# maciejkula/spotlight

Hardware: AMD Instinct MI355X
Metric: training interactions/sec, BPR dim=64 (higher is better)
Workload: dtype f32

## Files before the change

spotlight_amd/csrc/slk_api.hip:

```cpp
#include <stdarg.h>

#include <stdlib.h>

#include "slk_common.h"

static char g_create_err[512] = {0};

int slk_fail(slk_ctx *ctx, int code, const char *fmt, ...) {
    char *dst = ctx ? ctx->err : g_create_err;
    va_list ap;
    va_start(ap, fmt);
    vsnprintf(dst, 512, fmt, ap);
    va_end(ap);
    return code;
}

int slk_ensure(slk_ctx *ctx, slk_buf &b, size_t bytes) {
    if (bytes <= b.cap) return SLK_OK;
    if (b.p) {
        SLK_HIP(ctx, hipFree(b.p));
        b.p = nullptr;
        b.cap = 0;
    }
    size_t want = bytes + bytes / 8 + 256;
    void *p = nullptr;
    if (hipMalloc(&p, want) != hipSuccess) {
        (void)hipGetLastError();
        return slk_fail(ctx, SLK_ENOMEM, "hipMalloc of %zu scratch bytes failed", want);
    }
    b.p = p;
    b.cap = want;
    return SLK_OK;
}

int slk_ensure_lflags_host(slk_ctx *ctx, slk_prep_bufs &pb, size_t n) {
    if (n > pb.h_lflags_cap) {
        if (pb.h_lflags) (void)hipHostFree(pb.h_lflags);
        pb.h_lflags = nullptr;
        pb.h_lflags_cap = 0;
        void *p = nullptr;
        const size_t want = n + n / 4 + 64;
        if (hipHostMalloc(&p, want * sizeof(int), hipHostMallocDefault) != hipSuccess) {
            (void)hipGetLastError();
            return slk_fail(ctx, SLK_ENOMEM, "hipHostMalloc of %zu flag words failed", want);
        }
        pb.h_lflags = (int *)p;
        pb.h_lflags_cap = want;
    }
    for (size_t i = 0; i < n; ++i) pb.h_lflags[i] = 1;
    pb.h_lflags_n = n;
    return SLK_OK;
}

void slk_prof_begin(slk_ctx *ctx, int cls, hipStream_t s) {
    if (!ctx->prof_on) return;
    slk_prof_span sp;
    sp.cls = cls;
    for (hipEvent_t *e : {&sp.a, &sp.b}) {
        if (!ctx->ev_pool.empty()) {
            *e = ctx->ev_pool.back();
            ctx->ev_pool.pop_back();
        } else {
            (void)hipEventCreate(e);
        }
    }
    (void)hipEventRecord(sp.a, s);
    ctx->spans.push_back(sp);
}

void slk_prof_end(slk_ctx *ctx, hipStream_t s) {
    if (!ctx->prof_on) return;
    (void)hipEventRecord(ctx->spans.back().b, s);
    if (ctx->spans.size() >= 8192) slk_prof_drain(ctx);
}

int slk_prof_drain(slk_ctx *ctx) {
    for (slk_prof_span &sp : ctx->spans) {
        SLK_HIP(ctx, hipEventSynchronize(sp.b));
        float ms = 0.0f;
        SLK_HIP(ctx, hipEventElapsedTime(&ms, sp.a, sp.b));
        ctx->prof_launches[sp.cls] += 1;
        ctx->prof_ms[sp.cls] += (double)ms;
        ctx->ev_pool.push_back(sp.a);
        ctx->ev_pool.push_back(sp.b);
    }
    ctx->spans.clear();
    return SLK_OK;
}

int slk_prep_stream_init(slk_ctx *ctx) {
    if (ctx->prep_stream) return SLK_OK;
    SLK_HIP(ctx, hipStreamCreateWithFlags(&ctx->prep_stream, hipStreamNonBlocking));
    SLK_HIP(ctx, hipMemsetAsync(&ctx->d_rng->sort_abort, 0, sizeof(int32_t), ctx->prep_stream));
    SLK_HIP(ctx, hipStreamSynchronize(ctx->prep_stream));
    for (hipEvent_t *e : {&ctx->ev_start, &ctx->ev_prep[0], &ctx->ev_prep[1], &ctx->ev_done[0], &ctx->ev_done[1]})
        if (!*e) SLK_HIP(ctx, hipEventCreateWithFlags(e, hipEventDisableTiming));
    return SLK_OK;
}

hipStream_t slk_copy_stream(slk_ctx *ctx) {
    if (!ctx->copy_stream && hipStreamCreateWithFlags(&ctx->copy_stream, hipStreamNonBlocking) != hipSuccess) {
        (void)hipGetLastError();
        ctx->copy_stream = nullptr;
    }
    return ctx->copy_stream;
}

SLK_EXPORT int slk_abi_version(void) { return SLK_ABI_VERSION; }

SLK_EXPORT int slk_ctx_create(slk_ctx **out, int device_id) {
    if (!out) return slk_fail(nullptr, SLK_EINVAL, "slk_ctx_create: out is NULL");
    *out = nullptr;
    int ndev = 0;
    if (hipGetDeviceCount(&ndev) != hipSuccess || ndev <= 0) {
        (void)hipGetLastError();
        return slk_fail(nullptr, SLK_EIO, "slk_ctx_create: no HIP device visible");
    }
    if (device_id < 0 || device_id >= ndev)
        return slk_fail(nullptr, SLK_EINVAL, "slk_ctx_create: device %d out of range (%d devices)",
                        device_id, ndev);
    slk_ctx *ctx = new slk_ctx();
    ctx->device = device_id;
    if (hipSetDevice(device_id) != hipSuccess) {
        delete ctx;
        return slk_fail(nullptr, SLK_EIO, "slk_ctx_create: hipSetDevice(%d) failed", device_id);
    }
    hipDeviceProp_t prop;
    if (hipGetDeviceProperties(&prop, device_id) == hipSuccess && prop.multiProcessorCount > 0) {
        ctx->num_cus = prop.multiProcessorCount;
        if (prop.sharedMemPerBlock > 0) ctx->lds_per_block = prop.sharedMemPerBlock;
        if (prop.maxSharedMemoryPerMultiProcessor > 0) ctx->lds_per_cu = prop.maxSharedMemoryPerMultiProcessor;
        if (ctx->lds_per_cu < ctx->lds_per_block) ctx->lds_per_cu = ctx->lds_per_block;
    }
    if (hipMalloc(reinterpret_cast<void **>(&ctx->d_rng), sizeof(slk_rng_dev)) != hipSuccess) {
        delete ctx;
        return slk_fail(nullptr, SLK_ENOMEM, "slk_ctx_create: hipMalloc(rng) failed");
    }
    (void)hipMemset(ctx->d_rng, 0, sizeof(slk_rng_dev));
    int32_t pos = 624;
    (void)hipMemcpy(&ctx->d_rng->pos, &pos, sizeof(pos), hipMemcpyHostToDevice);
    *out = ctx;
    return SLK_OK;
}

SLK_EXPORT void slk_ctx_destroy(slk_ctx *ctx) {
    if (!ctx) return;
    if (ctx->shadow_active)
        fprintf(stderr, "libspotlight_hip: slk_ctx_destroy with an OPEN item-bias shadow (slk_bias_shadow_begin without _end): "
                        "the caller's item biases and their Adagrad accumulator keep their pre-scope values; the training of the "
                        "scope is lost\n");
    if (ctx->pp_active)
        fprintf(stderr, "libspotlight_hip: slk_ctx_destroy with an OPEN user-row ping-pong (slk_user_pingpong_begin without _end): "
                        "the rows whose current copy is the ctx's are not written back; the caller's user table is a mix of pre- and "
                        "in-scope rows -- the training of the scope is lost\n");
    (void)hipSetDevice(ctx->device);
    (void)hipDeviceSynchronize();
    slk_prof_drain(ctx);
    for (hipEvent_t e : ctx->ev_pool) (void)hipEventDestroy(e);
    slk_buf *bufs[] = {&ctx->raw, &ctx->cnt, &ctx->neg32, &ctx->ukey[0], &ctx->ukey[1], &ctx->uval[0],
                       &ctx->uval[1], &ctx->uit, &ctx->ikey[0], &ctx->ikey[1], &ctx->ipay[0],
                       &ctx->ipay[1], &ctx->gk, &ctx->sk, &ctx->snap, &ctx->losspart,
                       &ctx->sort_tmp, &ctx->dgrad[0], &ctx->dgrad[1], &ctx->dgrad[2], &ctx->dgrad[3], &ctx->ipart,
                       &ctx->ipart_meta, &ctx->upart_meta, &ctx->pf_neg, &ctx->call_neg, &ctx->mt_tmp, &ctx->bias_shadow, &ctx->pp_alt,
                       &ctx->pp_flags};
    for (slk_buf *b : bufs)
        if (b->p) (void)hipFree(b->p);
    for (slk_buf &b : ctx->extra)
        if (b.p) (void)hipFree(b.p);
    for (slk_prep_bufs &pb : ctx->pb) {
        slk_buf *pbs[] = {&pb.neg32, &pb.ukey[0], &pb.ukey[1], &pb.uval[0], &pb.uval[1], &pb.uit, &pb.ikey[0],
                          &pb.ikey[1], &pb.ipay[0], &pb.ipay[1], &pb.bik[0], &pb.bik[1], &pb.bip[0], &pb.bip[1],
                          &pb.buk[0], &pb.buk[1], &pb.bup[0], &pb.bup[1], &pb.lflags, &pb.mflag, &pb.msorted};
        for (slk_buf *b : pbs)
            if (b->p) (void)hipFree(b->p);
        if (pb.ev_lflags) (void)hipEventDestroy(pb.ev_lflags);
        if (pb.h_lflags) (void)hipHostFree(pb.h_lflags);
    }
    for (hipEvent_t e : {ctx->ev_start, ctx->ev_prep[0], ctx->ev_prep[1], ctx->ev_done[0], ctx->ev_done[1], ctx->ev_coef[0], ctx->ev_coef[1],
                         ctx->ev_sampled})
        if (e) (void)hipEventDestroy(e);
    for (void *h : ctx->h_coef)
        if (h) (void)hipHostFree(h);
    if (ctx->prep_stream) (void)hipStreamDestroy(ctx->prep_stream);
    if (ctx->copy_stream) (void)hipStreamDestroy(ctx->copy_stream);
    if (ctx->d_rng) (void)hipFree(ctx->d_rng);
    for (uint32_t *j : ctx->d_jump)
        if (j) (void)hipFree(j);
    delete ctx;
}

SLK_EXPORT const char *slk_last_error(const slk_ctx *ctx) { return ctx ? ctx->err : g_create_err; }

namespace {
struct slk_opt_desc {
    const char *name;
    int64_t lo, hi;
    int64_t (*get)(const slk_ctx *);
    void (*set)(slk_ctx *, int64_t);
};
#define SLK_OPT(name_, member_, lo_, hi_)                                              \
    {name_, (int64_t)(lo_), (int64_t)(hi_), [](const slk_ctx *c) -> int64_t { return (int64_t)c->member_; }, \
     [](slk_ctx *c, int64_t v) { c->member_ = (decltype(c->member_))v; }}
const int64_t SLK_OPT_MAX = INT64_MAX;
const slk_opt_desc slk_options[] = {
    SLK_OPT("chunk_interactions", opt_chunk_interactions, 1, SLK_OPT_MAX),
    SLK_OPT("overlap_prep", opt_overlap_prep, 0, 2),
    SLK_OPT("overlap_min_batch", opt_overlap_min_batch, 0, SLK_OPT_MAX),
    SLK_OPT("prefetch_wait", opt_prefetch_wait, 0, 1),
    SLK_OPT("mt_long_min_blocks", opt_mt_long_min_blocks, 2, SLK_OPT_MAX),
    SLK_OPT("sort_big_min", opt_sort_big_min, 1, SLK_OPT_MAX),
    SLK_OPT("sort_debug", opt_sort_debug, 0, 3),
    SLK_OPT("item_grid_mult", opt_item_grid_mult, 1, 4096),
    SLK_OPT("user_grid_mult", opt_user_grid_mult, 1, 4096),
    SLK_OPT("seq_variant", opt_seq_variant, 0, 1),
    SLK_OPT("explicit_fused", opt_explicit_fused, 0, 1),
    SLK_OPT("epoch_kernel", opt_epoch_kernel, 0, 1),
    SLK_OPT("item_lat_max_tiles", opt_item_lat_max_tiles, 0, SLK_OPT_MAX),
    SLK_OPT("epoch_adaptive", opt_epoch_adaptive, 0, 1),
    SLK_OPT("epoch_adaptive_max_batch", opt_epoch_adaptive_max_batch, 1, (int64_t)1 << 20),
    SLK_OPT("epoch_max_batch", opt_epoch_max_batch, 1, (int64_t)1 << 20),
    SLK_OPT("epoch_max_grid", opt_epoch_max_grid, 1, 16384),
    SLK_OPT("epoch_barrier", opt_epoch_barrier, -1, 1),
    SLK_OPT("epoch_cooperative", opt_epoch_cooperative, 0, 1),
    SLK_OPT("epoch_debug", opt_epoch_debug, 0, 63),
    SLK_OPT("epoch_dense_elems", opt_epoch_dense_elems, 0, SLK_OPT_MAX),
    SLK_OPT("user_lat_max_batch", opt_user_lat_max_batch, 0, SLK_OPT_MAX),
    SLK_OPT("item_long_gate", opt_item_long_gate, 0, 1),
    SLK_OPT("adaptive_late_min_batch", opt_adaptive_late_min_batch, 0, SLK_OPT_MAX),
    SLK_OPT("shuffle_band", opt_shuffle_band, 0, 1024),
    SLK_OPT("nt", opt_nt, 0, 63),
    SLK_OPT("record_nt_min_bytes", opt_record_nt_min_bytes, 0, SLK_OPT_MAX),
    SLK_OPT("user_bias_zero_hint", opt_user_bias_zero_hint, 0, 1),
    SLK_OPT("user_grid_own_occ", opt_user_grid_own_occ, 0, 1),
    SLK_OPT("item_single_min_items", opt_item_single_min_items, 0, SLK_OPT_MAX),
};
#undef SLK_OPT
const slk_opt_desc slk_eval_options[] = {
    {"topk_items_per_wg", 0, (int64_t)1 << 40, [](const slk_ctx *c) -> int64_t { return c->opt_topk_items_per_wg; },
     [](slk_ctx *c, int64_t v) { c->opt_topk_items_per_wg = v; }},
    {"eval_items_per_wg", 0, (int64_t)1 << 40, [](const slk_ctx *c) -> int64_t { return c->opt_eval_items_per_wg; },
     [](slk_ctx *c, int64_t v) { c->opt_eval_items_per_wg = v; }},
    {"foldin_wg_min_len", 0, (int64_t)1 << 40, [](const slk_ctx *c) -> int64_t { return c->opt_foldin_wg_min_len; },
     [](slk_ctx *c, int64_t v) { c->opt_foldin_wg_min_len = v; }},
};
const slk_opt_desc *slk_find_option(const char *name) {
    for (const slk_opt_desc &d : slk_options)
        if (!strcmp(name, d.name)) return &d;
    for (const slk_opt_desc &d : slk_eval_options)
        if (!strcmp(name, d.name)) return &d;
    return nullptr;
}
}

SLK_EXPORT int slk_ctx_set_option(slk_ctx *ctx, const char *name, int64_t value) {
    if (!ctx || !name) return SLK_EINVAL;
    const slk_opt_desc *d = slk_find_option(name);
    if (!d || value < d->lo || value > d->hi)
        return slk_fail(ctx, SLK_EINVAL, "slk_ctx_set_option: unknown option or bad value: %s = %lld", name,
                        (long long)value);
    d->set(ctx, value);
    return SLK_OK;
}

SLK_EXPORT int slk_ctx_get_option(slk_ctx *ctx, const char *name, int64_t *value) {
    if (!ctx || !name || !value) return SLK_EINVAL;
    const slk_opt_desc *d = slk_find_option(name);
    if (!d) return slk_fail(ctx, SLK_EINVAL, "slk_ctx_get_option: unknown option %s", name);
    *value = d->get(ctx);
    return SLK_OK;
}

SLK_EXPORT int slk_ctx_get_stat(slk_ctx *ctx, const char *name, int64_t *value) {
    if (!ctx || !name || !value) return SLK_EINVAL;
    if (!strcmp(name, "shuffle_sweeps")) *value = ctx->fy_sweeps;
    else if (!strcmp(name, "shuffle_fallbacks")) *value = ctx->fy_fallbacks;
    else if (!strcmp(name, "epoch_refused")) *value = ctx->epoch_refused ? 1 : 0;
    else if (!strcmp(name, "user_long_launches")) *value = ctx->stat_user_long;
    else if (!strcmp(name, "item_long_launches")) *value = ctx->stat_item_long;
    else if (!strcmp(name, "overlapped_chunks")) *value = ctx->stat_overlapped;
    else if (!strcmp(name, "prefetched_chunks")) *value = ctx->stat_prefetched;
    else if (!strcmp(name, "shadowed_calls")) *value = ctx->stat_shadowed;
    else if (!strcmp(name, "pingpong_calls")) *value = ctx->stat_pingpong;
    else if (!strcmp(name, "single_minibatches")) *value = ctx->stat_single;
    else if (!strcmp(name, "lds_per_block")) *value = (int64_t)ctx->lds_per_block;
    else if (!strcmp(name, "lds_per_cu")) *value = (int64_t)ctx->lds_per_cu;
    else if (!strcmp(name, "prefetch_pending")) *value = !ctx->pf.valid ? 0 : (ctx->pf.all ? 2 : 1);
    else return slk_fail(ctx, SLK_EINVAL, "slk_ctx_get_stat: unknown statistic %s", name);
    return SLK_OK;
}

SLK_EXPORT int slk_profile_enable(slk_ctx *ctx, int32_t on) {
    if (!ctx) return SLK_EINVAL;
    if (!on) slk_prof_drain(ctx);
    ctx->prof_on = on != 0;
    return SLK_OK;
}

SLK_EXPORT int slk_profile_read(slk_ctx *ctx, int32_t cls, int64_t *launches, double *total_ms) {
    if (!ctx || cls < 0 || cls >= SLK_K_COUNT) return SLK_EINVAL;
    int rc = slk_prof_drain(ctx);
    if (rc) return rc;
    if (launches) *launches = ctx->prof_launches[cls];
    if (total_ms) *total_ms = ctx->prof_ms[cls];
    return SLK_OK;
}

SLK_EXPORT int slk_profile_reset(slk_ctx *ctx) {
    if (!ctx) return SLK_EINVAL;
    int rc = slk_prof_drain(ctx);
    for (int i = 0; i < SLK_K_COUNT; ++i) {
        ctx->prof_launches[i] = 0;
        ctx->prof_ms[i] = 0.0;
    }
    return rc;
}
```

spotlight_amd/csrc/slk_bilinear.hip:

```cpp
#include <math.h>

#include "slk_kernels.h"

#ifndef SLK_PP_PIPE
#define SLK_PP_PIPE 2
#endif
template <int VEC, int G, int UPD, int UMODE, bool BLOOM, bool LAT = false, bool ULONG = false, bool PP = false, bool SGL = false>
__global__ __launch_bounds__(256) void k_user_pass(slk_pass_args a) {
    static_assert(!LAT || (UMODE == 0 && !BLOOM), "LAT is the pair mode over plain tables");
    static_assert(!PP || (UMODE == 0 && !BLOOM), "PP is the pair mode over plain tables");
    static_assert(!SGL || (PP && !LAT && !ULONG && UPD == SLK_UPD_ADAGRAD), "SGL: the plain ping-pong form, Adagrad");
    static_assert(!ULONG || !BLOOM, "long user runs: plain tables");
    constexpr uint32_t S = SLK_USER_TILE;
    constexpr bool PRE = UMODE != 0;
    constexpr bool EXPL = UMODE == 2;
    __shared__ double red[256];
    constexpr int GPB = 256 / G;
    const int lane = threadIdx.x % G;
    const int grp = threadIdx.x / G;
    const int D = a.D;
    const int d0 = lane * VEC;
    const bool on = d0 < D;
    const uint32_t stride = gridDim.x * GPB;
    float loss_acc = 0.0f;

    const uint32_t n_turns = ULONG ? (a.end - a.begin + S - 1u) / S : a.end - a.begin;
    constexpr bool PIPE = PP && !LAT && !ULONG && SLK_PP_PIPE >= 1;
    constexpr bool PIPE_IDS = PIPE && SLK_PP_PIPE >= 2;
    uint32_t pk_key = 0u, pk_prev = 0u, pk_flag = 0u, pn_key = 0u, pn_prev = 0u;
    uint32_t pk_ip = 0u, pk_in = 0u, pn_ip = 0u, pn_in = 0u;
    uint32_t pk_mf = 0u, pn_mf = 0u;
    auto ld_mf = [&](uint32_t pos) -> uint32_t { return (uint32_t)*reinterpret_cast<const uint16_t *>(a.mflag + 2 * (size_t)pos); };
    if (PIPE) {
        const uint32_t t0 = blockIdx.x * GPB + grp;
        if (t0 < n_turns) {
            pk_key = a.ukey[a.begin + t0];
            pk_prev = t0 > 0u ? a.ukey[a.begin + t0 - 1u] : 0u;
            if (PIPE_IDS) {
                pk_ip = a.uit[2 * (size_t)(a.begin + t0)];
                pk_in = a.uit[2 * (size_t)(a.begin + t0) + 1];
            }
            if (SGL) pk_mf = ld_mf(a.begin + t0);
            pk_flag = (uint32_t)a.uflag[pk_key & a.umask];
        }
        if (t0 + stride < n_turns) {
            pn_key = a.ukey[a.begin + t0 + stride];
            pn_prev = a.ukey[a.begin + t0 + stride - 1u];
            if (PIPE_IDS) {
                pn_ip = a.uit[2 * (size_t)(a.begin + t0 + stride)];
                pn_in = a.uit[2 * (size_t)(a.begin + t0 + stride) + 1];
            }
            if (SGL) pn_mf = ld_mf(a.begin + t0 + stride);
        }
    }
    for (uint32_t turn = blockIdx.x * GPB + grp; turn < n_turns; turn += stride) {
    const uint32_t p_lo = a.begin + (ULONG ? turn * S : turn);
    const uint32_t p_hi = ULONG ? (p_lo + S < a.end ? p_lo + S : a.end) : p_lo + 1u;
    for (uint32_t p = p_lo; p < p_hi; ++p) {
        const bool nt_keys = (SLK_NT_OF(a) & 8) != 0;
        const uint32_t key = PIPE ? pk_key : slk_ld_u32(a.ukey + p, nt_keys);
        uint32_t lat_ip = 0u, lat_in = 0u;
        bool is_head;
        uint32_t cur_piped = 0u, mf_piped = 0u;
        if (PIPE) {
            is_head = !(p > a.begin && pk_prev == key);
            cur_piped = pk_flag;
            lat_ip = pk_ip;
            lat_in = pk_in;
            mf_piped = pk_mf;
            pk_mf = pn_mf;
            pk_key = pn_key;
            pk_prev = pn_prev;
            pk_ip = pn_ip;
            pk_in = pn_in;
            if (turn + stride < n_turns) pk_flag = (uint32_t)a.uflag[pn_key & a.umask];
            if (turn + 2u * stride < n_turns) {
                pn_key = a.ukey[p + 2u * stride];
                pn_prev = a.ukey[p + 2u * stride - 1u];
                if (PIPE_IDS) {
                    pn_ip = a.uit[2 * (size_t)(p + 2u * stride)];
                    pn_in = a.uit[2 * (size_t)(p + 2u * stride) + 1];
                }
                if (SGL) pn_mf = ld_mf(p + 2u * stride);
            }
        } else if (LAT) {
            const uint32_t prev = p > a.begin ? a.ukey[p - 1] : ~key;
            lat_ip = a.uit[2 * (size_t)p];
            lat_in = a.uit[2 * (size_t)p + 1];
            is_head = prev != key;
        } else {
            is_head = !(p > a.begin && a.ukey[p - 1] == key);
        }
        bool run_long = false;
        uint32_t seg_limit = a.end;
        if (ULONG) {
            const uint32_t rel = p - a.begin;
            if (is_head) {
                const uint32_t t0 = a.begin + (rel + S - 1u) / S * S;
                run_long = t0 + S <= a.end && a.ukey[t0 + S - 1u] == key;
            } else if (rel % S == 0u) {
                run_long = (rel >= S && a.ukey[p - S] == key) || (p + S <= a.end && a.ukey[p + S - 1u] == key);
                is_head = false;
            }
            if (!is_head && !(run_long && rel % S == 0u)) continue;
            if (run_long) seg_limit = a.begin + (rel / S + 1u) * S < a.end ? a.begin + (rel / S + 1u) * S : a.end;
        } else if (!is_head) {
            continue;
        }
        const uint32_t user = key & a.umask;
        const size_t uoff = (size_t)user * D + d0;
        constexpr bool pp = PP;
        const uint32_t cur = PIPE ? cur_piped : (pp ? (uint32_t)a.uflag[user] : 0u);
        float *const unew = pp ? (cur ? a.P[0] : a.P0alt) + uoff : nullptr;
        slk_vec<VEC> u;
        if (BLOOM)
            u = slk_emb_vec<VEC>(a.P[0], a.ub, user, D, d0, on);
        else
            u = on ? slk_vload_if_nt<VEC>((cur ? a.P0alt : a.P[0]) + uoff, (SLK_NT_OF(a) & 1) != 0) : slk_vzero<VEC>();
        const float bu = (UMODE == 0 && !BLOOM && a.ubz) ? 0.0f : a.P[2][user];
        constexpr bool EARLY_ADAM = !BLOOM && UPD == SLK_UPD_SPARSE_ADAM && !ULONG;
        constexpr bool EARLY_STATE = ((EXPL || LAT || SGL || (PIPE && SLK_PP_PIPE >= 3)) && !BLOOM && UPD == SLK_UPD_ADAGRAD) || EARLY_ADAM;
        slk_vec<VEC> su = slk_vzero<VEC>(), su2 = slk_vzero<VEC>();
        if (EARLY_STATE && on) su = slk_vload_if_nt<VEC>(a.S1[0] + uoff, (SLK_NT_OF(a) & 1) != 0);
        if (EARLY_ADAM && on) su2 = slk_vload_if_nt<VEC>(a.S2[0] + uoff, (SLK_NT_OF(a) & 1) != 0);
        float sbu = 0.0f, sbu2 = 0.0f;
        if (EARLY_STATE && !(SGL && a.ubz)) sbu = a.S1[2][user];
        if (EARLY_ADAM) sbu2 = a.S2[2][user];
        slk_vec<VEC> gu = slk_vzero<VEC>();
        float gbu = 0.0f;
        uint32_t q = p;
        constexpr bool NEXT_KEY = UMODE != 0;
        uint32_t next_key = 0;
        if (NEXT_KEY) next_key = (q + 1 < seg_limit) ? a.ukey[q + 1] : ~key;
        do {
            float *rec = a.snap + (size_t)(q - a.begin) * a.RS;
            uint32_t e_item = 0;
            float e_rating = 0.0f;
            if (EXPL) {
                e_item = a.uit[q];
                e_rating = a.ratings[a.uk[q]];
            }
            if (on && !pp) slk_vstore_if_nt<VEC>(rec + d0, u, (SLK_NT_OF(a) & 16) != 0);
            if (!PRE) {
                uint32_t ip, in;
                if ((LAT || PIPE_IDS) && q == p) {
                    ip = lat_ip;
                    in = lat_in;
                } else {
                    ip = slk_ld_u32(a.uit + 2 * (size_t)q, nt_keys);
                    in = slk_ld_u32(a.uit + 2 * (size_t)q + 1, nt_keys);
                }
                slk_vec<VEC> vi, vj;
                if (BLOOM) {
                    vi = slk_emb_vec<VEC>(a.P[1], a.ib, ip, D, d0, on);
                    vj = slk_emb_vec<VEC>(a.P[1], a.ib, in, D, d0, on);
                } else {
                    vi = on ? slk_vload<VEC>(a.P[1] + (size_t)ip * D + d0) : slk_vzero<VEC>();
                    vj = on ? slk_vload<VEC>(a.P[1] + (size_t)in * D + d0) : slk_vzero<VEC>();
                }
                const float bip = a.P[3][SLK_B3(a, ip)], bin = a.P[3][SLK_B3(a, in)];
                uint32_t mf = 0xffffu;
                slk_vec<VEC> svi = slk_vzero<VEC>(), svj = slk_vzero<VEC>();
                float sbi = 0.0f, sbj = 0.0f;
                if (SGL) {
                    mf = (q == p) ? mf_piped : ld_mf(q);
                    const bool nt_rows = (SLK_NT_OF(a) & 2) != 0;
                    if (!(mf & 0xffu)) {
                        if (on) svi = slk_vload_if_nt<VEC>(a.S1[1] + (size_t)ip * D + d0, nt_rows);
                        if (lane == 0) sbi = a.S1[3][SLK_B3(a, ip)];
                    }
                    if (!(mf >> 8)) {
                        if (on) svj = slk_vload_if_nt<VEC>(a.S1[1] + (size_t)in * D + d0, nt_rows);
                        if (lane == 0) sbj = a.S1[3][SLK_B3(a, in)];
                    }
                }
                const float sp = slk_group_sum<G>(slk_vdot<VEC>(u, vi)) + bu + bip;
                const float sn = slk_group_sum<G>(slk_vdot<VEC>(u, vj)) + bu + bin;
                float l, gp, gn;
                slk_pair_loss(a.loss_kind, sp, sn, a.inv_b, l, gp, gn);
#pragma unroll
                for (int i = 0; i < VEC; ++i) gu.v[i] += gp * vi.v[i] + gn * vj.v[i];
                gbu += gp + gn;
                if (lane == 0) {
                    if (pp) {
                        float srcf;
                        const uint32_t src = user | (cur << 31);
                        memcpy(&srcf, &src, 4);
                        reinterpret_cast<float4 *>(a.gsn)[q - a.begin] = make_float4(gp, srcf, gn, srcf);
                    } else {
                        float *gq = a.gsn + 2 * (size_t)(q - a.begin);
                        gq[0] = gp;
                        gq[1] = gn;
                    }
                    loss_acc += l;
                }
                if (SGL) {
                    const bool nt_rows = (SLK_NT_OF(a) & 2) != 0;
                    auto once = [&](uint32_t item, slk_vec<VEC> &v, slk_vec<VEC> &sv, float g, float b, float bs) {
                        const size_t voff = (size_t)item * D + d0;
                        if (on) {
                            slk_vec<VEC> gv;
#pragma unroll
                            for (int i = 0; i < VEC; ++i) gv.v[i] = 0.0f + g * u.v[i];
                            slk_apply_vec_pre<VEC, UPD>(a, 1, voff, v, sv, gv, nullptr, nt_rows);
                        }
                        if (lane == 0) {
                            slk_vec<1> bpv, bsv, gbv;
                            bpv.v[0] = b;
                            bsv.v[0] = bs;
                            gbv.v[0] = 0.0f + g;
                            slk_apply_vec_pre<1, UPD>(a, 3, SLK_B3(a, item), bpv, bsv, gbv);
                        }
                    };
                    if (!(mf & 0xffu) && gp != 0.0f) once(ip, vi, svi, gp, bip, sbi);
                    if (!(mf >> 8) && gn != 0.0f) once(in, vj, svj, gn, bin, sbj);
                }
            } else if (EXPL) {
                const uint32_t it = e_item;
                const float bi = a.P[3][SLK_B3(a, it)];
                slk_vec<VEC> v;
                if (BLOOM)
                    v = slk_emb_vec<VEC>(a.P[1], a.ib, it, D, d0, on);
                else
                    v = on ? slk_vload<VEC>(a.P[1] + (size_t)it * D + d0) : slk_vzero<VEC>();
                const float sc = slk_group_sum<G>(slk_vdot<VEC>(u, v)) + bu + bi;
                float l, g;
                slk_explicit_loss(a.loss_kind, sc, e_rating, a.inv_b, a.end - a.begin, l, g);
                if (lane == 0) {
                    a.gsn[q - a.begin] = g;
                    loss_acc += l;
                }
                if (g != 0.0f) {
                    slk_vaxpy<VEC>(gu, g, v);
                    gbu += g;
                }
            } else {
                const size_t kb = (size_t)a.uk[q] * a.NP, qb = (size_t)q * a.NP;
                for (int s0 = 0; s0 < a.NP; s0 += G) {
                    const int s = s0 + lane;
                    float gs = 0.0f;
                    uint32_t it_l = 0u;
                    if (s < a.NP) {
                        gs = a.gk[kb + s];
                        it_l = a.uit[qb + s];
                        a.gsn[(size_t)(q - a.begin) * a.NP + s] = gs;
                    }
                    unsigned long long live = slk_group_or<G>(gs != 0.0f ? 1ull << lane : 0ull);
                    while (live) {
                        const int j0 = __builtin_ctzll(live);
                        live &= live - 1ull;
                        const bool two = live != 0ull;
                        const int j1 = two ? __builtin_ctzll(live) : j0;
                        if (two) live &= live - 1ull;
                        const uint32_t i0 = __shfl(it_l, j0, G), i1 = __shfl(it_l, j1, G);
                        const float g0 = __shfl(gs, j0, G), g1 = __shfl(gs, j1, G);
                        slk_vec<VEC> v0, v1 = slk_vzero<VEC>();
                        if (BLOOM) {
                            v0 = slk_emb_vec<VEC>(a.P[1], a.ib, i0, D, d0, on);
                            if (two) v1 = slk_emb_vec<VEC>(a.P[1], a.ib, i1, D, d0, on);
                        } else {
                            v0 = on ? slk_vload<VEC>(a.P[1] + (size_t)i0 * D + d0) : slk_vzero<VEC>();
                            if (two && on) v1 = slk_vload<VEC>(a.P[1] + (size_t)i1 * D + d0);
                        }
                        slk_vaxpy<VEC>(gu, g0, v0);
                        gbu += g0;
                        if (two) {
                            slk_vaxpy<VEC>(gu, g1, v1);
                            gbu += g1;
                        }
                    }
                }
            }
            ++q;
            if (NEXT_KEY) {
                if (next_key != key) break;
                next_key = (q + 1 < seg_limit) ? a.ukey[q + 1] : ~key;
            } else if (!(q < seg_limit && a.ukey[q] == key)) {
                break;
            }
        } while (true);

        if (ULONG && run_long) {
            const bool ends = !(q < a.end && a.ukey[q] == key);
            const size_t slot = 2 * (size_t)((p - a.begin) / S) + (is_head ? 1u : 0u);
            float *pp = a.upart + slot * (size_t)a.UPS;
            if (on) slk_vstore<VEC>(pp + d0, gu);
            if (lane == 0) {
                pp[a.UPS - 1] = gbu;
                a.upart_meta[2 * slot] = key;
                a.upart_meta[2 * slot + 1] = (a.upart_gen << SLK_IPART_GEN_SHIFT) | (is_head ? (uint32_t)SLK_IPART_STARTS : 0u) |
                                             (ends ? (uint32_t)SLK_IPART_ENDS : 0u);
                if (is_head) atomicAdd(a.upart_count, 1u);
            }
            p = q - 1u;
            continue;
        }
        if (BLOOM && a.ub.n_hash) {
            if (on) slk_vstore<VEC>(a.urec + (size_t)(p - a.begin) * a.RSU + d0, gu);
        } else if (on) {
            if (EARLY_ADAM)
                slk_apply_vec_pre<VEC, UPD, true>(a, 0, uoff, u, su, gu, &su2, (SLK_NT_OF(a) & 1) != 0, unew);
            else if (EARLY_STATE)
                slk_apply_vec_pre<VEC, UPD>(a, 0, uoff, u, su, gu, nullptr, (SLK_NT_OF(a) & 1) != 0, unew);
            else
                slk_apply_vec<VEC, UPD>(a, 0, uoff, u, gu, (SLK_NT_OF(a) & 1) != 0, unew);
        }
        if (pp && lane == 0) a.uflag[user] = (uint8_t)(cur ^ 1u);
        if (EARLY_ADAM) {
            if (lane == 0) {
                slk_vec<1> bpv, bsv, bsv2, gbv;
                bpv.v[0] = bu;
                bsv.v[0] = sbu;
                bsv2.v[0] = sbu2;
                gbv.v[0] = gbu;
                slk_apply_vec_pre<1, UPD, true>(a, 2, user, bpv, bsv, gbv, &bsv2);
            }
        } else if (EARLY_STATE) {
            if (lane == 0 && gbu != 0.0f) {
                slk_vec<1> bpv, bsv, gbv;
                bpv.v[0] = bu;
                bsv.v[0] = sbu;
                gbv.v[0] = gbu;
                slk_apply_vec_pre<1, UPD>(a, 2, user, bpv, bsv, gbv);
            }
        } else if (lane == 0) {
            slk_apply_bias<UPD>(a, 2, user, gbu);
        }
        if (ULONG) p = q - 1u;
    }
    }
    if (!PRE || EXPL) {
        const double tot = slk_block_sum_256((double)loss_acc, red);
        if (threadIdx.x == 0) a.loss_partial[blockIdx.x] = tot;
    }
}

template <int VEC, int G, int UPD, bool PP = false>
__global__ __launch_bounds__(256) void k_user_stitch(slk_pass_args a) {
    constexpr int GPB = 256 / G;
    constexpr uint32_t S = SLK_USER_TILE;
    const int lane = threadIdx.x % G;
    const int grp = threadIdx.x / G;
    const int D = a.D;
    const int d0 = lane * VEC;
    const bool on = d0 < D;
    const uint32_t ntiles = (a.end - a.begin + S - 1u) / S;
    if (*a.upart_count == 0u) return;
    const uint32_t gen = a.upart_gen;
    for (uint32_t tile = blockIdx.x * GPB + grp; tile < ntiles; tile += gridDim.x * GPB) {
        const size_t slot = 2 * (size_t)tile + 1;
        const uint32_t fl = a.upart_meta[2 * slot + 1];
        if ((fl >> SLK_IPART_GEN_SHIFT) != gen) continue;
        const uint32_t key = a.upart_meta[2 * slot];
        const float *pp = a.upart + slot * (size_t)a.UPS;
        slk_vec<VEC> gu = on ? slk_vload<VEC>(pp + d0) : slk_vzero<VEC>();
        float gbu = pp[a.UPS - 1];
        uint32_t t2 = tile + 1;
        bool more = (fl & SLK_IPART_ENDS) == 0;
        constexpr int R = G <= 16 ? 2 : 1;
        constexpr int TPR = R * G;
        constexpr bool SPEC = G <= 16;
        while (more) {
            slk_vec<VEC> sc[SPEC ? TPR : 1];
            float sb[SPEC ? TPR : 1];
            if (SPEC) {
#pragma unroll
                for (int e = 0; e < (SPEC ? TPR : 1); ++e) {
                    sc[e] = slk_vzero<VEC>();
                    sb[e] = 0.0f;
                    if (t2 + (uint32_t)e < ntiles) {
                        const float *q = a.upart + 2 * (size_t)(t2 + (uint32_t)e) * (size_t)a.UPS;
                        if (on) sc[e] = slk_vload<VEC>(q + d0);
                        sb[e] = q[a.UPS - 1];
                    }
                }
            }
            uint2 kf[R];
#pragma unroll
            for (int j = 0; j < R; ++j) {
                const uint32_t tl = t2 + (uint32_t)(lane + j * G);
                kf[j] = make_uint2(0u, 0u);
                if (tl < ntiles) kf[j] = *reinterpret_cast<const uint2 *>(a.upart_meta + 4 * (size_t)tl);
            }
            uint32_t f[R];
#pragma unroll
            for (int j = 0; j < R; ++j) {
                f[j] = kf[j].y;
                if (t2 + (uint32_t)(lane + j * G) >= ntiles || (f[j] >> SLK_IPART_GEN_SHIFT) != gen || (f[j] & SLK_IPART_STARTS) ||
                    kf[j].x != key)
                    f[j] = 0u;
                else
                    f[j] |= 1u;
            }
            int cnt = 0;
            bool ended = false;
#pragma unroll
            for (int j = 0; j < R; ++j) {
                if (!ended && cnt == j * G) {
                    const unsigned long long valid = slk_group_or<G>((f[j] & 1u) ? 1ull << lane : 0ull);
                    const unsigned long long ends = slk_group_or<G>((f[j] & SLK_IPART_ENDS) ? 1ull << lane : 0ull);
                    const unsigned long long full = G == 64 ? ~0ull : (1ull << G) - 1ull;
                    int c = (valid & full) == full ? G : __builtin_ctzll(~valid);
                    const unsigned long long e_in = ends & (c == 64 ? ~0ull : (1ull << c) - 1ull);
                    if (e_in) {
                        c = __builtin_ctzll(e_in) + 1;
                        ended = true;
                    }
                    cnt += c;
                }
            }
            if (SPEC) {
#pragma unroll
                for (int e = 0; e < (SPEC ? TPR : 1); ++e) {
                    if (e < cnt) {
#pragma unroll
                        for (int i = 0; i < VEC; ++i) gu.v[i] += sc[e].v[i];
                        gbu += sb[e];
                    }
                }
            }
            for (int l0 = 0; !SPEC && l0 < cnt; l0 += SLK_STITCH_BATCH) {
                slk_vec<VEC> cc[SLK_STITCH_BATCH];
                float cb[SLK_STITCH_BATCH];
#pragma unroll
                for (int e = 0; e < SLK_STITCH_BATCH; ++e) {
                    cc[e] = slk_vzero<VEC>();
                    cb[e] = 0.0f;
                    if (l0 + e < cnt) {
                        const float *q = a.upart + 2 * (size_t)(t2 + (uint32_t)(l0 + e)) * (size_t)a.UPS;
                        if (on) cc[e] = slk_vload<VEC>(q + d0);
                        cb[e] = q[a.UPS - 1];
                    }
                }
#pragma unroll
                for (int e = 0; e < SLK_STITCH_BATCH; ++e) {
                    if (l0 + e < cnt) {
#pragma unroll
                        for (int i = 0; i < VEC; ++i) gu.v[i] += cc[e].v[i];
                        gbu += cb[e];
                    }
                }
            }
            more = !ended && cnt == TPR;
            t2 += (uint32_t)TPR;
        }
        const uint32_t user = key & a.umask;
        const size_t uoff = (size_t)user * D + d0;
        constexpr bool pingpong = PP;
        uint32_t cur = 0u;
        if (pingpong) cur = __shfl(lane == 0 ? (uint32_t)a.uflag[user] : 0u, 0, G);
        if (on) {
            slk_vec<VEC> u = slk_vload_if_nt<VEC>((cur ? a.P0alt : a.P[0]) + uoff, (SLK_NT_OF(a) & 1) != 0);
            slk_apply_vec<VEC, UPD>(a, 0, uoff, u, gu, (SLK_NT_OF(a) & 1) != 0, pingpong ? (cur ? a.P[0] : a.P0alt) + uoff : nullptr);
        }
        if (pingpong && lane == 0) a.uflag[user] = (uint8_t)(cur ^ 1u);
        if (lane == 0) slk_apply_bias<UPD>(a, 2, user, gbu);
    }
}

__global__ __launch_bounds__(256) void k_user_long_flags(const uint32_t *ukey, uint32_t n, uint32_t per_mb, int *flags) {
    constexpr uint32_t S = SLK_USER_TILE;
    const uint32_t tiles_per_mb = (per_mb + S - 1) / S;
    const uint32_t n_mb = (n + per_mb - 1) / per_mb;
    for (uint32_t i = blockIdx.x * 256 + threadIdx.x; i < n_mb * tiles_per_mb; i += gridDim.x * 256) {
        const uint32_t mb = i / tiles_per_mb, q = i - mb * tiles_per_mb;
        const uint32_t w0 = mb * per_mb, w1 = (n - w0 < per_mb) ? n : w0 + per_mb;
        const uint32_t t0 = w0 + q * S;
        if (t0 >= w1 || w1 - t0 < S) continue;
        if (ukey[t0] == ukey[t0 + S - 1]) flags[mb] = 1;
    }
}

template <int VEC, int G>
__global__ __launch_bounds__(256) void k_score_pass(slk_pass_args a) {
    constexpr int GPB = 256 / G;
    const int lane = threadIdx.x % G;
    const int grp = threadIdx.x / G;
    const int D = a.D;
    const int d0 = lane * VEC;
    const bool on = d0 < D;
    const uint32_t stride = gridDim.x * GPB;
    for (uint32_t q = a.begin + blockIdx.x * GPB + grp; q < a.end; q += stride) {
        const uint32_t user = a.ukey[q] & a.umask;
        const slk_vec<VEC> u = slk_emb_vec<VEC>(a.P[0], a.ub, user, D, d0, on);
        const float bu = a.P[2][user];
        const size_t kb = (size_t)a.uk[q] * a.NP, qb = (size_t)q * a.NP;
        constexpr int SB = 3;
        for (int s0 = 0; s0 < a.NP; s0 += SB) {
            slk_vec<VEC> v[SB];
            float bi[SB];
#pragma unroll
            for (int j = 0; j < SB; ++j) {
                v[j] = slk_vzero<VEC>();
                bi[j] = 0.0f;
                if (s0 + j < a.NP) {
                    const uint32_t it = a.uit[qb + s0 + j];
                    v[j] = slk_emb_vec<VEC>(a.P[1], a.ib, it, D, d0, on);
                    bi[j] = a.P[3][SLK_B3(a, it)];
                }
            }
#pragma unroll
            for (int j = 0; j < SB; ++j) {
                const float sc = slk_group_sum<G>(slk_vdot<VEC>(u, v[j])) + bu + bi[j];
                if (lane == 0 && s0 + j < a.NP) a.sk[kb + s0 + j] = sc;
            }
        }
    }
}


__global__ __launch_bounds__(256) void k_explicit_loss(const float *sk, const float *ratings, float *gk, uint32_t k0,
                                                       uint32_t bm, int loss_kind, float inv_b, double *loss_partial) {
    __shared__ double red[256];
    double lsum = 0.0;
    for (uint32_t c = blockIdx.x * 256 + threadIdx.x; c < bm; c += gridDim.x * 256) {
        const float sc = sk[k0 + c], r = ratings[k0 + c];
        float l, g;
        slk_explicit_loss(loss_kind, sc, r, inv_b, bm, l, g);
        gk[k0 + c] = g;
        lsum += (double)l;
    }
    const double tot = slk_block_sum_256(lsum, red);
    if (threadIdx.x == 0) loss_partial[blockIdx.x] = tot;
}


struct slk_sweep_all_args {
    float *p[4], *s1[4], *s2[4], *g[4];
    size_t numel[4];
    unsigned first[5];
    int adam;
    float wd, w1, beta2, omb2, step_size, bc2_sqrt, eps, clr;
};

__global__ __launch_bounds__(256) void k_dense_sweep_all(slk_sweep_all_args a) {
    int t = 0;
    while (t < 3 && blockIdx.x >= a.first[t + 1]) ++t;
    const size_t local = blockIdx.x - a.first[t], nblk = a.first[t + 1] - a.first[t];
    float *p = a.p[t], *s1 = a.s1[t], *s2 = a.s2[t], *g = a.g[t];
    const size_t numel = a.numel[t];
    if (a.adam) {
        for (size_t e = local * 256 + threadIdx.x; e < numel; e += nblk * 256) {
            const float gv = g[e] + a.wd * p[e];
            g[e] = 0.0f;
            const float m = s1[e] + a.w1 * (gv - s1[e]);
            const float v = s2[e] * a.beta2 + a.omb2 * (gv * gv);
            s1[e] = m;
            s2[e] = v;
            p[e] += -a.step_size * (m / (sqrtf(v) / a.bc2_sqrt + a.eps));
        }
    } else {
        for (size_t e = local * 256 + threadIdx.x; e < numel; e += nblk * 256) {
            const float gv = g[e] + a.wd * p[e];
            g[e] = 0.0f;
            const float s = s1[e] + gv * gv;
            s1[e] = s;
            p[e] += -a.clr * (gv / (sqrtf(s) + a.eps));
        }
    }
}

__global__ __launch_bounds__(256) void k_i64_to_u32(const int64_t *in, uint32_t *out, size_t n) {
    for (size_t i = (size_t)blockIdx.x * 256 + threadIdx.x; i < n; i += (size_t)gridDim.x * 256)
        out[i] = (uint32_t)in[i];
}

__global__ __launch_bounds__(256) void k_u32_to_i64(const uint32_t *in, int64_t *out, size_t n) {
    for (size_t i = (size_t)blockIdx.x * 256 + threadIdx.x; i < n; i += (size_t)gridDim.x * 256)
        out[i] = (int64_t)in[i];
}

__global__ __launch_bounds__(256) void k_pack_items(const uint32_t *uk, const int64_t *items,
                                                    const uint32_t *neg32, uint32_t nc, int nn, uint32_t *uit) {
    const int NP = nn + 1;
    for (uint32_t q = blockIdx.x * 256 + threadIdx.x; q < nc; q += gridDim.x * 256) {
        const uint32_t k = uk[q];
        uit[(size_t)q * NP] = (uint32_t)items[k];
        for (int r = 0; r < nn; ++r) uit[(size_t)q * NP + 1 + r] = neg32[(size_t)k * nn + r];
    }
}

__global__ __launch_bounds__(256) void k_invert_perm(const uint32_t *uk, uint32_t nc, uint32_t *qk) {
    for (uint32_t q = blockIdx.x * 256 + threadIdx.x; q < nc; q += gridDim.x * 256) qk[uk[q]] = q;
}

__global__ __launch_bounds__(256) void k_build_live_keys(const uint32_t *live, const uint32_t *uit, uint32_t n_live,
                                                         slk_bloom_dev ib, bool hashed, uint32_t *key, uint32_t *val) {
    const uint32_t H = hashed ? (uint32_t)ib.n_hash : 1u;
    for (uint32_t e = blockIdx.x * 256 + threadIdx.x; e < n_live * H; e += gridDim.x * 256) {
        const uint32_t l = e / H, h = e - l * H;
        const uint32_t r = live[l];
        uint32_t k = 0xffffffffu;
        if (r != 0xffffffffu) k = hashed ? slk_bloom_row(ib, uit[r], (int)h) : uit[r];
        key[e] = k;
        val[e] = r;
    }
}

__global__ __launch_bounds__(256) void k_build_item_bloom_keys(const uint32_t *uit, uint32_t nocc, int NP,
                                                               uint32_t bsz, unsigned cbits, slk_bloom_dev ib,
                                                               uint32_t *key, uint32_t *val) {
    const uint32_t H = (uint32_t)ib.n_hash;
    for (uint32_t e = blockIdx.x * 256 + threadIdx.x; e < nocc * H; e += gridDim.x * 256) {
        const uint32_t r = e / H, h = e - r * H;
        const uint32_t q = r / (uint32_t)NP;
        key[e] = ((q / bsz) << cbits) | slk_bloom_row(ib, uit[r], (int)h);
        val[e] = r;
    }
}

__global__ __launch_bounds__(256) void k_build_user_bloom_keys(const uint32_t *ukey, uint32_t umask, uint32_t nc,
                                                               uint32_t bsz, unsigned cbits, slk_bloom_dev ub,
                                                               uint32_t *key, uint32_t *val) {
    const uint32_t H = (uint32_t)ub.n_hash;
    for (uint32_t e = blockIdx.x * 256 + threadIdx.x; e < nc * H; e += gridDim.x * 256) {
        const uint32_t p = e / H, h = e - p * H;
        const uint32_t mb = p / bsz;
        const bool head = (p % bsz == 0) || ukey[p - 1] != ukey[p];
        key[e] = (mb << cbits) | (head ? slk_bloom_row(ub, ukey[p] & umask, (int)h) : ub.rows);
        val[e] = p;
    }
}

template <int VEC, int G>
__global__ __launch_bounds__(256) void k_predict(const float *U, const float *V, const float *bu,
                                                 const float *bi, int D, slk_bloom_dev ub, slk_bloom_dev ib,
                                                 const int64_t *users, int64_t n_users, const int64_t *items,
                                                 int64_t n, float *out) {
    constexpr int GPB = 256 / G;
    const int lane = threadIdx.x % G;
    const int grp = threadIdx.x / G;
    const int d0 = lane * VEC;
    const bool on = d0 < D;
    for (int64_t k = (int64_t)blockIdx.x * GPB + grp; k < n; k += (int64_t)gridDim.x * GPB) {
        const int64_t u = users[n_users == 1 ? 0 : k];
        const int64_t i = items ? items[k] : k;
        const slk_vec<VEC> a = slk_emb_vec<VEC>(U, ub, (uint32_t)u, D, d0, on);
        const slk_vec<VEC> b = slk_emb_vec<VEC>(V, ib, (uint32_t)i, D, d0, on);
        const float s = (slk_chain_dot<VEC, G>(a, b) + bu[u]) + bi[i];
        if (lane == 0) out[k] = s;
    }
}

typedef slk_pass_fn pass_fn;

template <int VEC, int G, bool BLOOM>
static pass_fn user_pass_fn2(int upd, int umode) {
    if (umode == 2) {
        if (upd == SLK_UPD_ADAGRAD) return k_user_pass<VEC, G, SLK_UPD_ADAGRAD, 2, BLOOM>;
        if (upd == SLK_UPD_SPARSE_ADAM) return k_user_pass<VEC, G, SLK_UPD_SPARSE_ADAM, 2, BLOOM>;
        if (upd == SLK_UPD_SGD) return k_user_pass<VEC, G, SLK_UPD_SGD, 2, BLOOM>;
        return k_user_pass<VEC, G, SLK_UPD_GRAD_ONLY, 2, BLOOM>;
    }
    if (umode == 1) {
        if (upd == SLK_UPD_ADAGRAD) return k_user_pass<VEC, G, SLK_UPD_ADAGRAD, 1, BLOOM>;
        if (upd == SLK_UPD_SPARSE_ADAM) return k_user_pass<VEC, G, SLK_UPD_SPARSE_ADAM, 1, BLOOM>;
        if (upd == SLK_UPD_SGD) return k_user_pass<VEC, G, SLK_UPD_SGD, 1, BLOOM>;
        return k_user_pass<VEC, G, SLK_UPD_GRAD_ONLY, 1, BLOOM>;
    }
    if (upd == SLK_UPD_ADAGRAD) return k_user_pass<VEC, G, SLK_UPD_ADAGRAD, 0, BLOOM>;
    if (upd == SLK_UPD_SPARSE_ADAM) return k_user_pass<VEC, G, SLK_UPD_SPARSE_ADAM, 0, BLOOM>;
    if (upd == SLK_UPD_SGD) return k_user_pass<VEC, G, SLK_UPD_SGD, 0, BLOOM>;
    return k_user_pass<VEC, G, SLK_UPD_GRAD_ONLY, 0, BLOOM>;
}

template <int VEC, int G, bool ULONG = false>
static pass_fn user_pass_lat_fn(int upd) {
    if (upd == SLK_UPD_ADAGRAD) return k_user_pass<VEC, G, SLK_UPD_ADAGRAD, 0, false, true, ULONG>;
    if (upd == SLK_UPD_SPARSE_ADAM) return k_user_pass<VEC, G, SLK_UPD_SPARSE_ADAM, 0, false, true, ULONG>;
    if (upd == SLK_UPD_SGD) return k_user_pass<VEC, G, SLK_UPD_SGD, 0, false, true, ULONG>;
    return k_user_pass<VEC, G, SLK_UPD_GRAD_ONLY, 0, false, true, ULONG>;
}

template <int VEC, int G, bool LAT, bool ULONG>
static pass_fn user_pass_pp_fn(int upd) {
    if (upd == SLK_UPD_ADAGRAD) return k_user_pass<VEC, G, SLK_UPD_ADAGRAD, 0, false, LAT, ULONG, true>;
    if (upd == SLK_UPD_SPARSE_ADAM) return k_user_pass<VEC, G, SLK_UPD_SPARSE_ADAM, 0, false, LAT, ULONG, true>;
    return k_user_pass<VEC, G, SLK_UPD_SGD, 0, false, LAT, ULONG, true>;
}
template <int VEC, int G>
static pass_fn user_pass_sgl_fn() {
    return k_user_pass<VEC, G, SLK_UPD_ADAGRAD, 0, false, false, false, true, true>;
}
template <int VEC, int G>
static slk_item_fns item_pass_sgl_fn() {
    return {k_item_pass<VEC, G, SLK_UPD_ADAGRAD, SLK_ITEM_SNAPPPS>, k_item_stitch<VEC, G, SLK_UPD_ADAGRAD, SLK_PART_BOTH>,
            k_item_pass<VEC, G, SLK_UPD_ADAGRAD, SLK_ITEM_SNAPPPS, SLK_PART_BOTH, false>,
            k_item_pass<VEC, G, SLK_UPD_ADAGRAD, SLK_ITEM_SNAPPPS, SLK_PART_BOTH, false, 4>};
}
template <int VEC, int G>
static pass_fn user_stitch_pp_fn(int upd) {
    if (upd == SLK_UPD_ADAGRAD) return k_user_stitch<VEC, G, SLK_UPD_ADAGRAD, true>;
    if (upd == SLK_UPD_SPARSE_ADAM) return k_user_stitch<VEC, G, SLK_UPD_SPARSE_ADAM, true>;
    return k_user_stitch<VEC, G, SLK_UPD_SGD, true>;
}
template <int VEC, int G>
static slk_item_fns item_pass_pp_fn(int upd) {
    if (upd == SLK_UPD_ADAGRAD)
        return {k_item_pass<VEC, G, SLK_UPD_ADAGRAD, SLK_ITEM_SNAPPP>, k_item_stitch<VEC, G, SLK_UPD_ADAGRAD, SLK_PART_BOTH>,
                k_item_pass<VEC, G, SLK_UPD_ADAGRAD, SLK_ITEM_SNAPPP, SLK_PART_BOTH, false>,
                k_item_pass<VEC, G, SLK_UPD_ADAGRAD, SLK_ITEM_SNAPPP, SLK_PART_BOTH, false, 4>};
    if (upd == SLK_UPD_SPARSE_ADAM)
        return {k_item_pass<VEC, G, SLK_UPD_SPARSE_ADAM, SLK_ITEM_SNAPPP>, k_item_stitch<VEC, G, SLK_UPD_SPARSE_ADAM, SLK_PART_BOTH>,
                k_item_pass<VEC, G, SLK_UPD_SPARSE_ADAM, SLK_ITEM_SNAPPP, SLK_PART_BOTH, false>,
                k_item_pass<VEC, G, SLK_UPD_SPARSE_ADAM, SLK_ITEM_SNAPPP, SLK_PART_BOTH, false, 4>};
    return {k_item_pass<VEC, G, SLK_UPD_SGD, SLK_ITEM_SNAPPP>, k_item_stitch<VEC, G, SLK_UPD_SGD, SLK_PART_BOTH>,
            k_item_pass<VEC, G, SLK_UPD_SGD, SLK_ITEM_SNAPPP, SLK_PART_BOTH, false>,
            k_item_pass<VEC, G, SLK_UPD_SGD, SLK_ITEM_SNAPPP, SLK_PART_BOTH, false, 4>};
}

template <int VEC, int G, int UMODE>
static pass_fn user_pass_long_fn1(int upd) {
    if (upd == SLK_UPD_ADAGRAD) return k_user_pass<VEC, G, SLK_UPD_ADAGRAD, UMODE, false, false, true>;
    if (upd == SLK_UPD_SPARSE_ADAM) return k_user_pass<VEC, G, SLK_UPD_SPARSE_ADAM, UMODE, false, false, true>;
    if (upd == SLK_UPD_SGD) return k_user_pass<VEC, G, SLK_UPD_SGD, UMODE, false, false, true>;
    return k_user_pass<VEC, G, SLK_UPD_GRAD_ONLY, UMODE, false, false, true>;
}
template <int VEC, int G>
static pass_fn user_pass_long_fn(int upd, int umode) {
    if (umode == 2) return user_pass_long_fn1<VEC, G, 2>(upd);
    if (umode == 1) return user_pass_long_fn1<VEC, G, 1>(upd);
    return user_pass_long_fn1<VEC, G, 0>(upd);
}
template <int VEC, int G>
static pass_fn user_stitch_fn(int upd) {
    if (upd == SLK_UPD_ADAGRAD) return k_user_stitch<VEC, G, SLK_UPD_ADAGRAD>;
    if (upd == SLK_UPD_SPARSE_ADAM) return k_user_stitch<VEC, G, SLK_UPD_SPARSE_ADAM>;
    if (upd == SLK_UPD_SGD) return k_user_stitch<VEC, G, SLK_UPD_SGD>;
    return k_user_stitch<VEC, G, SLK_UPD_GRAD_ONLY>;
}

template <int VEC, int G>
static pass_fn user_pass_fn(int upd, int umode, bool bloom) {
    return bloom ? user_pass_fn2<VEC, G, true>(upd, umode) : user_pass_fn2<VEC, G, false>(upd, umode);
}


int slk_check_tables(slk_ctx *ctx, const slk_tables *t, unsigned table_mask, int *vec, int *g, bool shadow_ok, bool pingpong_ok) {
    if (!t) return slk_fail(ctx, SLK_EINVAL, "tables is NULL");
    for (int i = 0; i < 4; ++i)
        if (((table_mask >> i) & 1u) && !t->d_param[i])
            return slk_fail(ctx, SLK_EINVAL, "tables->d_param[%d] is NULL", i);
    if (!shadow_ok && (table_mask & 8u) && ctx->shadow_active && t->d_param[3] == ctx->shadow_src_p)
        return slk_fail(ctx, SLK_EINVAL, "the item biases of these tables are shadowed (slk_bias_shadow_begin): the array is stale until "
                                         "slk_bias_shadow_end, and only slk_bilinear_train indexes the shadow");
    if (!pingpong_ok && (table_mask & 1u) && ctx->pp_active && t->d_param[0] == ctx->pp_src_u)
        return slk_fail(ctx, SLK_EINVAL, "the user rows of these tables are ping-ponged (slk_user_pingpong_begin): the array holds only "
                                         "some of the current rows until slk_user_pingpong_end, and only slk_bilinear_train reads both copies");
    if (((table_mask & 5u) && (t->num_users < 1 || t->num_users >= ((int64_t)1 << 31))) || t->num_items < 1 ||
        t->num_items >= ((int64_t)1 << 31))
        return slk_fail(ctx, SLK_EINVAL, "table rows must be in [1, 2^31): users %lld items %lld",
                        (long long)t->num_users, (long long)t->num_items);
    if (!slk_pick_layout(t->dim, vec, g))
        return slk_fail(ctx, SLK_EINVAL,
                        "embedding dim %d unsupported (need dim %% 4 == 0 and <= 256, or dim <= 64)", t->dim);
    const slk_bloom *bl[2] = {(table_mask & 1u) ? t->user_bloom : nullptr, (table_mask & 2u) ? t->item_bloom : nullptr};
    for (int side = 0; side < 2; ++side) {
        const slk_bloom *b = bl[side];
        if (!b) continue;
        if (b->n_hash < 1 || b->n_hash > 8 || b->rows < 1 || b->rows >= ((int64_t)1 << 30) || b->skip_row >= b->rows ||
            b->skip_row < -1 || b->padding_idx < -1)
            return slk_fail(ctx, SLK_EINVAL, "bad BloomEmbedding descriptor: rows %lld n_hash %d skip_row %lld",
                            (long long)b->rows, b->n_hash, (long long)b->skip_row);
    }
    return SLK_OK;
}

int slk_check_optim(slk_ctx *ctx, const slk_optim *optim, unsigned table_mask) {
    if (!optim) return slk_fail(ctx, SLK_EINVAL, "optim is NULL");
    if (optim->kind < SLK_OPT_ADAGRAD || optim->kind > SLK_OPT_SGD)
        return slk_fail(ctx, SLK_EINVAL, "unknown optimizer kind %d", optim->kind);
    if (optim->kind == SLK_OPT_SGD) {
        if (optim->weight_decay != 0.0) return slk_fail(ctx, SLK_EINVAL, "SGD: weight_decay must be 0 (a full-table sweep per step is not built)");
        return SLK_OK;
    }
    const bool need_s2 = optim->kind == SLK_OPT_SPARSE_ADAM || optim->kind == SLK_OPT_ADAM_DENSE;
    for (int i = 0; i < 4; ++i) {
        if (!((table_mask >> i) & 1u)) continue;
        if (!optim->d_state1[i]) return slk_fail(ctx, SLK_EINVAL, "optim->d_state1[%d] is NULL", i);
        if (need_s2 && !optim->d_state2[i]) return slk_fail(ctx, SLK_EINVAL, "optim->d_state2[%d] is NULL", i);
    }
    if (optim->kind == SLK_OPT_ADAGRAD && optim->weight_decay != 0.0)
        return slk_fail(ctx, SLK_EINVAL, "row-sparse Adagrad requires weight_decay == 0 (use ADAGRAD_DENSE)");
    return SLK_OK;
}

int slk_ensure_dgrad(slk_ctx *ctx, const size_t elems[4], unsigned table_mask, hipStream_t s) {
    for (int t = 0; t < 4; ++t) {
        if (!((table_mask >> t) & 1u)) continue;
        if (ctx->dgrad_elems[t] != elems[t] || !ctx->dgrad[t].p) {
            int rc = slk_ensure(ctx, ctx->dgrad[t], elems[t] * 4);
            if (rc) return rc;
            SLK_HIP(ctx, hipMemsetAsync(ctx->dgrad[t].p, 0, elems[t] * 4, s));
            ctx->dgrad_elems[t] = elems[t];
        }
    }
    return SLK_OK;
}

int slk_dense_sweeps(slk_ctx *ctx, float *const params[4], const slk_optim *optim, unsigned table_mask,
                     hipStream_t s) {
    const double step = (double)(optim->step + 1);
    slk_prof_begin(ctx, SLK_K_DENSE_SWEEP, s);
    slk_sweep_all_args w;
    memset(&w, 0, sizeof(w));
    w.wd = (float)optim->weight_decay;
    w.eps = (float)optim->eps;
    w.adam = optim->kind == SLK_OPT_ADAM_DENSE;
    if (w.adam) {
        const double bc1 = 1.0 - pow(optim->beta1, step), bc2 = 1.0 - pow(optim->beta2, step);
        w.w1 = (float)(1.0 - optim->beta1);
        w.beta2 = (float)optim->beta2;
        w.omb2 = (float)(1.0 - optim->beta2);
        w.step_size = (float)(optim->lr / bc1);
        w.bc2_sqrt = (float)sqrt(bc2);
    } else {
        w.clr = (float)(optim->lr / (1.0 + (step - 1.0) * optim->lr_decay));
    }
    unsigned blocks = 0;
    for (int t = 0; t < 4; ++t) {
        w.first[t] = blocks;
        if (!((table_mask >> t) & 1u)) continue;
        w.p[t] = params[t];
        w.s1[t] = optim->d_state1[t];
        w.s2[t] = optim->d_state2[t];
        w.g[t] = (float *)ctx->dgrad[t].p;
        w.numel[t] = ctx->dgrad_elems[t];
        blocks += slk_grid_for(ctx, w.numel[t], 256);
    }
    w.first[4] = blocks;
    if (blocks) {
        hipLaunchKernelGGL(k_dense_sweep_all, dim3(blocks), dim3(256), 0, s, w);
        SLK_LAUNCH_CHECK(ctx, "k_dense_sweep_all");
    }
    slk_prof_end(ctx, s);
    return SLK_OK;
}

int slk_launch_i64_to_u32(slk_ctx *ctx, const int64_t *in, uint32_t *out, size_t n, hipStream_t s) {
    hipLaunchKernelGGL(k_i64_to_u32, dim3(slk_grid_for(ctx, n, 256)), dim3(256), 0, s, in, out, n);
    SLK_LAUNCH_CHECK(ctx, "k_i64_to_u32");
    return SLK_OK;
}

SLK_EXPORT int slk_bilinear_predict(slk_ctx *ctx, const slk_tables *tables, const int64_t *d_users,
                                    int64_t n_users, const int64_t *d_items, int64_t n, float *d_out,
                                    void *stream) {
    if (!ctx) return SLK_EINVAL;
    int vec, g, rc;
    if ((rc = slk_check_tables(ctx, tables, 15u, &vec, &g))) return rc;
    if (n < 0 || !d_users || (n > 0 && !d_out)) return slk_fail(ctx, SLK_EINVAL, "slk_bilinear_predict: bad arguments");
    if (n_users != 1 && n_users != n)
        return slk_fail(ctx, SLK_EINVAL, "slk_bilinear_predict: n_users must be 1 or n (%lld vs %lld)",
                        (long long)n_users, (long long)n);
    if (n == 0) return SLK_OK;
    SLK_HIP(ctx, hipSetDevice(ctx->device));
    hipStream_t s = (hipStream_t)stream;
    ctx->last_stream = s;
    slk_prof_begin(ctx, SLK_K_SCORE, s);
    if (n_users == 1 && !d_items) {
        if (n != tables->num_items)
            return slk_fail(ctx, SLK_EINVAL, "slk_bilinear_predict: d_items == NULL scores all %lld items, n is %lld",
                            (long long)tables->num_items, (long long)n);
        const float *rep, *rbias;
        const int64_t *gmap;
        if ((rc = slk_eval_user_rep(ctx, tables, vec, g, d_users, &rep, &rbias, &gmap, s))) return rc;
        rc = slk_eval_predict_all(ctx, tables, rep, rbias, gmap, d_out, s);
        slk_prof_end(ctx, s);
        return rc;
    }
#define SLK_PREDICT(V_, G_)                                                                          \
    hipLaunchKernelGGL((k_predict<V_, G_>), dim3(slk_grid_for(ctx, (size_t)n, 256 / G_)), dim3(256), 0, s, \
                       (const float *)tables->d_param[0], (const float *)tables->d_param[1],          \
                       (const float *)tables->d_param[2], (const float *)tables->d_param[3],          \
                       (int)tables->dim, ubd, ibd, d_users, n_users, d_items, n, d_out)
    slk_bloom_dev ubd, ibd;
    slk_bloom_to_dev(tables->user_bloom, &ubd);
    slk_bloom_to_dev(tables->item_bloom, &ibd);
    SLK_FOR_LAYOUT(vec, g, SLK_PREDICT);
#undef SLK_PREDICT
    SLK_LAUNCH_CHECK(ctx, "k_predict");
    slk_prof_end(ctx, s);
    return SLK_OK;
}

struct train_call {
    enum { TRAIN, RESERVE, PREFETCH } mode;
    const slk_tables *tables;
    slk_optim *optim;
    const int64_t *users, *items;
    const float *ratings;
    const int64_t *neg_in;
    int64_t *neg_out;
    float *mb_loss;
    int64_t n, batch_size;
    int32_t loss, n_neg;
    hipStream_t s;
};

struct train_plan {
    int vec, g, D;
    int RS, RSU, UPS;
    size_t utiles;
    unsigned ubits, ibits, ucbits, icbits;
    slk_bloom_dev ubd, ibd;
    int Hu, Hi;
    bool bloom, adaptive, expl, fused, pre, dense, late;
    int nn, NP, umode, nsets;
    int64_t bsz, mb_per_chunk, chunk_cap, occ_mult;
    size_t nc_max, n_chunks;
    bool side, pingpong, sgl_on, shadowed, one_draw, epoch_route;
    size_t dense_elems[4];
};

struct train_run {
    const uint32_t *neg_all;
    int64_t mb_global;
    bool epoch_route;
};

struct train_kernels {
    pass_fn upass, spass, upass_lat, upass_long, upass_lat_long, ustitch, upass_sgl;
    slk_item_fns ipass, ipass_rows, ipass_bias, rpass_rows, ipass_sgl;
    unsigned gpb;
    int occ_user, occ_sgl;
};

static inline uint32_t *u32p(const slk_buf &b) { return (uint32_t *)b.p; }
static inline float *f32p(const slk_buf &b) { return (float *)b.p; }
static inline int64_t chunk_begin(const train_plan &p, size_t ck) { return (int64_t)ck * p.chunk_cap; }
static inline uint32_t chunk_len(const train_plan &p, const train_call &c, size_t ck) {
    const int64_t c1 = chunk_begin(p, ck + 1);
    return (uint32_t)((c1 < c.n ? c1 : c.n) - chunk_begin(p, ck));
}

static int run_training(slk_ctx *ctx, const train_call &c);

SLK_EXPORT int slk_bilinear_train(slk_ctx *ctx, const slk_tables *tables, slk_optim *optim,
                                  const int64_t *d_users, const int64_t *d_items, int64_t n,
                                  int64_t batch_size, int32_t loss, int32_t n_neg, const int64_t *d_neg_in,
                                  int64_t *d_neg_out, float *d_mb_loss, void *stream) {
    return run_training(ctx, {train_call::TRAIN, tables, optim, d_users, d_items, nullptr, d_neg_in, d_neg_out, d_mb_loss, n,
                              batch_size, loss, n_neg, (hipStream_t)stream});
}

SLK_EXPORT int slk_bilinear_reserve(slk_ctx *ctx, const slk_tables *tables, const slk_optim *optim, int64_t n,
                                    int64_t batch_size, int32_t loss, int32_t n_neg, void *stream) {
    slk_optim o;
    if (!optim) return slk_fail(ctx, SLK_EINVAL, "optim is NULL");
    o = *optim;
    return run_training(ctx, {train_call::RESERVE, tables, &o, nullptr, nullptr, nullptr, nullptr, nullptr, nullptr, n, batch_size,
                              loss, n_neg, (hipStream_t)stream});
}

SLK_EXPORT int slk_bilinear_prefetch(slk_ctx *ctx, const slk_tables *tables, const slk_optim *optim, const int64_t *d_users,
                                     const int64_t *d_items, int64_t n, int64_t batch_size, int32_t loss, int32_t n_neg,
                                     const uint32_t *h_key, int32_t pos, void *stream) {
    if (!ctx) return SLK_EINVAL;
    if (!optim) return slk_fail(ctx, SLK_EINVAL, "optim is NULL");
    if (h_key) {
        if (pos < 0 || pos > 624) return slk_fail(ctx, SLK_EINVAL, "slk_bilinear_prefetch: pos %d outside [0, 624]", pos);
        SLK_HIP(ctx, hipSetDevice(ctx->device));
        if (ctx->sampled_valid && ctx->ev_sampled) SLK_HIP(ctx, hipEventSynchronize(ctx->ev_sampled));
        int rc = slk_rng_write_state(ctx, h_key, pos);
        if (rc) return rc;
    }
    slk_optim o = *optim;
    return run_training(ctx, {train_call::PREFETCH, tables, &o, d_users, d_items, nullptr, nullptr, nullptr, nullptr, n, batch_size,
                              loss, n_neg, (hipStream_t)stream});
}

SLK_EXPORT int slk_bilinear_train_explicit(slk_ctx *ctx, const slk_tables *tables, slk_optim *optim,
                                           const int64_t *d_users, const int64_t *d_items, const float *d_ratings,
                                           int64_t n, int64_t batch_size, int32_t loss, float *d_mb_loss,
                                           void *stream) {
    if (ctx && (loss < SLK_LOSS_REGRESSION || loss > SLK_LOSS_LOGISTIC))
        return slk_fail(ctx, SLK_EINVAL, "slk_bilinear_train_explicit: loss kind %d is not regression/poisson/logistic", loss);
    if (ctx && n > 0 && !d_ratings) return slk_fail(ctx, SLK_EINVAL, "slk_bilinear_train_explicit: d_ratings is NULL");
    return run_training(ctx, {train_call::TRAIN, tables, optim, d_users, d_items, d_ratings, nullptr, nullptr, d_mb_loss, n,
                              batch_size, loss, 0, (hipStream_t)stream});
}

static int plan_training(slk_ctx *ctx, const train_call &c, train_plan *plan) {
    train_plan &p = *plan;
    const slk_tables *tables = c.tables;
    const slk_optim *optim = c.optim;
    const bool reserve = c.mode == train_call::RESERVE, prefetch = c.mode == train_call::PREFETCH;
    const int64_t n = c.n;
    int rc;
    p.n_chunks = 0;
    if ((rc = slk_check_tables(ctx, tables, 15u, &p.vec, &p.g, true, true))) return rc;
    if ((rc = slk_check_optim(ctx, optim, 15u))) return rc;
    if (n < 0 || c.batch_size < 1) return slk_fail(ctx, SLK_EINVAL, "slk_bilinear_train: n %lld batch_size %lld",
                                                   (long long)n, (long long)c.batch_size);
    if (c.loss < SLK_LOSS_POINTWISE || c.loss > SLK_LOSS_LOGISTIC)
        return slk_fail(ctx, SLK_EINVAL, "unknown loss kind %d", c.loss);
    p.adaptive = c.loss == SLK_LOSS_ADAPTIVE_HINGE;
    p.expl = c.loss >= SLK_LOSS_REGRESSION;
    if (p.expl != (c.ratings != nullptr) && !reserve)
        return slk_fail(ctx, SLK_EINVAL, "ratings go with (and only with) the regression/poisson/logistic losses");
    p.fused = p.expl && ctx->opt_explicit_fused;
    p.pre = p.adaptive || p.expl;
    p.umode = p.fused ? 2 : (p.pre ? 1 : 0);
    p.nn = p.adaptive ? c.n_neg : (p.expl ? 0 : 1);
    if (!p.expl && (p.nn < 1 || p.nn > 1024)) return slk_fail(ctx, SLK_EINVAL, "num_negative_samples %d outside [1, 1024]", p.nn);
    p.NP = p.nn + 1;
    p.dense = optim->kind == SLK_OPT_ADAM_DENSE || optim->kind == SLK_OPT_ADAGRAD_DENSE;
    if (n == 0) return SLK_OK;
    if (!reserve && (!c.users || !c.items || (!c.mb_loss && !prefetch)))
        return slk_fail(ctx, SLK_EINVAL, "slk_bilinear_train: NULL id/loss pointer");
    if (c.batch_size * (int64_t)p.NP >= ((int64_t)1 << 31))
        return slk_fail(ctx, SLK_EINVAL, "batch_size * (1 + negatives) must be < 2^31");
    SLK_HIP(ctx, hipSetDevice(ctx->device));
    ctx->last_stream = c.s;

    p.D = tables->dim;
    p.ubits = slk_bits_for((uint64_t)tables->num_users - 1);
    p.ibits = slk_bits_for((uint64_t)tables->num_items - 1);
    unsigned idbits = p.ubits > p.ibits ? p.ubits : p.ibits;
    slk_bloom_to_dev(tables->user_bloom, &p.ubd);
    slk_bloom_to_dev(tables->item_bloom, &p.ibd);
    p.bloom = p.ubd.n_hash || p.ibd.n_hash;
    const int Hu = p.Hu = p.ubd.n_hash, Hi = p.Hi = p.ibd.n_hash;
    p.ucbits = Hu ? slk_bits_for((uint64_t)p.ubd.rows) : 0;
    p.icbits = Hi ? slk_bits_for((uint64_t)p.ibd.rows - 1) : 0;
    if (p.ucbits > idbits) idbits = p.ucbits;
    if (p.icbits > idbits) idbits = p.icbits;
    p.occ_mult = (int64_t)p.NP * (Hi ? Hi : 1) > (int64_t)(Hu ? Hu : 1) ? (int64_t)p.NP * (Hi ? Hi : 1) : (int64_t)(Hu ? Hu : 1);
    const int64_t bsz = p.bsz = c.batch_size < n ? c.batch_size : n;
    int64_t mb_per_chunk = (int64_t)1 << (32 - idbits);
    const int64_t cap_inter = ctx->opt_chunk_interactions;
    if (mb_per_chunk * bsz > cap_inter) mb_per_chunk = cap_inter / bsz;
    while (mb_per_chunk > 1 && mb_per_chunk * bsz * p.occ_mult >= ((int64_t)1 << 31)) mb_per_chunk >>= 1;
    if (mb_per_chunk < 1) mb_per_chunk = 1;
    if (bsz * p.occ_mult >= ((int64_t)1 << 31))
        return slk_fail(ctx, SLK_EINVAL, "batch_size * lookups per interaction must be < 2^31");
    const bool maybe_epoch = ctx->opt_epoch_kernel && !ctx->epoch_refused && bsz <= ctx->opt_epoch_max_batch;
    if (maybe_epoch && mb_per_chunk > ((int64_t)1 << 13)) mb_per_chunk = (int64_t)1 << 13;
    p.mb_per_chunk = mb_per_chunk;
    p.chunk_cap = mb_per_chunk * bsz;
    p.nc_max = (size_t)(p.chunk_cap < n ? p.chunk_cap : n);
    p.n_chunks = (size_t)((n + p.chunk_cap - 1) / p.chunk_cap);

    p.late = p.adaptive && optim->kind != SLK_OPT_SPARSE_ADAM && (Hi > 0 || bsz >= ctx->opt_adaptive_late_min_batch);
    p.side = ctx->opt_overlap_prep && p.n_chunks > 1 && bsz >= ctx->opt_overlap_min_batch;
    p.nsets = p.n_chunks > 1 ? 2 : 1;
    p.one_draw = !c.neg_in && p.nn > 0 && p.n_chunks > 1 && (uint64_t)n * (uint64_t)p.nn < ((uint64_t)1 << 30);
    p.RS = (p.D + 3) / 4 * 4;
    p.UPS = p.RS + 4;
    p.utiles = ((size_t)bsz + SLK_USER_TILE - 1) / SLK_USER_TILE;
    p.RSU = p.D + 4;
    p.pingpong = ctx->pp_active && ctx->pp_src_u == tables->d_param[0];
    if (ctx->pp_active && !p.pingpong && !reserve)
        return slk_fail(ctx, SLK_EINVAL, "slk_bilinear_train: a user-row ping-pong (slk_user_pingpong_begin) is open on this ctx for OTHER "
                                         "tables; close it (slk_user_pingpong_end / _abort) before training another model");
    if (p.pingpong && (p.pre || p.bloom || p.dense || tables->num_users != ctx->pp_rows || p.D != ctx->pp_dim))
        return slk_fail(ctx, SLK_EINVAL, "slk_bilinear_train: the user rows are ping-ponged (slk_user_pingpong_begin): only the pair losses "
                                         "(pointwise, bpr, hinge) over plain tables of the scope's shape with a row-sparse optimizer train inside the scope");
    p.sgl_on = p.pingpong && optim->kind == SLK_OPT_ADAGRAD && ctx->opt_item_single_min_items > 0 &&
               tables->num_items >= ctx->opt_item_single_min_items;
    p.shadowed = ctx->shadow_active && ctx->shadow_src_p == tables->d_param[3] && !p.dense &&
                 optim->kind == SLK_OPT_ADAGRAD && ctx->shadow_src_s == optim->d_state1[3];
    if (ctx->shadow_active && !p.shadowed && ctx->shadow_src_p == tables->d_param[3])
        return slk_fail(ctx, SLK_EINVAL, "slk_bilinear_train: the item biases are shadowed (slk_bias_shadow_begin) for another optimizer state");
    if (ctx->shadow_active && !p.shadowed && !reserve)
        return slk_fail(ctx, SLK_EINVAL, "slk_bilinear_train: an item-bias shadow (slk_bias_shadow_begin) is open on this ctx for OTHER "
                                         "tables; close it (slk_bias_shadow_end / _abort) before training another model");
    p.epoch_route = !p.shadowed && !p.pingpong && (!p.pre || p.adaptive || p.fused) &&
                    slk_epoch_eligible(ctx, tables, optim, bsz, c.loss, p.bloom);
    p.dense_elems[0] = (size_t)(Hu ? p.ubd.rows : tables->num_users) * p.D;
    p.dense_elems[1] = (size_t)(Hi ? p.ibd.rows : tables->num_items) * p.D;
    p.dense_elems[2] = (size_t)tables->num_users;
    p.dense_elems[3] = (size_t)tables->num_items;
    return SLK_OK;
}

static int ensure_dense_buffers(slk_ctx *ctx, const train_plan &p, hipStream_t s) { return slk_ensure_dgrad(ctx, p.dense_elems, 15u, s); }

static int ensure_scratch(slk_ctx *ctx, const train_plan &p, hipStream_t s) {
    const size_t nc_max = p.nc_max, NP = (size_t)p.NP, Hi = (size_t)p.Hi, Hu = (size_t)p.Hu, bsz = (size_t)p.bsz;
    const bool late = p.late;
    int rc;
    for (int st = 0; st < p.nsets; ++st) {
        slk_prep_bufs &pb = ctx->pb[st];
        if ((rc = slk_ensure(ctx, pb.neg32, nc_max * p.nn * 4))) return rc;
        for (int b = 0; b < 2; ++b) {
            if ((rc = slk_ensure(ctx, pb.ukey[b], nc_max * 4))) return rc;
            if ((rc = slk_ensure(ctx, pb.uval[b], nc_max * 8))) return rc;
            if (!late && (rc = slk_ensure(ctx, pb.ikey[b], nc_max * NP * 4))) return rc;
            if (!(late && b == 1) && (rc = slk_ensure(ctx, pb.ipay[b], late ? nc_max * 4 : nc_max * NP * 4))) return rc;
            if (!late && Hi && (rc = slk_ensure(ctx, pb.bik[b], nc_max * NP * Hi * 4))) return rc;
            if (!late && Hi && (rc = slk_ensure(ctx, pb.bip[b], nc_max * NP * Hi * 4))) return rc;
            if (Hu && (rc = slk_ensure(ctx, pb.buk[b], nc_max * Hu * 4))) return rc;
            if (Hu && (rc = slk_ensure(ctx, pb.bup[b], nc_max * Hu * 4))) return rc;
        }
        if (p.pre && (rc = slk_ensure(ctx, pb.uit, nc_max * NP * 4))) return rc;
        if (p.sgl_on && (rc = slk_ensure(ctx, pb.mflag, nc_max * NP + 16))) return rc;
        if (p.sgl_on && (rc = slk_ensure(ctx, pb.msorted, nc_max * NP + 16))) return rc;
        if ((rc = slk_ensure(ctx, pb.lflags, 2 * (size_t)p.mb_per_chunk * 4))) return rc;
    }
    if ((rc = slk_ensure(ctx, ctx->snap, bsz * p.RS * 4))) return rc;
    if ((rc = slk_ensure(ctx, ctx->extra[BL_GSN], bsz * NP * (p.pingpong ? 8 : 4)))) return rc;
    const unsigned max_grid = (unsigned)ctx->num_cus * (unsigned)(ctx->opt_user_grid_mult > 8 ? ctx->opt_user_grid_mult : 8);
    if ((rc = slk_ensure(ctx, ctx->losspart, (size_t)max_grid * 8))) return rc;
    if (p.pre) {
        if ((rc = slk_ensure(ctx, ctx->gk, nc_max * NP * 4))) return rc;
        if ((rc = slk_ensure(ctx, ctx->sk, nc_max * NP * 4))) return rc;
    }
    if (late) {
        const size_t nl = 2 * bsz, nlh = nl * (Hi ? Hi : 1);
        if ((rc = slk_ensure(ctx, ctx->extra[BL_LIVE], nl * 4))) return rc;
        for (int b = 0; b < 4; ++b)
            if ((rc = slk_ensure(ctx, ctx->extra[BL_LK0 + b], nlh * 4))) return rc;
    }
    if (!p.bloom) {
        if ((rc = slk_ensure(ctx, ctx->extra[BL_UPART], 2 * p.utiles * (size_t)p.UPS * 4))) return rc;
        const size_t meta_bytes = 2 * p.utiles * 8 + 64;
        if (meta_bytes > ctx->upart_meta.cap) {
            if ((rc = slk_ensure(ctx, ctx->upart_meta, meta_bytes))) return rc;
            SLK_HIP(ctx, hipMemsetAsync(ctx->upart_meta.p, 0, ctx->upart_meta.cap, s));
        }
    }
    if (Hu && (rc = slk_ensure(ctx, ctx->extra[BL_UREC], bsz * p.RSU * 4))) return rc;
    if (p.dense && !p.epoch_route && (rc = ensure_dense_buffers(ctx, p, s))) return rc;
    return SLK_OK;
}

static int warm_prep_stream(slk_ctx *ctx, const train_plan &p, const train_call &c) {
    hipStream_t s = c.s, ps = ctx->prep_stream;
    slk_prep_bufs &pb = ctx->pb[1];
    int rc;
    if ((rc = slk_ensure(ctx, ctx->extra[BL_LIVE], sizeof(slk_rng_dev) + 64))) return rc;
    SLK_HIP(ctx, hipEventRecord(ctx->ev_start, s));
    SLK_HIP(ctx, hipStreamWaitEvent(ps, ctx->ev_start, 0));
    SLK_HIP(ctx, hipMemcpyAsync(ctx->extra[BL_LIVE].p, ctx->d_rng, sizeof(slk_rng_dev), hipMemcpyDeviceToDevice, ps));
    if ((rc = slk_sample_u32(ctx, c.tables->num_items, 4096, u32p(pb.neg32), nullptr, ps))) return rc;
    SLK_HIP(ctx, hipMemcpyAsync(ctx->d_rng, ctx->extra[BL_LIVE].p, sizeof(slk_rng_dev), hipMemcpyDeviceToDevice, ps));
    SLK_HIP(ctx, hipMemsetAsync(pb.ukey[0].p, 0, 4096 * 4, ps));
    if ((rc = slk_sort_pairs_u32_u64(ctx, u32p(pb.ukey[0]), u32p(pb.ukey[1]), (const uint64_t *)pb.uval[0].p, (uint64_t *)pb.uval[1].p,
                                     4096, 20, ps)))
        return rc;
    if (!p.late) {
        SLK_HIP(ctx, hipMemsetAsync(pb.ikey[0].p, 0, 4096 * 4, ps));
        if ((rc = slk_sort_pairs_u32_u32(ctx, u32p(pb.ikey[0]), u32p(pb.ikey[1]), u32p(pb.ipay[0]), u32p(pb.ipay[1]), 4096, 20, ps)))
            return rc;
    }
    SLK_HIP(ctx, hipEventRecord(ctx->ev_prep[1], ps));
    SLK_HIP(ctx, hipStreamWaitEvent(s, ctx->ev_prep[1], 0));
    SLK_HIP(ctx, hipEventRecord(ctx->ev_done[1], s));
    SLK_HIP(ctx, hipStreamWaitEvent(ps, ctx->ev_done[1], 0));
    SLK_HIP(ctx, hipStreamSynchronize(ps));
    SLK_HIP(ctx, hipStreamSynchronize(s));
    ctx->last_stream = s;
    ctx->sampled_valid = false;
    ctx->prep_warmed = true;
    return SLK_OK;
}

static int reserve_extras(slk_ctx *ctx, const train_plan &p, const train_call &c) {
    int rc;
    if (p.side && (rc = slk_prep_stream_init(ctx))) return rc;
    for (int st = 0; st < p.nsets; ++st) {
        slk_prep_bufs &pb = ctx->pb[st];
        if ((rc = slk_ensure_lflags_host(ctx, pb, 2 * (size_t)p.mb_per_chunk))) return rc;
        pb.h_lflags_n = 0;
        if (!pb.ev_lflags) SLK_HIP(ctx, hipEventCreateWithFlags(&pb.ev_lflags, hipEventDisableTiming));
    }
    if (p.side && !ctx->prep_warmed && p.nn > 0 && p.nc_max >= 4096 && (rc = warm_prep_stream(ctx, p, c))) return rc;
    const uint32_t n_mb = (uint32_t)((p.nc_max + p.bsz - 1) / p.bsz);
    if (p.epoch_route && (rc = slk_epoch_reserve(ctx, c.tables, c.optim, n_mb, p.bsz, (int)c.loss, p.NP))) return rc;
    if (p.one_draw && (rc = slk_ensure(ctx, ctx->call_neg, (size_t)c.n * p.nn * 4))) return rc;
    if ((rc = slk_sample_reserve(ctx, c.tables->num_items, p.one_draw ? c.n * (int64_t)p.nn : (int64_t)p.nc_max * p.nn))) return rc;
    return slk_sort_reserve(ctx, p.nc_max * (size_t)p.occ_mult);
}

static void pick_kernels(slk_ctx *ctx, const train_plan &p, const slk_optim *optim, train_kernels *kernels) {
    train_kernels &k = *kernels;
    const int upd = slk_upd_for(optim->kind), umode = p.umode;
    const bool bloom = p.bloom;
    k = train_kernels{};
#define SLK_PICK(V_, G_)                                                                    \
    do {                                                                                    \
        k.upass = user_pass_fn<V_, G_>(upd, umode, bloom);                                  \
        if (umode == 0 && !bloom) k.upass_lat = user_pass_lat_fn<V_, G_>(upd);              \
        if (umode == 0 && !bloom) k.upass_lat_long = user_pass_lat_fn<V_, G_, true>(upd);   \
        if (!bloom) k.upass_long = user_pass_long_fn<V_, G_>(upd, umode);                   \
        if (!bloom) k.ustitch = user_stitch_fn<V_, G_>(upd);                                \
        k.ipass = slk_item_pass_fn<V_, G_, SLK_ITEM_SNAP>(upd);                             \
        k.spass = k_score_pass<V_, G_>;                                                     \
        if (p.pingpong) {                                                                   \
            k.upass = user_pass_pp_fn<V_, G_, false, false>(upd);                           \
            k.upass_lat = user_pass_pp_fn<V_, G_, true, false>(upd);                        \
            k.upass_long = user_pass_pp_fn<V_, G_, false, true>(upd);                       \
            k.upass_lat_long = user_pass_pp_fn<V_, G_, true, true>(upd);                    \
            k.ustitch = user_stitch_pp_fn<V_, G_>(upd);                                     \
            k.ipass = item_pass_pp_fn<V_, G_>(upd);                                         \
            if (p.sgl_on) {                                                                 \
                k.upass_sgl = user_pass_sgl_fn<V_, G_>();                                   \
                k.ipass_sgl = item_pass_sgl_fn<V_, G_>();                                   \
            }                                                                               \
        }                                                                                   \
        if (bloom) {                                                                        \
            k.ipass_rows = slk_item_pass_fn<V_, G_, SLK_ITEM_SNAP, SLK_PART_ROWS>(upd);     \
            k.ipass_bias = slk_item_pass_fn<V_, G_, SLK_ITEM_SNAP, SLK_PART_BIAS>(upd);     \
            k.rpass_rows = slk_item_pass_fn<V_, G_, SLK_ITEM_ROW, SLK_PART_ROWS>(upd);      \
        }                                                                                   \
    } while (0)
    SLK_FOR_LAYOUT(p.vec, p.g, SLK_PICK);
#undef SLK_PICK
    k.gpb = 256u / (unsigned)p.g;
    k.occ_user = slk_occupancy_of(ctx, k.upass);
    for (pass_fn f : {k.upass_lat, k.upass_long, k.upass_lat_long}) {
        const int o = slk_occupancy_of(ctx, f);
        if (o < k.occ_user) k.occ_user = o;
    }
    k.occ_sgl = p.sgl_on ? slk_occupancy_of(ctx, k.upass_sgl) : k.occ_user;
}

static int prep_sample(slk_ctx *ctx, const train_plan &p, const train_call &c, const train_run &run, size_t ck, slk_prep_bufs &pb, hipStream_t s) {
    const int64_t c0 = chunk_begin(p, ck);
    const size_t nneg = (size_t)chunk_len(p, c, ck) * p.nn;
    if (run.neg_all) return SLK_OK;

    if (p.nn == 0) return SLK_OK;
    if (c.neg_in) {
        slk_prof_begin(ctx, SLK_K_SAMPLE, s);
        hipLaunchKernelGGL(k_i64_to_u32, dim3(slk_grid_for(ctx, nneg, 256)), dim3(256), 0, s, c.neg_in + c0 * p.nn, u32p(pb.neg32), nneg);
        SLK_LAUNCH_CHECK(ctx, "k_i64_to_u32");
        if (c.neg_out)
            SLK_HIP(ctx, hipMemcpyAsync(c.neg_out + c0 * p.nn, c.neg_in + c0 * p.nn, nneg * 8, hipMemcpyDeviceToDevice, s));
        slk_prof_end(ctx, s);
        return SLK_OK;
    }
    return slk_sample_u32(ctx, c.tables->num_items, (int64_t)nneg, u32p(pb.neg32), c.neg_out ? c.neg_out + c0 * p.nn : nullptr, s);
}

static int prep_single_flags(slk_ctx *ctx, const train_plan &p, const train_call &c, slk_prep_bufs &pb, size_t ck, hipStream_t s) {
    const uint32_t nocc = chunk_len(p, c, ck) * (uint32_t)p.NP;
    SLK_HIP(ctx, hipMemsetAsync(pb.mflag.p, 0, (size_t)nocc, s));
    hipLaunchKernelGGL(k_item_multi_flags, dim3(slk_grid_for(ctx, nocc, 256)), dim3(256), 0, s, (const uint32_t *)pb.ikey[1].p,
                       (const uint32_t *)pb.ipay[1].p, nocc, (uint32_t)p.bsz * (uint32_t)p.NP, (uint8_t *)pb.msorted.p, (uint8_t *)pb.mflag.p);
    SLK_LAUNCH_CHECK(ctx, "k_item_multi_flags");
    return SLK_OK;
}

static int prep_sort(slk_ctx *ctx, const train_plan &p, const train_call &c, const train_run &run, size_t ck, slk_prep_bufs &pb, hipStream_t s) {
    int rc;
    const int64_t c0 = chunk_begin(p, ck);
    const uint32_t nc = chunk_len(p, c, ck), nocc = nc * (uint32_t)p.NP, bsz = (uint32_t)p.bsz;
    const int64_t *cu = c.users + c0, *ci = c.items + c0;
    const uint32_t *neg32 = run.neg_all ? run.neg_all + (size_t)c0 * p.nn : u32p(pb.neg32);
    const int Hi = p.Hi, Hu = p.Hu;

    slk_prof_begin(ctx, SLK_K_PREP, s);
    const unsigned mbbits = slk_bits_for((uint64_t)((nc - 1) / bsz));
    uint32_t *const ukey = u32p(pb.ukey[1]);
    const uint32_t *uit, *uk = nullptr;
    uint32_t *const ukeys[2] = {u32p(pb.ukey[0]), ukey};
    if (!p.pre) {
        uint64_t *const uvals[2] = {(uint64_t *)pb.uval[0].p, (uint64_t *)pb.uval[1].p};
        if ((rc = slk_sort_user_fat(ctx, cu, ci, neg32, nc, (size_t)bsz, p.ubits, mbbits, ukeys, uvals, s))) return rc;
        uit = u32p(pb.uval[1]);
    } else {
        uint32_t *const uvals[2] = {u32p(pb.uval[0]), u32p(pb.uval[1])};
        if ((rc = slk_sort_user_idx(ctx, cu, nc, (size_t)bsz, p.ubits, mbbits, ukeys, uvals, s))) return rc;
        uk = u32p(pb.uval[1]);
        hipLaunchKernelGGL(k_pack_items, dim3(slk_grid_for(ctx, nc, 256)), dim3(256), 0, s, uk, ci, neg32, nc, p.nn, u32p(pb.uit));
        SLK_LAUNCH_CHECK(ctx, "k_pack_items");
        uit = u32p(pb.uit);
    }
    if (p.late) {
        hipLaunchKernelGGL(k_invert_perm, dim3(slk_grid_for(ctx, nc, 256)), dim3(256), 0, s, uk, nc, u32p(pb.ipay[0]));
        SLK_LAUNCH_CHECK(ctx, "k_invert_perm");
    } else {
        uint32_t *const ikeys[2] = {u32p(pb.ikey[0]), u32p(pb.ikey[1])};
        uint32_t *const ivals[2] = {u32p(pb.ipay[0]), u32p(pb.ipay[1])};
        if ((rc = slk_sort_item_occ(ctx, uit, nocc, (size_t)bsz, p.NP, p.ibits, mbbits, ikeys, ivals, s))) return rc;
        if (p.sgl_on && (rc = prep_single_flags(ctx, p, c, pb, ck, s))) return rc;
    }
    if (!run.epoch_route) {
        const uint32_t n_mb_c = (nc + bsz - 1) / bsz;
        const unsigned gpb = 256u / (unsigned)p.g;
        if ((rc = slk_ensure(ctx, pb.lflags, 2 * (size_t)n_mb_c * 4))) return rc;
        SLK_HIP(ctx, hipMemsetAsync(pb.lflags.p, 0, 2 * (size_t)n_mb_c * 4, s));
        if (!p.late) {
            hipLaunchKernelGGL(k_item_long_flags, dim3(slk_grid_for(ctx, nocc / (4 * gpb) + n_mb_c, 256)), dim3(256), 0, s,
                               (const uint32_t *)pb.ikey[1].p, nocc, bsz * (uint32_t)p.NP, 4u * gpb,
                               (uint32_t)((1ull << p.ibits) - 1), 0xffffffffu, 0xffffffffu, (int *)pb.lflags.p);
            SLK_LAUNCH_CHECK(ctx, "k_item_long_flags");
        }
        if (!p.bloom) {
            hipLaunchKernelGGL(k_user_long_flags, dim3(slk_grid_for(ctx, nc / SLK_USER_TILE + n_mb_c, 256)), dim3(256), 0, s,
                               (const uint32_t *)ukey, nc, bsz, (int *)pb.lflags.p + n_mb_c);
            SLK_LAUNCH_CHECK(ctx, "k_user_long_flags");
        }
        if ((rc = slk_ensure_lflags_host(ctx, pb, 2 * (size_t)n_mb_c))) return rc;
        SLK_HIP(ctx, hipMemcpyAsync(pb.h_lflags, pb.lflags.p, 2 * (size_t)n_mb_c * 4, hipMemcpyDeviceToHost, s));
        if (!pb.ev_lflags) SLK_HIP(ctx, hipEventCreateWithFlags(&pb.ev_lflags, hipEventDisableTiming));
        SLK_HIP(ctx, hipEventRecord(pb.ev_lflags, s));
    } else {
        pb.h_lflags_n = 0;
    }
    if (Hi && !p.late) {
        hipLaunchKernelGGL(k_build_item_bloom_keys, dim3(slk_grid_for(ctx, (size_t)nocc * Hi, 256)), dim3(256), 0, s,
                           uit, nocc, p.NP, bsz, p.icbits, p.ibd, u32p(pb.bik[0]), u32p(pb.bip[0]));
        SLK_LAUNCH_CHECK(ctx, "k_build_item_bloom_keys");
        if ((rc = slk_sort_pairs_u32_u32(ctx, u32p(pb.bik[0]), u32p(pb.bik[1]), u32p(pb.bip[0]), u32p(pb.bip[1]), (size_t)nocc * Hi,
                                         p.icbits + mbbits, s, true)))
            return rc;
    }
    if (Hu) {
        hipLaunchKernelGGL(k_build_user_bloom_keys, dim3(slk_grid_for(ctx, (size_t)nc * Hu, 256)), dim3(256), 0, s,
                           (const uint32_t *)ukey, (uint32_t)((1ull << p.ubits) - 1), nc, bsz, p.ucbits, p.ubd,
                           u32p(pb.buk[0]), u32p(pb.bup[0]));
        SLK_LAUNCH_CHECK(ctx, "k_build_user_bloom_keys");
        if ((rc = slk_sort_pairs_u32_u32(ctx, u32p(pb.buk[0]), u32p(pb.buk[1]), u32p(pb.bup[0]), u32p(pb.bup[1]), (size_t)nc * Hu,
                                         p.ucbits + mbbits, s, true)))
            return rc;
    }
    slk_prof_end(ctx, s);
    return SLK_OK;
}

struct minibatch {
    uint32_t b0, b1, bm;
    slk_pass_args a;
    int ugm;
    unsigned ugrid;
    bool item_may_long, user_may_long;
    bool sgl;
};

static void chunk_pass_args(slk_ctx *ctx, const train_plan &p, const train_call &c, size_t ck, const slk_prep_bufs &pb, slk_pass_args *args) {
    slk_pass_args &a = *args;
    const slk_tables *tables = c.tables;
    const slk_optim *optim = c.optim;
    memset(&a, 0, sizeof(a));
    for (int t = 0; t < 4; ++t) {
        a.P[t] = tables->d_param[t];
        a.S1[t] = p.dense ? f32p(ctx->dgrad[t]) : optim->d_state1[t];
        a.S2[t] = optim->d_state2[t];
    }
    if (p.shadowed) {
        a.P[3] = f32p(ctx->bias_shadow);
        a.S1[3] = f32p(ctx->bias_shadow) + 1;
        a.bsh3 = 1u;
    }
    if (p.pingpong) {
        a.P0alt = f32p(ctx->pp_alt);
        a.uflag = (uint8_t *)ctx->pp_flags.p;
    }
    a.D = p.D;
    a.NP = p.NP;
    a.ukey = u32p(pb.ukey[1]);
    a.umask = (uint32_t)((1ull << p.ubits) - 1);
    a.uit = p.pre ? u32p(pb.uit) : u32p(pb.uval[1]);
    a.uk = p.pre ? u32p(pb.uval[1]) : nullptr;
    a.gk = f32p(ctx->gk);
    a.sk = f32p(ctx->sk);
    a.snap = f32p(ctx->snap);
    a.RS = p.RS;
    a.gsn = f32p(ctx->extra[BL_GSN]);
    a.ikey = u32p(pb.ikey[1]);
    a.imask = (uint32_t)((1ull << p.ibits) - 1);
    a.ipay = u32p(pb.ipay[1]);
    a.loss_partial = (double *)ctx->losspart.p;
    a.loss_kind = c.loss;
    a.pad_item = a.pad_item2 = 0xffffffffu;
    a.ub = p.ubd;
    a.ib = p.ibd;
    a.urec = f32p(ctx->extra[BL_UREC]);
    a.RSU = p.RSU;
    a.ubz = (tables->flags & SLK_TABLES_USER_BIAS_ZERO) && (c.loss == SLK_LOSS_BPR || c.loss == SLK_LOSS_HINGE) && !p.bloom &&
            (optim->kind == SLK_OPT_ADAGRAD || optim->kind == SLK_OPT_SGD) && ctx->opt_user_bias_zero_hint;
    a.nt = ctx->opt_nt;
    if (p.fused) a.ratings = c.ratings + chunk_begin(p, ck);
}

static int sort_live_list(slk_ctx *ctx, const train_plan &p, const minibatch &mb, bool hashed, hipStream_t s) {
    const uint32_t n = 2 * mb.bm * (hashed ? (uint32_t)p.Hi : 1u);
    hipLaunchKernelGGL(k_build_live_keys, dim3(slk_grid_for(ctx, n, 256)), dim3(256), 0, s, (const uint32_t *)ctx->extra[BL_LIVE].p,
                       mb.a.uit, 2 * mb.bm, p.ibd, hashed, u32p(ctx->extra[BL_LK0]), u32p(ctx->extra[BL_LV0]));
    SLK_LAUNCH_CHECK(ctx, hashed ? "k_build_live_keys<hashed>" : "k_build_live_keys");
    return slk_sort_pairs_u32_u32_in(ctx, ctx->extra[BL_LATE_SORT], u32p(ctx->extra[BL_LK0]), u32p(ctx->extra[BL_LK1]),
                                     u32p(ctx->extra[BL_LV0]), u32p(ctx->extra[BL_LV1]), n, (hashed ? p.icbits : p.ibits) + 1, s,
                                     true);
}

static int score_stage(slk_ctx *ctx, const train_plan &p, const train_call &c, const train_kernels &k, size_t ck, const slk_prep_bufs &pb, minibatch &mb, hipStream_t s) {
    slk_pass_args &a = mb.a;
    int rc;
    a.n_loss_partial = (int)mb.ugrid;
    if (!p.pre || p.fused) return SLK_OK;
    slk_prof_begin(ctx, SLK_K_SCORE, s);
    hipLaunchKernelGGL(k.spass, dim3(mb.ugrid), dim3(256), 0, s, a);
    SLK_LAUNCH_CHECK(ctx, "k_score_pass");
    const unsigned sgrid = slk_grid_for(ctx, mb.bm, 256);
    if (p.expl) {
        hipLaunchKernelGGL(k_explicit_loss, dim3(sgrid), dim3(256), 0, s, (const float *)ctx->sk.p, c.ratings + chunk_begin(p, ck),
                           f32p(ctx->gk), mb.b0, mb.bm, (int)c.loss, a.inv_b, (double *)ctx->losspart.p);
        SLK_LAUNCH_CHECK(ctx, "k_explicit_loss");
    } else {
        hipLaunchKernelGGL(k_adaptive_select<0>, dim3(sgrid), dim3(256), 0, s, (const float *)ctx->sk.p, f32p(ctx->gk), mb.b0, mb.bm,
                           p.nn, a.inv_b, (double *)ctx->losspart.p, p.late ? (const uint32_t *)pb.ipay[0].p : (const uint32_t *)nullptr,
                           p.late ? u32p(ctx->extra[BL_LIVE]) : (uint32_t *)nullptr);
        SLK_LAUNCH_CHECK(ctx, "k_adaptive_select");
    }
    a.n_loss_partial = (int)sgrid;
    slk_prof_end(ctx, s);
    if (p.late) {
        slk_prof_begin(ctx, SLK_K_PREP, s);
        if ((rc = sort_live_list(ctx, p, mb, false, s))) return rc;
        slk_prof_end(ctx, s);
        a.ikey = u32p(ctx->extra[BL_LK1]);
        a.ipay = u32p(ctx->extra[BL_LV1]);
        a.imask = 0xffffffffu;
        a.ibegin = 0;
        a.iend = 2 * mb.bm;
    }
    return SLK_OK;
}

static int user_stage(slk_ctx *ctx, const train_plan &p, const train_kernels &k, const slk_prep_bufs &pb, minibatch &mb, hipStream_t s) {
    slk_pass_args &a = mb.a;
    slk_prof_begin(ctx, SLK_K_USER_PASS, s);
    const bool lat = k.upass_lat && (int64_t)mb.bm <= ctx->opt_user_lat_max_batch;
    const bool sgl = mb.sgl = p.sgl_on && k.upass_sgl && !mb.user_may_long && !lat;
    if (sgl) {
        a.mflag = (const uint8_t *)pb.mflag.p;
        a.msorted = (const uint8_t *)pb.msorted.p;
        ++ctx->stat_single;
    }
    const pass_fn uform = sgl ? k.upass_sgl : (mb.user_may_long ? (lat ? k.upass_lat_long : k.upass_long) : (lat ? k.upass_lat : k.upass));
    unsigned ugrid_form = mb.ugrid;
    if (ctx->opt_user_grid_own_occ || sgl) {
        const int occ_form = sgl ? k.occ_sgl : slk_occupancy_of(ctx, uform);
        ugrid_form = slk_grid_for(ctx, mb.bm, k.gpb, mb.ugm < occ_form ? mb.ugm : occ_form);
        if (!p.pre || p.fused) a.n_loss_partial = (int)ugrid_form;
    }
    if (mb.user_may_long) {
        if (ctx->upart_gen >= 0x0ffffffeu) {
            SLK_HIP(ctx, hipMemsetAsync(ctx->upart_meta.p, 0, ctx->upart_meta.cap, s));
            ctx->upart_gen = 0u;
        }
        ++ctx->upart_gen;
        a.upart = f32p(ctx->extra[BL_UPART]);
        a.upart_meta = u32p(ctx->upart_meta);
        a.upart_count = a.upart_meta + 4 * p.utiles;
        a.upart_gen = ctx->upart_gen;
        a.UPS = p.UPS;
        SLK_HIP(ctx, hipMemsetAsync(a.upart_count, 0, 4, s));
        hipLaunchKernelGGL(uform, dim3(ugrid_form), dim3(256), 0, s, a);
        SLK_LAUNCH_CHECK(ctx, "k_user_pass<ULONG>");
        ++ctx->stat_user_long;
        hipLaunchKernelGGL(k.ustitch, dim3(slk_grid_for(ctx, ((size_t)mb.bm + SLK_USER_TILE - 1) / SLK_USER_TILE, k.gpb)), dim3(256), 0, s, a);
        SLK_LAUNCH_CHECK(ctx, "k_user_stitch");
    } else {
        hipLaunchKernelGGL(uform, dim3(ugrid_form), dim3(256), 0, s, a);
        SLK_LAUNCH_CHECK(ctx, "k_user_pass");
    }
    slk_prof_end(ctx, s);
    return SLK_OK;
}

static int item_stage(slk_ctx *ctx, const train_plan &p, const train_call &c, const train_kernels &k, const slk_prep_bufs &pb, minibatch &mb, hipStream_t s) {
    slk_pass_args &a = mb.a;
    const int Hi = p.Hi, Hu = p.Hu, g = p.g;
    int rc;
    slk_prof_begin(ctx, SLK_K_ITEM_PASS, s);
    if (!Hi) {
        if ((rc = slk_launch_item_pass(ctx, mb.sgl ? k.ipass_sgl : k.ipass, a, g, s, "k_item_pass", mb.item_may_long))) return rc;
    } else {
        if ((rc = slk_launch_item_pass(ctx, k.ipass_bias, a, g, s, "k_item_pass<BIAS>", mb.item_may_long))) return rc;
        slk_pass_args r = a;
        r.mb_loss_out = nullptr;
        r.ikey = u32p(pb.bik[1]);
        r.ipay = u32p(pb.bip[1]);
        r.ibegin = a.ibegin * (uint32_t)Hi;
        r.iend = a.iend * (uint32_t)Hi;
        r.imask = (uint32_t)((1ull << p.icbits) - 1);
        if (p.late) {
            if ((rc = sort_live_list(ctx, p, mb, true, s))) return rc;
            r.ikey = u32p(ctx->extra[BL_LK1]);
            r.ipay = u32p(ctx->extra[BL_LV1]);
            r.ibegin = 0;
            r.iend = 2 * mb.bm * (uint32_t)Hi;
            r.imask = 0xffffffffu;
        }
        r.pad_item = c.tables->item_bloom->skip_row < 0 ? 0xffffffffu : (uint32_t)c.tables->item_bloom->skip_row;
        if ((rc = slk_launch_item_pass(ctx, k.ipass_rows, r, g, s, "k_item_pass<ROWS>"))) return rc;
    }
    if (Hu) {
        slk_pass_args r = a;
        r.mb_loss_out = nullptr;
        r.P[1] = a.P[0];
        r.S1[1] = a.S1[0];
        r.S2[1] = a.S2[0];
        r.snap = a.urec;
        r.RS = p.RSU;
        r.ikey = u32p(pb.buk[1]);
        r.ipay = u32p(pb.bup[1]);
        r.ibegin = mb.b0 * (uint32_t)Hu;
        r.iend = mb.b1 * (uint32_t)Hu;
        r.imask = (uint32_t)((1ull << p.ucbits) - 1);
        r.pad_item = c.tables->user_bloom->skip_row < 0 ? 0xffffffffu : (uint32_t)c.tables->user_bloom->skip_row;
        r.pad_item2 = p.ubd.rows;
        if ((rc = slk_launch_item_pass(ctx, k.rpass_rows, r, g, s, "k_item_pass<ROW,ROWS>"))) return rc;
    }
    slk_prof_end(ctx, s);
    return SLK_OK;
}

static int run_passes(slk_ctx *ctx, const train_plan &p, const train_call &c, const train_kernels &k, train_run &run, size_t ck, slk_prep_bufs &pb, hipStream_t s) {
    int rc;
    const uint32_t nc = chunk_len(p, c, ck), bsz = (uint32_t)p.bsz;
    const uint32_t n_mb_c = (nc + bsz - 1) / bsz;
    slk_pass_args chunk_args;
    chunk_pass_args(ctx, p, c, ck, pb, &chunk_args);
    const int ugm = p.side && ctx->opt_user_grid_mult > 6 ? 6 : ctx->opt_user_grid_mult;
    minibatch mb;
    mb.ugm = ugm;
    for (uint32_t b0 = 0; b0 < nc; b0 += bsz, ++run.mb_global) {
        const uint32_t b1 = (nc - b0 < bsz) ? nc : b0 + bsz, bm = b1 - b0;
        mb.b0 = b0, mb.b1 = b1, mb.bm = bm;
        slk_pass_args &a = mb.a = chunk_args;
        a.begin = b0;
        a.end = b1;
        a.ibegin = b0 * (uint32_t)p.NP;
        a.iend = b1 * (uint32_t)p.NP;
        a.inv_b = 1.0f / (float)bm;
        a.mb_loss_out = c.mb_loss + run.mb_global;
        slk_set_opt_coeffs(a, c.optim);
        if (ctx->opt_record_nt_min_bytes > 0 && (int64_t)bm * p.RS * 4 >= ctx->opt_record_nt_min_bytes) a.nt |= 16;
        mb.ugrid = slk_grid_for(ctx, bm, k.gpb, ugm < k.occ_user ? ugm : k.occ_user);
        if ((rc = score_stage(ctx, p, c, k, ck, pb, mb, s))) return rc;

        if (b0 == 0 && pb.ev_lflags && pb.h_lflags_n) SLK_HIP(ctx, hipEventSynchronize(pb.ev_lflags));
        const uint32_t mb_c = b0 / bsz;
        const bool have_flags = pb.h_lflags_n >= 2 * (size_t)n_mb_c;
        mb.item_may_long = p.late || !ctx->opt_item_long_gate || !have_flags || pb.h_lflags[mb_c] != 0;
        mb.user_may_long = !p.bloom && (!ctx->opt_item_long_gate || !have_flags || pb.h_lflags[n_mb_c + mb_c] != 0);

        if ((rc = user_stage(ctx, p, k, pb, mb, s))) return rc;
        if ((rc = item_stage(ctx, p, c, k, pb, mb, s))) return rc;
        if (p.dense && (rc = slk_dense_sweeps(ctx, c.tables->d_param, c.optim, 15u, s))) return rc;
        c.optim->step += 1;
    }
    return SLK_OK;
}

static int run_chunk(slk_ctx *ctx, const train_plan &p, const train_call &c, const train_kernels &k, train_run &run, size_t ck, slk_prep_bufs &pb, hipStream_t s) {
    if (!run.epoch_route) return run_passes(ctx, p, c, k, run, ck, pb, s);
    const int64_t c0 = chunk_begin(p, ck);
    const uint32_t nc = chunk_len(p, c, ck);
    int rc = slk_epoch_run_chunk(ctx, c.tables, c.optim, pb, nc, p.bsz, p.ubits, p.ibits, (int)c.loss, p.NP, p.RS, f32p(ctx->snap),
                                 f32p(ctx->extra[BL_GSN]), c.mb_loss + run.mb_global, p.expl ? c.ratings + c0 : nullptr, s);
    if (rc == SLK_EAGAIN_EPOCH) {
        run.epoch_route = false;
        if (p.dense && (rc = ensure_dense_buffers(ctx, p, s))) return rc;
        return run_passes(ctx, p, c, k, run, ck, pb, s);
    }
    run.mb_global += (nc + p.bsz - 1) / p.bsz;
    return rc;
}

static int prefetch_first_chunk(slk_ctx *ctx, const train_plan &p, const train_call &c, train_run &run) {
    int rc;
    hipStream_t s = c.s;
    ctx->pf.valid = false;
    if (!p.side || run.epoch_route || c.neg_in) return SLK_OK;
    if ((rc = slk_prep_stream_init(ctx))) return rc;
    hipStream_t ps = ctx->prep_stream;
    const int set = ctx->last_pipe_set >= 0 ? (ctx->last_pipe_set ^ 1) : 0;
    if (ctx->opt_overlap_prep != 1 || ctx->opt_prefetch_wait || ctx->last_pipe_set < 0) {
        SLK_HIP(ctx, hipEventRecord(ctx->ev_start, s));
        SLK_HIP(ctx, hipStreamWaitEvent(ps, ctx->ev_start, 0));
    } else if (ctx->sampled_valid && ctx->ev_sampled) {
        SLK_HIP(ctx, hipStreamWaitEvent(ps, ctx->ev_sampled, 0));
    }
    SLK_HIP(ctx, hipStreamWaitEvent(ps, ctx->ev_done[set], 0));
    if (p.one_draw) {
        if ((rc = slk_ensure(ctx, ctx->pf_neg, (size_t)c.n * p.nn * 4))) return rc;
        if ((rc = slk_sample_u32(ctx, c.tables->num_items, c.n * (int64_t)p.nn, u32p(ctx->pf_neg), nullptr, ps))) return rc;
        run.neg_all = u32p(ctx->pf_neg);
    } else if ((rc = prep_sample(ctx, p, c, run, 0, ctx->pb[set], ps))) {
        return rc;
    }
    if (ctx->opt_overlap_prep == 1 && (rc = prep_sort(ctx, p, c, run, 0, ctx->pb[set], ps))) return rc;
    SLK_HIP(ctx, hipEventRecord(ctx->ev_prep[set], ps));
    ctx->pf = {true, set, c.users, c.items, c.n, p.bsz, (int64_t)p.nc_max, (int)c.loss, p.nn, p.one_draw, p.sgl_on};
    return SLK_OK;
}

static int run_inline(slk_ctx *ctx, const train_plan &p, const train_call &c, const train_kernels &k, train_run &run) {
    int rc;
    if ((rc = prep_sample(ctx, p, c, run, 0, ctx->pb[0], c.s))) return rc;
    if ((rc = prep_sort(ctx, p, c, run, 0, ctx->pb[0], c.s))) return rc;
    if ((rc = run_chunk(ctx, p, c, k, run, 0, ctx->pb[0], c.s))) return rc;
    ctx->last_stream = c.s;
    ctx->last_pipe_set = -1;
    return SLK_OK;
}

static int run_pipelined(slk_ctx *ctx, const train_plan &p, const train_call &c, const train_kernels &k, train_run &run, bool have0) {
    int rc;
    hipStream_t s = c.s;
    const bool side = p.side;
    const bool sort_ahead = !side || ctx->opt_overlap_prep == 1;
    if (side && (rc = slk_prep_stream_init(ctx))) return rc;
    hipStream_t ps = side ? ctx->prep_stream : s;
    if (side) {
        SLK_HIP(ctx, hipEventRecord(ctx->ev_start, s));
        SLK_HIP(ctx, hipStreamWaitEvent(ps, ctx->ev_start, 0));
    }
    int set = have0 ? ctx->pf.set : 0;
    if (have0) ++ctx->stat_prefetched;
    if (have0 && ctx->pf.all) run.neg_all = u32p(ctx->pf_neg);
    const bool flags0 = have0 && sort_ahead && p.sgl_on && !ctx->pf.sgl_on;
    if (!have0) {
        if (p.one_draw) {
            if ((rc = slk_ensure(ctx, ctx->call_neg, (size_t)c.n * p.nn * 4))) return rc;
            if ((rc = slk_sample_u32(ctx, c.tables->num_items, c.n * (int64_t)p.nn, u32p(ctx->call_neg), c.neg_out, ps))) return rc;
            run.neg_all = u32p(ctx->call_neg);
        } else if ((rc = prep_sample(ctx, p, c, run, 0, ctx->pb[set], ps))) {
            return rc;
        }
        if (sort_ahead && (rc = prep_sort(ctx, p, c, run, 0, ctx->pb[set], ps))) return rc;
        if (side) SLK_HIP(ctx, hipEventRecord(ctx->ev_prep[set], ps));
    }
    for (size_t ck = 0; ck < p.n_chunks; ++ck, set ^= 1) {
        if (side) SLK_HIP(ctx, hipStreamWaitEvent(s, ctx->ev_prep[set], 0));
        if (ck == 0 && flags0) {
            slk_prof_begin(ctx, SLK_K_PREP, s);
            if ((rc = prep_single_flags(ctx, p, c, ctx->pb[set], 0, s))) return rc;
            slk_prof_end(ctx, s);
        }
        if (ck == 0 && have0 && run.neg_all && c.neg_out) {
            const size_t nneg = (size_t)c.n * p.nn;
            hipLaunchKernelGGL(k_u32_to_i64, dim3(slk_grid_for(ctx, nneg, 256)), dim3(256), 0, s, run.neg_all, c.neg_out, nneg);
            SLK_LAUNCH_CHECK(ctx, "k_u32_to_i64");
        }
        if (!sort_ahead && (rc = prep_sort(ctx, p, c, run, ck, ctx->pb[set], s))) return rc;
        if (ck + 1 < p.n_chunks) {
            if (side && (ck > 0 || have0)) SLK_HIP(ctx, hipStreamWaitEvent(ps, ctx->ev_done[set ^ 1], 0));
            if (!sort_ahead) {
                SLK_HIP(ctx, hipEventRecord(ctx->ev_start, s));
                SLK_HIP(ctx, hipStreamWaitEvent(ps, ctx->ev_start, 0));
            }
            if ((rc = prep_sample(ctx, p, c, run, ck + 1, ctx->pb[set ^ 1], ps))) return rc;
            if (sort_ahead && (rc = prep_sort(ctx, p, c, run, ck + 1, ctx->pb[set ^ 1], ps))) return rc;
            if (side) {
                SLK_HIP(ctx, hipEventRecord(ctx->ev_prep[set ^ 1], ps));
                ++ctx->stat_overlapped;
            }
        }
        if ((rc = run_chunk(ctx, p, c, k, run, ck, ctx->pb[set], s))) return rc;
        if (side) SLK_HIP(ctx, hipEventRecord(ctx->ev_done[set], s));
    }
    ctx->last_pipe_set = side ? (set ^ 1) : -1;
    ctx->last_stream = s;
    return SLK_OK;
}

static int run_training(slk_ctx *ctx, const train_call &c) {
    if (!ctx) return SLK_EINVAL;
    train_plan p;
    int rc;
    if ((rc = plan_training(ctx, c, &p))) return rc;
    if (p.n_chunks == 0) return SLK_OK;
    const bool training = c.mode == train_call::TRAIN;
    if (p.shadowed && training) ++ctx->stat_shadowed;
    if (p.pingpong && training) ++ctx->stat_pingpong;
    if ((rc = ensure_scratch(ctx, p, c.s))) return rc;
    if (c.mode == train_call::RESERVE) return reserve_extras(ctx, p, c);
    train_kernels k;
    pick_kernels(ctx, p, c.optim, &k);
    train_run run = {nullptr, 0, p.epoch_route};
    if (!training) return prefetch_first_chunk(ctx, p, c, run);

    if (ctx->pf.valid && (c.neg_in || p.expl)) ctx->pf.valid = false;
    const bool have0 = ctx->pf.valid;
    ctx->pf.valid = false;
    if (have0 && (!p.side || p.epoch_route || ctx->pf.users != (const void *)c.users || ctx->pf.items != (const void *)c.items ||
                  ctx->pf.n != c.n || ctx->pf.bsz != p.bsz || ctx->pf.loss != (int)c.loss || ctx->pf.nn != p.nn ||
                  ctx->pf.nc0 != (int64_t)p.nc_max || c.neg_in))
        return slk_fail(ctx, SLK_EINVAL, "slk_bilinear_train: a chunk was prepared ahead (slk_bilinear_prefetch) for another call; its "
                                         "draws are consumed -- set the RNG state again");
    return p.nsets == 1 ? run_inline(ctx, p, c, k, run) : run_pipelined(ctx, p, c, k, run, have0);
}

__global__ __launch_bounds__(256) void k_bias_shadow_pack(const float *p, const float *s1, float2 *sh, size_t n) {
    for (size_t i = (size_t)blockIdx.x * 256 + threadIdx.x; i < n; i += (size_t)gridDim.x * 256) sh[i] = make_float2(p[i], s1[i]);
}

__global__ __launch_bounds__(256) void k_bias_shadow_unpack(const float2 *sh, float *p, float *s1, size_t n) {
    for (size_t i = (size_t)blockIdx.x * 256 + threadIdx.x; i < n; i += (size_t)gridDim.x * 256) {
        const float2 v = sh[i];
        p[i] = v.x;
        s1[i] = v.y;
    }
}

SLK_EXPORT int slk_bias_shadow_begin(slk_ctx *ctx, const slk_tables *tables, const slk_optim *optim, void *stream) {
    if (!ctx || !tables || !optim) return SLK_EINVAL;
    SLK_HIP(ctx, hipSetDevice(ctx->device));
    if (ctx->shadow_active) return slk_fail(ctx, SLK_EINVAL, "slk_bias_shadow_begin: a shadow is already active on this ctx");
    if (optim->kind != SLK_OPT_ADAGRAD || !tables->d_param[3] || !optim->d_state1[3] || tables->item_bloom || tables->num_items < 1)
        return slk_fail(ctx, SLK_EINVAL, "slk_bias_shadow_begin: row-sparse Adagrad over a plain item table only");
    hipStream_t s = (hipStream_t)stream;
    int rc;
    if ((rc = slk_ensure(ctx, ctx->bias_shadow, (size_t)tables->num_items * 8))) return rc;
    hipLaunchKernelGGL(k_bias_shadow_pack, dim3(slk_grid_for(ctx, (size_t)tables->num_items, 256)), dim3(256), 0, s,
                       (const float *)tables->d_param[3], (const float *)optim->d_state1[3], (float2 *)ctx->bias_shadow.p,
                       (size_t)tables->num_items);
    SLK_LAUNCH_CHECK(ctx, "k_bias_shadow_pack");
    ctx->shadow_src_p = tables->d_param[3];
    ctx->shadow_src_s = optim->d_state1[3];
    ctx->shadow_rows = tables->num_items;
    ctx->shadow_active = true;
    ctx->last_stream = s;
    return SLK_OK;
}

SLK_EXPORT int slk_bias_shadow_end(slk_ctx *ctx, void *stream) {
    if (!ctx) return SLK_EINVAL;
    if (!ctx->shadow_active) return SLK_OK;
    float *const dst_p = ctx->shadow_src_p, *const dst_s = ctx->shadow_src_s;
    const int64_t rows = ctx->shadow_rows;
    ctx->shadow_active = false;
    ctx->shadow_src_p = ctx->shadow_src_s = nullptr;
    SLK_HIP(ctx, hipSetDevice(ctx->device));
    hipStream_t s = (hipStream_t)stream;
    hipLaunchKernelGGL(k_bias_shadow_unpack, dim3(slk_grid_for(ctx, (size_t)rows, 256)), dim3(256), 0, s,
                       (const float2 *)ctx->bias_shadow.p, dst_p, dst_s, (size_t)rows);
    SLK_LAUNCH_CHECK(ctx, "k_bias_shadow_unpack");
    ctx->last_stream = s;
    return SLK_OK;
}

SLK_EXPORT int slk_bias_shadow_abort(slk_ctx *ctx) {
    if (!ctx) return SLK_EINVAL;
    ctx->shadow_active = false;
    ctx->shadow_src_p = ctx->shadow_src_s = nullptr;
    return SLK_OK;
}

__global__ __launch_bounds__(256) void k_pingpong_merge(float *P0, const float *alt, const uint8_t *flag, size_t rows, int D) {
    if (D % 4 == 0) {
        const size_t per = (size_t)D / 4, n = rows * per;
        for (size_t e = (size_t)blockIdx.x * 256 + threadIdx.x; e < n; e += (size_t)gridDim.x * 256)
            if (flag[e / per]) reinterpret_cast<float4 *>(P0)[e] = reinterpret_cast<const float4 *>(alt)[e];
    } else {
        const size_t n = rows * (size_t)D;
        for (size_t e = (size_t)blockIdx.x * 256 + threadIdx.x; e < n; e += (size_t)gridDim.x * 256)
            if (flag[e / (size_t)D]) P0[e] = alt[e];
    }
}

SLK_EXPORT int slk_user_pingpong_begin(slk_ctx *ctx, const slk_tables *tables, const slk_optim *optim, void *stream) {
    if (!ctx) return SLK_EINVAL;
    if (!tables || !optim) return slk_fail(ctx, SLK_EINVAL, "slk_user_pingpong_begin: NULL tables / optim");
    if (ctx->pp_active) return slk_fail(ctx, SLK_EINVAL, "slk_user_pingpong_begin: a ping-pong is already active on this ctx");
    if (tables->user_bloom || tables->item_bloom || !tables->d_param[0] ||
        (optim->kind != SLK_OPT_ADAGRAD && optim->kind != SLK_OPT_SPARSE_ADAM && optim->kind != SLK_OPT_SGD))
        return slk_fail(ctx, SLK_EINVAL, "slk_user_pingpong_begin: plain tables and a row-sparse optimizer (Adagrad, SparseAdam, SGD) only");
    int vec, g, rc;
    if ((rc = slk_check_tables(ctx, tables, 15u, &vec, &g, true))) return rc;
    SLK_HIP(ctx, hipSetDevice(ctx->device));
    hipStream_t s = (hipStream_t)stream;
    const size_t rows = (size_t)tables->num_users;
    if ((rc = slk_ensure(ctx, ctx->pp_alt, rows * (size_t)tables->dim * 4))) return rc;
    if ((rc = slk_ensure(ctx, ctx->pp_flags, (rows + 15) / 16 * 16))) return rc;
    SLK_HIP(ctx, hipMemsetAsync(ctx->pp_flags.p, 0, (rows + 15) / 16 * 16, s));
    ctx->pp_src_u = tables->d_param[0];
    ctx->pp_rows = tables->num_users;
    ctx->pp_dim = tables->dim;
    ctx->pp_active = true;
    ctx->last_stream = s;
    return SLK_OK;
}

SLK_EXPORT int slk_user_pingpong_end(slk_ctx *ctx, void *stream) {
    if (!ctx) return SLK_EINVAL;
    if (!ctx->pp_active) return SLK_OK;
    float *const dst = ctx->pp_src_u;
    const int64_t rows = ctx->pp_rows;
    const int D = ctx->pp_dim;
    ctx->pp_active = false;
    ctx->pp_src_u = nullptr;
    SLK_HIP(ctx, hipSetDevice(ctx->device));
    hipStream_t s = (hipStream_t)stream;
    hipLaunchKernelGGL(k_pingpong_merge, dim3(slk_grid_for(ctx, (size_t)rows * (size_t)((D + 3) / 4), 256)), dim3(256), 0, s, dst,
                       (const float *)ctx->pp_alt.p, (const uint8_t *)ctx->pp_flags.p, (size_t)rows, D);
    SLK_LAUNCH_CHECK(ctx, "k_pingpong_merge");
    ctx->last_stream = s;
    return SLK_OK;
}

SLK_EXPORT int slk_user_pingpong_abort(slk_ctx *ctx) {
    if (!ctx) return SLK_EINVAL;
    ctx->pp_active = false;
    ctx->pp_src_u = nullptr;
    return SLK_OK;
}
```

spotlight_amd/csrc/slk_common.h:

```cpp
#pragma once
#include <hip/hip_runtime.h>
#include <stdint.h>
#include <stdio.h>
#include <string.h>

#include <vector>

#include "../../include/spotlight_hip.h"

#define SLK_EAGAIN_EPOCH 1
#define SLK_EXPORT extern "C" __attribute__((visibility("default")))

#if defined(__HIPCC__)
#define SLK_WAVES_PER_EU(n) __attribute__((amdgpu_waves_per_eu(n, n)))
#define SLK_WAVES_PER_EU_RANGE(lo, hi) __attribute__((amdgpu_waves_per_eu(lo, hi)))
#else
#define SLK_WAVES_PER_EU(n)
#define SLK_WAVES_PER_EU_RANGE(lo, hi)
#endif

#if defined(__HIPCC__)
#define SLK_DRAIN_VMEM() asm volatile("s_waitcnt vmcnt(0)" ::: "memory")
#else
#define SLK_DRAIN_VMEM() ((void)0)
#endif

#if defined(__HIPCC__)
#define SLK_WAVE_SYNC()                                          \
    do {                                                         \
        __builtin_amdgcn_fence(__ATOMIC_RELEASE, "wavefront");   \
        __builtin_amdgcn_wave_barrier();                         \
        __builtin_amdgcn_fence(__ATOMIC_ACQUIRE, "wavefront");   \
    } while (0)
#else
#define SLK_WAVE_SYNC() __syncthreads()
#endif

#if defined(__HIPCC__)
#define SLK_SUBWAVE_SYNC() SLK_WAVE_SYNC()
#else
#define SLK_SUBWAVE_SYNC() ((void)__shfl(0, 0))
#endif

#if defined(__HIPCC__)
#define SLK_RESIDENT_GRID_LAUNCH() ((void)0)
#else
#define SLK_RESIDENT_GRID_LAUNCH() ::emu::next_launch_resident()
#endif

struct slk_buf {
    void *p = nullptr;
    size_t cap = 0;
};

struct slk_rng_dev {
    uint32_t key[624];
    int32_t pos;
    int32_t insufficient;
    unsigned long long t_last;
    unsigned long long accepted;
    int32_t epoch_abort;
    int32_t sort_abort;
};

#define SLK_EXTRA_BUFS 56

enum slk_extra_slot {
    SH_OKEY0 = 0, SH_OKEY1, SH_OVAL0, SH_OVAL1, SH_VSLOT, SH_HIST, SH_SEGSTART, SH_UNITBASE, SH_MBOFF, SH_RID, SH_SEGTAB, SH_GSLOT,
    SH_UIT = 48, SH_GPOS,
    BL_UREC = 16, BL_LIVE, BL_LK0, BL_LK1, BL_LV0, BL_LV1, BL_GSN, BL_UPART, BL_LATE_SORT = 38,
    TS_T0 = 26, TS_T1, TS_T2, TS_T3, TS_T4, TS_SMALL, TS_SORT, TS_USERS, TS_ITEMS, TS_HEADS, TS_ROWOFF,
    FY_B0 = TS_T0, FY_B1, FY_B2, FY_B3, FY_B4, FY_SMALL, FY_SORT,
    SQ_MCOUNT = 12, SQ_REP, SQ_BIK0, SQ_BIK1,
    SQ_BIP0 = BL_UREC, SQ_BIP1,
    SQ_GSN = BL_UPART,
    SQ_MCOUNT_B = TS_T4,
    EM_SORT = TS_SORT,
    EM_KEY0 = 40, EM_KEY1, EM_PAY0, EM_PAY1, EM_HEADS, EM_PART0, EM_PART1,
    EP_COEF = EM_KEY0, EP_BAR, EP_PARTIAL, EP_TOUCH,
    EV_REP = 24, EV_RBIAS, EV_ST = 37, EV_CNT = 39, EV_TOPK = 50, EV_TOPK_FLAG,
    SLK_EXTRA_END
};
static_assert(SLK_EXTRA_END <= SLK_EXTRA_BUFS, "slk_ctx::extra holds every slot of slk_extra_slot");

struct slk_prep_bufs {
    slk_buf neg32, ukey[2], uval[2], uit, ikey[2], ipay[2];
    slk_buf bik[2], bip[2], buk[2], bup[2];
    slk_buf mflag, msorted;
    slk_buf lflags;
    int *h_lflags = nullptr;
    size_t h_lflags_cap = 0;
    size_t h_lflags_n = 0;
    hipEvent_t ev_lflags = nullptr;
};

struct slk_prof_span {
    int cls;
    hipEvent_t a, b;
};

struct slk_ctx {
    int device = 0;
    int num_cus = 256;
    size_t lds_per_block = (size_t)160 * 1024;
    size_t lds_per_cu = (size_t)160 * 1024;
    char err[512] = {0};
    hipStream_t last_stream = nullptr;
    slk_rng_dev *d_rng = nullptr;
    uint32_t *d_jump[2] = {nullptr, nullptr};
    bool mt_attr_set = false;
    slk_buf bias_shadow;
    float *shadow_src_p = nullptr, *shadow_src_s = nullptr;
    int64_t shadow_rows = 0;
    bool shadow_active = false;
    slk_buf pp_alt, pp_flags;
    float *pp_src_u = nullptr;
    int64_t pp_rows = 0;
    int pp_dim = 0;
    bool pp_active = false;
    slk_buf mt_tmp;

    slk_buf raw, cnt, neg32, ukey[2], uval[2], uit, ikey[2], ipay[2], gk, sk, snap, losspart,
        sort_tmp, dgrad[4], ipart, ipart_meta, upart_meta;
    size_t dgrad_elems[4] = {0, 0, 0, 0};
    int64_t opt_chunk_interactions = (int64_t)1 << 23;
    int opt_overlap_prep = 0;
    int64_t opt_mt_long_min_blocks = 16385;
    int opt_prefetch_wait = 0;
    int64_t opt_overlap_min_batch = (int64_t)1 << 16;
    int64_t opt_sort_big_min = (int64_t)1 << 20;
    int opt_sort_debug = 0;
    int opt_item_grid_mult = 128;
    int opt_user_grid_mult = 8;
    int opt_seq_variant = 1;
    int64_t opt_adaptive_late_min_batch = (int64_t)1 << 18;
    int64_t opt_user_lat_max_batch = (int64_t)1 << 17;
    int64_t opt_item_lat_max_tiles = 2048;
    int opt_item_long_gate = 1;
    int opt_explicit_fused = 1;
    int opt_epoch_kernel = 1;
    int64_t opt_epoch_max_batch = 1024;
    bool epoch_refused = false;
    int opt_epoch_adaptive = 1;
    int64_t opt_epoch_adaptive_max_batch = 1024;
    int epoch_bars_per_mb = 2;
    int opt_epoch_barrier = -1;
    int opt_epoch_cooperative = 0;
    int opt_epoch_debug = 0;
    int opt_epoch_max_grid = 256;
    int64_t opt_epoch_dense_elems = (int64_t)1 << 18;
    void *h_coef[2] = {nullptr, nullptr};
    size_t h_coef_cap[2] = {0, 0};
    hipEvent_t ev_coef[2] = {nullptr, nullptr};
    int coef_flip = 0;
    int opt_nt = 3;
    int64_t opt_item_single_min_items = (int64_t)1 << 24;
    int opt_user_grid_own_occ = 0;
    int64_t opt_topk_items_per_wg = 0;
    int64_t opt_eval_items_per_wg = 0;
    int64_t opt_foldin_wg_min_len = 0;
    int opt_user_bias_zero_hint = 1;
    int64_t opt_record_nt_min_bytes = (int64_t)192 << 20;
    slk_prep_bufs pb[2];
    hipStream_t prep_stream = nullptr;
    bool prep_warmed = false;
    hipEvent_t ev_sampled = nullptr;
    bool sampled_valid = false;
    hipStream_t copy_stream = nullptr;
    hipEvent_t ev_start = nullptr, ev_prep[2] = {nullptr, nullptr}, ev_done[2] = {nullptr, nullptr};
    slk_buf extra[SLK_EXTRA_BUFS];
    int64_t shard_n = -1;
    int64_t sh_n = 0;
    int sh_M = 0, sh_S = 0, sh_world = 0;
    int sh_NP = 2;
    bool sh_adaptive = false;
    unsigned sh_ubits = 0;
    std::vector<int64_t> sh_ustart, sh_rstart;
    std::vector<int64_t> sh_sslots, sh_rslots;
    std::vector<uint64_t> sh_host, sh_host2;

    int64_t ts_rows = -1, ts_nseg = 0;
    int ts_L = 0, ts_step = 0;

    int64_t em_occ = -1, em_rows = 0, em_segments = -1;
    int em_dim = 0;

    struct {
        bool valid = false;
        int set = 0;
        const void *users = nullptr, *items = nullptr;
        int64_t n = 0, bsz = 0, nc0 = 0;
        int loss = 0, nn = 0;
        bool all = false;
        bool sgl_on = false;
    } pf;
    slk_buf pf_neg;
    slk_buf call_neg;
    int64_t stat_overlapped = 0;
    int64_t stat_prefetched = 0;
    int64_t stat_shadowed = 0;
    int64_t stat_pingpong = 0;
    int64_t stat_single = 0;
    int last_pipe_set = -1;
    uint32_t ipart_gen = 0;
    uint32_t upart_gen = 0;
    int64_t stat_user_long = 0, stat_item_long = 0;
    int fy_sweeps = 0;
    int fy_fallbacks = 0;
    int opt_shuffle_band = 1;

    bool prof_on = false;
    std::vector<slk_prof_span> spans;
    std::vector<hipEvent_t> ev_pool;
    std::vector<std::pair<const void *, int>> occ_cache;
    int64_t prof_launches[SLK_K_COUNT] = {0};
    double prof_ms[SLK_K_COUNT] = {0};
};

int slk_fail(slk_ctx *ctx, int code, const char *fmt, ...);
int slk_ensure(slk_ctx *ctx, slk_buf &b, size_t bytes);
int slk_ensure_lflags_host(slk_ctx *ctx, slk_prep_bufs &pb, size_t n);
void slk_prof_begin(slk_ctx *ctx, int cls, hipStream_t s);
void slk_prof_end(slk_ctx *ctx, hipStream_t s);
int slk_prof_drain(slk_ctx *ctx);
int slk_prep_stream_init(slk_ctx *ctx);
hipStream_t slk_copy_stream(slk_ctx *ctx);

#define SLK_HIP(ctx, call)                                                                   \
    do {                                                                                     \
        hipError_t e_ = (call);                                                              \
        if (e_ != hipSuccess)                                                                \
            return slk_fail((ctx), SLK_EIO, "%s failed: %s (%s:%d)", #call, hipGetErrorString(e_), \
                            __FILE__, __LINE__);                                             \
    } while (0)

#define SLK_LAUNCH_CHECK(ctx, what)                                                          \
    do {                                                                                     \
        hipError_t e_ = hipGetLastError();                                                   \
        if (e_ != hipSuccess)                                                                \
            return slk_fail((ctx), SLK_EIO, "launch of %s failed: %s", (what), hipGetErrorString(e_)); \
    } while (0)

struct slk_call {
    slk_ctx *const ctx;
    const hipStream_t s;
    bool open = false;
    slk_call(slk_ctx *c, void *stream) : ctx(c), s((hipStream_t)stream) {}
    slk_call(const slk_call &) = delete;
    int begin(int cls) {
        SLK_HIP(ctx, hipSetDevice(ctx->device));
        ctx->last_stream = s;
        slk_prof_begin(ctx, cls, s);
        open = true;
        return SLK_OK;
    }
    ~slk_call() {
        if (open) slk_prof_end(ctx, s);
    }
};

#define SLK_MT_JUMP_BLOCKS 64
#define SLK_MT_JUMP_LEVELS 2
static inline int slk_mt_jump_blocks(int level) { return level ? 4 * SLK_MT_JUMP_BLOCKS : SLK_MT_JUMP_BLOCKS; }
#define SLK_MT_JUMP_WG 256
static_assert(SLK_MT_JUMP_WG * SLK_MT_JUMP_BLOCKS + 1 == 16385, "slk_ctx::opt_mt_long_min_blocks");
#define SLK_MT_JUMP_TERMS 10752
#define SLK_MT_JUMP_PAD (33 * 624 - 1)
const uint32_t *slk_mt_jump_table(slk_ctx *ctx, int level);

int slk_sample_u32(slk_ctx *ctx, int64_t num_items, int64_t count, uint32_t *d_out32, int64_t *d_out64,
                   hipStream_t s);

int slk_sort_pairs_u32_u32(slk_ctx *ctx, const uint32_t *kin, uint32_t *kout, const uint32_t *vin,
                           uint32_t *vout, size_t n, unsigned end_bit, hipStream_t s, bool clobber = false);
int slk_sort_pairs_u32_u32_in(slk_ctx *ctx, slk_buf &scratch, const uint32_t *kin, uint32_t *kout, const uint32_t *vin,
                              uint32_t *vout, size_t n, unsigned end_bit, hipStream_t s, bool clobber = false);
int slk_sort_pairs_u64_u32_in(slk_ctx *ctx, slk_buf &scratch, const uint64_t *kin, uint64_t *kout, const uint32_t *vin,
                              uint32_t *vout, size_t n, unsigned end_bit, hipStream_t s, bool clobber = false);
int slk_sort_pairs_u32_u64(slk_ctx *ctx, const uint32_t *kin, uint32_t *kout, const uint64_t *vin,
                           uint64_t *vout, size_t n, unsigned end_bit, hipStream_t s, bool clobber = false);
int slk_sort_fy_steps(slk_ctx *ctx, slk_buf &scratch, const uint32_t *J, uint32_t n, uint32_t *const key[2], uint32_t *const val[2],
                      hipStream_t s);
int slk_sort_pairs_any(slk_ctx *ctx, int kind, const void *kin, void *kout, const void *vin, void *vout, size_t n, size_t seg_len,
                       unsigned bits, hipStream_t s, bool clobber);
int slk_sort_user_fat(slk_ctx *ctx, const int64_t *users, const int64_t *items, const uint32_t *neg32, size_t nc, size_t bsz,
                      unsigned ubits, unsigned mbbits, uint32_t *const key[2], uint64_t *const val[2], hipStream_t s);
int slk_sort_user_idx(slk_ctx *ctx, const int64_t *users, size_t nc, size_t bsz, unsigned ubits, unsigned mbbits,
                      uint32_t *const key[2], uint32_t *const val[2], hipStream_t s);
int slk_sort_item_occ(slk_ctx *ctx, const uint32_t *uit, size_t nocc, size_t bsz, int NP, unsigned ibits, unsigned mbbits,
                      uint32_t *const key[2], uint32_t *const val[2], hipStream_t s);

int slk_eval_predict_all(slk_ctx *ctx, const slk_tables *tables, const float *rep, const float *rbias, const int64_t *gmap,
                         float *d_out, hipStream_t s);
int slk_eval_user_rep(slk_ctx *ctx, const slk_tables *tables, int vec, int g, const int64_t *d_user, const float **rep,
                      const float **rbias, const int64_t **gmap, hipStream_t s);

int slk_check_tables(slk_ctx *ctx, const slk_tables *t, unsigned table_mask, int *vec, int *g, bool shadow_ok = false,
                     bool pingpong_ok = false);
int slk_launch_i64_to_u32(slk_ctx *ctx, const int64_t *in, uint32_t *out, size_t n, hipStream_t s);

int slk_sort_reserve(slk_ctx *ctx, size_t n);
int slk_compact_heads(slk_ctx *ctx, const uint32_t *d_sorted, uint32_t n, uint32_t *d_heads, uint32_t *d_segid,
                      uint32_t *nseg_out, hipStream_t s);
bool slk_epoch_eligible(const slk_ctx *ctx, const slk_tables *tables, const slk_optim *optim, int64_t bsz, int loss, bool bloom);
int slk_epoch_reserve(slk_ctx *ctx, const slk_tables *tables, const slk_optim *optim, uint32_t n_mb, int64_t bsz, int loss, int NP);
int slk_epoch_run_chunk(slk_ctx *ctx, const slk_tables *tables, slk_optim *optim, const slk_prep_bufs &pb, uint32_t nc,
                        int64_t bsz, unsigned ubits, unsigned ibits, int loss, int NP, int RS, float *snap, float *gsn,
                        float *d_mb_loss, const float *d_ratings, hipStream_t s);
int slk_mt_generate_blocks(slk_ctx *ctx, unsigned long long nblocks, hipStream_t s);
int slk_sample_reserve(slk_ctx *ctx, int64_t num_items, int64_t count);
int slk_mt_jump_reserve(slk_ctx *ctx, int level);
int slk_mt_level_for(const slk_ctx *ctx, unsigned long long nblocks);
int slk_rng_write_state(slk_ctx *ctx, const uint32_t *h_key, int32_t pos);

static inline unsigned slk_bits_for(uint64_t max_value) {
    unsigned b = 1;
    while (b < 64 && (max_value >> b)) ++b;
    return b;
}


template <int G>
__device__ __forceinline__ float slk_group_sum(float x) {
#pragma unroll
    for (int m = G / 2; m >= 1; m >>= 1) x += __shfl_xor(x, m, G);
    return x;
}

template <int G>
__device__ __forceinline__ unsigned long long slk_group_or(unsigned long long x) {
#pragma unroll
    for (int m = G / 2; m >= 1; m >>= 1) x |= __shfl_xor(x, m, G);
    return x;
}

template <int VEC>
struct slk_vec {
    float v[VEC];
};

template <int VEC>
__device__ __forceinline__ slk_vec<VEC> slk_vzero() {
    slk_vec<VEC> r;
#pragma unroll
    for (int i = 0; i < VEC; ++i) r.v[i] = 0.0f;
    return r;
}

template <int VEC>
__device__ __forceinline__ slk_vec<VEC> slk_vload(const float *p);
template <>
__device__ __forceinline__ slk_vec<4> slk_vload<4>(const float *p) {
    const float4 t = *reinterpret_cast<const float4 *>(p);
    slk_vec<4> r;
    r.v[0] = t.x; r.v[1] = t.y; r.v[2] = t.z; r.v[3] = t.w;
    return r;
}
template <>
__device__ __forceinline__ slk_vec<1> slk_vload<1>(const float *p) {
    slk_vec<1> r;
    r.v[0] = *p;
    return r;
}

template <int VEC>
__device__ __forceinline__ void slk_vstore(float *p, const slk_vec<VEC> &x);
template <>
__device__ __forceinline__ void slk_vstore<4>(float *p, const slk_vec<4> &x) {
    *reinterpret_cast<float4 *>(p) = make_float4(x.v[0], x.v[1], x.v[2], x.v[3]);
}
template <>
__device__ __forceinline__ void slk_vstore<1>(float *p, const slk_vec<1> &x) {
    *p = x.v[0];
}

#ifdef SLK_NT_FIXED
#define SLK_NT_OF(a) (SLK_NT_FIXED)
#else
#define SLK_NT_OF(a) ((a).nt)
#endif

template <int VEC>
__device__ __forceinline__ slk_vec<VEC> slk_vload_nt(const float *p) {
#if defined(__HIPCC__)
    slk_vec<VEC> r;
    if (VEC == 4) {
        typedef float slk_f4 __attribute__((ext_vector_type(4)));
        const slk_f4 t = __builtin_nontemporal_load(reinterpret_cast<const slk_f4 *>(p));
        r.v[0] = t.x; r.v[1 % VEC] = t.y; r.v[2 % VEC] = t.z; r.v[3 % VEC] = t.w;
    } else {
#pragma unroll
        for (int i = 0; i < VEC; ++i) r.v[i] = __builtin_nontemporal_load(p + i);
    }
    return r;
#else
    return slk_vload<VEC>(p);
#endif
}
template <int VEC>
__device__ __forceinline__ void slk_vstore_nt(float *p, const slk_vec<VEC> &x) {
#if defined(__HIPCC__)
    if (VEC == 4) {
        typedef float slk_f4 __attribute__((ext_vector_type(4)));
        slk_f4 t;
        t.x = x.v[0]; t.y = x.v[1 % VEC]; t.z = x.v[2 % VEC]; t.w = x.v[3 % VEC];
        __builtin_nontemporal_store(t, reinterpret_cast<slk_f4 *>(p));
    } else {
#pragma unroll
        for (int i = 0; i < VEC; ++i) __builtin_nontemporal_store(x.v[i], p + i);
    }
#else
    slk_vstore<VEC>(p, x);
#endif
}
__device__ __forceinline__ uint32_t slk_ld_u32(const uint32_t *p, bool nt) {
#if defined(__HIPCC__)
    return nt ? __builtin_nontemporal_load(p) : *p;
#else
    return *p;
#endif
}
template <int VEC>
__device__ __forceinline__ slk_vec<VEC> slk_vload_if_nt(const float *p, bool nt) {
    return nt ? slk_vload_nt<VEC>(p) : slk_vload<VEC>(p);
}
template <int VEC>
__device__ __forceinline__ void slk_vstore_if_nt(float *p, const slk_vec<VEC> &x, bool nt) {
    if (nt) slk_vstore_nt<VEC>(p, x);
    else slk_vstore<VEC>(p, x);
}

__device__ __forceinline__ float slk_ld_coh(const float *p) {
    const uint32_t b = __hip_atomic_load(reinterpret_cast<const uint32_t *>(p), __ATOMIC_RELAXED, __HIP_MEMORY_SCOPE_AGENT);
    float f;
    memcpy(&f, &b, 4);
    return f;
}
__device__ __forceinline__ void slk_st_coh(float *p, float x) {
    uint32_t b;
    memcpy(&b, &x, 4);
    __hip_atomic_store(reinterpret_cast<uint32_t *>(p), b, __ATOMIC_RELAXED, __HIP_MEMORY_SCOPE_AGENT);
}
template <int VEC>
__device__ __forceinline__ slk_vec<VEC> slk_vload_coh(const float *p) {
    slk_vec<VEC> r;
    if (VEC == 4) {
        const unsigned long long *q = reinterpret_cast<const unsigned long long *>(p);
        const unsigned long long lo = __hip_atomic_load(q, __ATOMIC_RELAXED, __HIP_MEMORY_SCOPE_AGENT);
        const unsigned long long hi = __hip_atomic_load(q + 1, __ATOMIC_RELAXED, __HIP_MEMORY_SCOPE_AGENT);
        const uint32_t w[4] = {(uint32_t)lo, (uint32_t)(lo >> 32), (uint32_t)hi, (uint32_t)(hi >> 32)};
#pragma unroll
        for (int i = 0; i < VEC; ++i) memcpy(&r.v[i], &w[i % 4], 4);
    } else {
#pragma unroll
        for (int i = 0; i < VEC; ++i) r.v[i] = slk_ld_coh(p + i);
    }
    return r;
}
template <int VEC>
__device__ __forceinline__ void slk_vstore_coh(float *p, const slk_vec<VEC> &x) {
    if (VEC == 4) {
        uint32_t w[4];
#pragma unroll
        for (int i = 0; i < 4; ++i) memcpy(&w[i], &x.v[i % VEC], 4);
        unsigned long long *q = reinterpret_cast<unsigned long long *>(p);
        __hip_atomic_store(q, (unsigned long long)w[0] | ((unsigned long long)w[1] << 32), __ATOMIC_RELAXED,
                           __HIP_MEMORY_SCOPE_AGENT);
        __hip_atomic_store(q + 1, (unsigned long long)w[2] | ((unsigned long long)w[3] << 32), __ATOMIC_RELAXED,
                           __HIP_MEMORY_SCOPE_AGENT);
    } else {
#pragma unroll
        for (int i = 0; i < VEC; ++i) slk_st_coh(p + i, x.v[i]);
    }
}

template <int VEC>
__device__ __forceinline__ float slk_vdot(const slk_vec<VEC> &a, const slk_vec<VEC> &b) {
    float s = 0.0f;
#pragma unroll
    for (int i = 0; i < VEC; ++i) s += a.v[i] * b.v[i];
    return s;
}

template <int VEC>
__device__ __forceinline__ void slk_vaxpy(slk_vec<VEC> &acc, float g, const slk_vec<VEC> &x) {
#pragma unroll
    for (int i = 0; i < VEC; ++i) acc.v[i] += g * x.v[i];
}

__device__ __forceinline__ double slk_block_sum_256(double x, double *red ) {
    const int t = threadIdx.x;
    red[t] = x;
    __syncthreads();
    for (int off = 128; off >= 1; off >>= 1) {
        if (t < off) red[t] += red[t + off];
        __syncthreads();
    }
    return red[0];
}
```

spotlight_amd/csrc/slk_sort.hip:

```cpp
#include "slk_common.h"

namespace {

constexpr int RS_RB = 8;
constexpr int RS_RADIX = 1 << RS_RB;
constexpr uint32_t RS_VAL_MASK = (1u << 30) - 1u;
constexpr uint32_t RS_AGG = 1u, RS_INC = 2u;
constexpr int RS_MAX_PASS = 8;
constexpr int RS_HIST_KEYS = 8192;
constexpr int RS_LBW = 16;
constexpr uint32_t RS_MAX_SPINS = 1u << 22;

enum { RS_LOAD_PLAIN = 0, RS_LOAD_USER_FAT, RS_LOAD_USER_IDX, RS_LOAD_ITEM_OCC, RS_LOAD_FY_STEPS };

struct rs_args {
    const void *kin, *vin;
    void *kout, *vout;
    const int64_t *users, *items;
    const uint32_t *neg32, *uit;
    uint32_t n, seg_len, tps, ntiles, hbps;
    uint32_t kseg;
    unsigned idbits;
    uint32_t fy_n;
    int npass, pass;
    int shift[RS_MAX_PASS], width[RS_MAX_PASS];
    uint32_t *hist, *base;
    uint32_t *ticket;
    uint32_t *status;
    int32_t *abort_flag;
    int xcd;
    uint32_t nseg;
    int debug;
};

template <class KeyT>
__device__ __forceinline__ uint32_t rs_digit(KeyT k, int shift, uint32_t mask) {
    return (uint32_t)(k >> shift) & mask;
}

template <class KeyT, class ValT, int LOADER>
__device__ __forceinline__ void rs_load(const rs_args &a, uint32_t gi, uint32_t seg, KeyT &k, ValT &v) {
    if (LOADER == RS_LOAD_FY_STEPS) {
        const uint32_t i = a.fy_n - 1u - gi, j = a.uit[gi];
        k = (KeyT)(j == i ? a.fy_n : j);
        v = (ValT)i;
        return;
    }
    if (LOADER != RS_LOAD_PLAIN && a.kseg) seg = gi / a.kseg;
    if (LOADER == RS_LOAD_PLAIN) {
        k = ((const KeyT *)a.kin)[gi];
        v = ((const ValT *)a.vin)[gi];
    } else if (LOADER == RS_LOAD_USER_FAT) {
        k = (KeyT)((seg << a.idbits) | (uint32_t)a.users[gi]);
        v = (ValT)(((uint64_t)a.neg32[gi] << 32) | (uint64_t)(uint32_t)a.items[gi]);
    } else if (LOADER == RS_LOAD_USER_IDX) {
        k = (KeyT)((seg << a.idbits) | (uint32_t)a.users[gi]);
        v = (ValT)gi;
    } else {
        k = (KeyT)((seg << a.idbits) | a.uit[gi]);
        v = (ValT)gi;
    }
}

template <class KeyT, int LOADER>
__device__ __forceinline__ KeyT rs_load_key(const rs_args &a, uint32_t gi, uint32_t seg) {
    if (LOADER == RS_LOAD_PLAIN) return ((const KeyT *)a.kin)[gi];
    if (LOADER == RS_LOAD_FY_STEPS) {
        const uint32_t j = a.uit[gi];
        return (KeyT)(j == a.fy_n - 1u - gi ? a.fy_n : j);
    }
    if (a.kseg) seg = gi / a.kseg;
    if (LOADER == RS_LOAD_ITEM_OCC) return (KeyT)((seg << a.idbits) | a.uit[gi]);
    return (KeyT)((seg << a.idbits) | (uint32_t)a.users[gi]);
}

template <class KeyT, int LOADER>
__global__ __launch_bounds__(256) void k_rs_hist(rs_args a) {
    __shared__ uint32_t sh[RS_MAX_PASS * RS_RADIX];
    const uint32_t seg = blockIdx.x / a.hbps, hb = blockIdx.x - seg * a.hbps;
    const uint32_t s0 = seg * a.seg_len;
    const uint32_t s1 = (a.n - s0 < a.seg_len) ? a.n : s0 + a.seg_len;
    const uint32_t b0 = s0 + hb * (uint32_t)RS_HIST_KEYS;
    const uint32_t b1 = (b0 >= s1 || s1 - b0 < (uint32_t)RS_HIST_KEYS) ? s1 : b0 + (uint32_t)RS_HIST_KEYS;
    for (int i = threadIdx.x; i < a.npass * RS_RADIX; i += 256) sh[i] = 0u;
    __syncthreads();
    for (uint32_t g0 = b0 + threadIdx.x; g0 < b1; g0 += 8u * 256u) {
        KeyT k[8];
#pragma unroll
        for (int u = 0; u < 8; ++u) {
            const uint32_t gi = g0 + (uint32_t)u * 256u;
            k[u] = gi < b1 ? rs_load_key<KeyT, LOADER>(a, gi, seg) : (KeyT)0;
        }
#pragma unroll
        for (int u = 0; u < 8; ++u) {
            if (g0 + (uint32_t)u * 256u >= b1) continue;
            for (int p = 0; p < a.npass; ++p)
                atomicAdd(&sh[p * RS_RADIX + rs_digit<KeyT>(k[u], a.shift[p], (1u << a.width[p]) - 1u)], 1u);
        }
    }
    __syncthreads();
    uint32_t *gh = a.hist + (size_t)seg * a.npass * RS_RADIX;
    for (int i = threadIdx.x; i < a.npass * RS_RADIX; i += 256) {
        const uint32_t c = sh[i];
        if (c) atomicAdd(&gh[i], c);
    }
}

template <int THREADS>
__device__ __forceinline__ uint32_t rs_block_excl_scan(uint32_t v, uint32_t *s_wsum) {
    const int lane = threadIdx.x & 63, w = threadIdx.x >> 6;
    uint32_t inc = v;
#pragma unroll
    for (int o = 1; o < 64; o <<= 1) {
        const uint32_t t = __shfl_up(inc, o);
        if (lane >= o) inc += t;
    }
    if (lane == 63) s_wsum[w] = inc;
    __syncthreads();
    uint32_t off = 0;
    for (int i = 0; i < THREADS / 64; ++i)
        if (i < w) off += s_wsum[i];
    __syncthreads();
    return off + inc - v;
}

__global__ __launch_bounds__(256) void k_rs_scan(rs_args a) {
    __shared__ uint32_t s_wsum[4];
    const uint32_t seg = blockIdx.x / (uint32_t)a.npass;
    const size_t o = (size_t)blockIdx.x * RS_RADIX + threadIdx.x;
    const uint32_t c = a.hist[o];
    a.base[o] = seg * a.seg_len + rs_block_excl_scan<256>(c, s_wsum);
}

__device__ __forceinline__ uint32_t rs_xcc_id() {
#if defined(__HIPCC__)
    return (uint32_t)__builtin_amdgcn_s_getreg((3 << 11) | 20) & 7u;
#else
    return blockIdx.x & 7u;
#endif
}

__device__ __forceinline__ unsigned long long rs_match(uint32_t d, int nbits, bool valid) {
    unsigned long long m = __ballot(valid);
    for (int b = 0; b < nbits; ++b) {
        const bool bit = (d >> b) & 1u;
        const unsigned long long bal = __ballot(bit);
        m &= bit ? bal : ~bal;
    }
    return valid ? m : 0ull;
}

__device__ __forceinline__ bool rs_walk(const rs_args &a, const uint32_t *row0, uint32_t radix, uint32_t tis, uint32_t &before) {
    int32_t t = (int32_t)tis - 1;
    uint32_t spins = 0;
    bool done = false;
    while (!done) {
        uint32_t v[RS_LBW];
#pragma unroll
        for (int i = 0; i < RS_LBW; ++i) {
            const int32_t ti = t - i;
            v[i] = ti >= 0 ? __hip_atomic_load(row0 + (size_t)ti * radix, __ATOMIC_RELAXED, __HIP_MEMORY_SCOPE_AGENT) : 0u;
        }
        int consumed = 0;
#pragma unroll
        for (int i = 0; i < RS_LBW; ++i) {
            const uint32_t f = v[i] >> 30;
            if (done || f == 0u || consumed != i) continue;
            before += v[i] & RS_VAL_MASK;
            ++consumed;
            if (f == RS_INC) done = true;
        }
        t -= consumed;
        if (!done && consumed == 0) {
            if (++spins > RS_MAX_SPINS) {
                *a.abort_flag = 1;
                return false;
            }
            __builtin_amdgcn_s_sleep(1);
        }
    }
    return true;
}

template <class KeyT, class ValT, int THREADS, int KPT, int LOADER, bool SINGLE>
__global__ __launch_bounds__(THREADS) SLK_WAVES_PER_EU_RANGE(4, 6) void k_rs_scatter(rs_args a) {
    constexpr int WAVES = THREADS / 64, KW = WAVES, TILE = KW * 64 * KPT;
    constexpr int OPT = (TILE + THREADS - 1) / THREADS;
    constexpr int XB = sizeof(KeyT) > sizeof(ValT) ? sizeof(KeyT) : sizeof(ValT);
    __shared__ uint32_t s_cnt[KW * RS_RADIX];
    __shared__ uint32_t s_lbase[RS_RADIX];
    __shared__ uint32_t s_goff[RS_RADIX];
    __shared__ uint32_t s_wsum[WAVES];
    __shared__ uint32_t s_tile;
    __shared__ __attribute__((aligned(16))) unsigned char s_x[(size_t)TILE * XB];

    const int lane = threadIdx.x & 63, wave = threadIdx.x >> 6;
    constexpr bool is_key = true;
    const int shift = a.shift[a.pass], nbits = a.width[a.pass];
    const uint32_t radix = 1u << nbits, dmask = radix - 1u;
    if (!SINGLE && threadIdx.x == 0) {
        if (a.xcd) {
            const uint32_t x0 = rs_xcc_id();
            uint32_t t = 0xffffffffu;
            for (uint32_t i = 0; i < 8u && t == 0xffffffffu; ++i) {
                const uint32_t x = (x0 + i) & 7u;
                const uint32_t nsx = a.nseg > x ? (a.nseg - x + 7u) / 8u : 0u;
                if (!nsx) continue;
                const uint32_t k = atomicAdd(a.ticket + 8 + a.pass * 8 + x, 1u);
                if (k < nsx * a.tps) t = (x + 8u * (k / a.tps)) * a.tps + k % a.tps;
            }
            s_tile = t;
        } else {
            s_tile = atomicAdd(a.ticket + a.pass, 1u);
        }
    }
    for (int i = threadIdx.x; i < KW * RS_RADIX; i += THREADS) s_cnt[i] = 0u;
    if (threadIdx.x < RS_RADIX) s_lbase[threadIdx.x] = 0u;
    __syncthreads();
    const uint32_t tile = SINGLE ? 0u : s_tile;
    if (tile == 0xffffffffu) return;
    const uint32_t seg = tile / a.tps, tis = tile - seg * a.tps;
    const uint32_t s0 = seg * a.seg_len;
    const uint32_t s1 = (a.n - s0 < a.seg_len) ? a.n : s0 + a.seg_len;
    const uint32_t t0 = s0 + tis * (uint32_t)TILE;
    const uint32_t cnt = t0 >= s1 ? 0u : ((s1 - t0 < (uint32_t)TILE) ? s1 - t0 : (uint32_t)TILE);

    KeyT key[KPT];
    ValT val[KPT];
    uint32_t pos2[KPT / 2];
    const uint32_t e0 = (uint32_t)wave * 64u * KPT + (uint32_t)lane;
    if (is_key) {
        if (LOADER == RS_LOAD_PLAIN) {
#pragma unroll
            for (int j = 0; j < KPT; ++j) {
                const uint32_t e = e0 + (uint32_t)j * 64u;
                key[j] = e < cnt ? ((const KeyT *)a.kin)[t0 + e] : (KeyT)0;
            }
#pragma unroll
            for (int j = 0; j < KPT; ++j) {
                const uint32_t e = e0 + (uint32_t)j * 64u;
                val[j] = e < cnt ? ((const ValT *)a.vin)[t0 + e] : (ValT)0;
            }
        } else {
#pragma unroll
            for (int j = 0; j < KPT; ++j) {
                const uint32_t e = e0 + (uint32_t)j * 64u;
                key[j] = 0;
                val[j] = 0;
                if (e < cnt) rs_load<KeyT, ValT, LOADER>(a, t0 + e, seg, key[j], val[j]);
            }
        }
        if (!SINGLE) {
#pragma unroll
            for (int j = 0; j < KPT; ++j)
                if (e0 + (uint32_t)j * 64u < cnt) atomicAdd(&s_lbase[rs_digit<KeyT>(key[j], shift, dmask)], 1u);
        }
    } else {
#pragma unroll
        for (int j = 0; j < KPT; ++j) {
            key[j] = 0;
            val[j] = 0;
        }
    }
    if (!SINGLE) __syncthreads();

    uint32_t tcount = 0, before = 0;
    uint32_t *wcnt = s_cnt + (is_key ? wave : 0) * RS_RADIX;
    auto rank_keys = [&]() {
#pragma unroll
        for (int j = 0; j < KPT; ++j) {
            if ((j & 1) == 0) pos2[j / 2] = 0u;
            if ((uint32_t)wave * 64u * KPT + (uint32_t)j * 64u >= cnt) continue;
            const bool valid = e0 + (uint32_t)j * 64u < cnt;
            const uint32_t dj = rs_digit<KeyT>(key[j], shift, dmask);
            uint32_t r;
            if (a.debug & 2) {
                r = valid ? atomicAdd(&wcnt[dj], 1u) : 0u;
            } else {
                const unsigned long long m = rs_match(dj, nbits, valid);
                const int leader = m ? __ffsll((long long)m) - 1 : lane;
                uint32_t first = 0;
                if (m && lane == leader) first = atomicAdd(&wcnt[dj], (uint32_t)__popcll(m));
                first = __shfl(first, leader);
                r = first + (uint32_t)__popcll(m & ((1ull << lane) - 1ull));
            }
            pos2[j / 2] = (j & 1) ? (pos2[j / 2] | (r << 16)) : r;
        }
    };
    {
        const uint32_t d = threadIdx.x;
        if (!SINGLE && d < radix) {
            tcount = s_lbase[d];
            __hip_atomic_store(a.status + (size_t)tile * radix + d, ((tis == 0 ? RS_INC : RS_AGG) << 30) | tcount, __ATOMIC_RELAXED,
                               __HIP_MEMORY_SCOPE_AGENT);
            if (tis != 0 && !(a.debug & 1)) {
                rs_walk(a, a.status + (size_t)(tile - tis) * radix + d, radix, tis, before);
                __hip_atomic_store(a.status + (size_t)tile * radix + d, (RS_INC << 30) | ((before + tcount) & RS_VAL_MASK), __ATOMIC_RELAXED,
                                   __HIP_MEMORY_SCOPE_AGENT);
            }
        }
        rank_keys();
        __syncthreads();
        if (d < radix) {
            uint32_t run = 0;
            for (int w = 0; w < KW; ++w) {
                const uint32_t c = s_cnt[w * RS_RADIX + d];
                s_cnt[w * RS_RADIX + d] = run;
                run += c;
            }
            if (SINGLE) tcount = run;
        }
        const uint32_t lb = rs_block_excl_scan<THREADS>(tcount, s_wsum);
        if (d < radix) {
            uint32_t gbase = lb;
            if (!SINGLE) gbase = a.base[((size_t)seg * a.npass + a.pass) * RS_RADIX + d];
            s_lbase[d] = lb;
            s_goff[d] = gbase + before - lb;
        }
    }
    __syncthreads();
    KeyT *xk = reinterpret_cast<KeyT *>(s_x);
    if (is_key) {
#pragma unroll
        for (int j = 0; j < KPT; ++j) {
            if (e0 + (uint32_t)j * 64u < cnt) {
                const uint32_t dj = rs_digit<KeyT>(key[j], shift, dmask);
                const uint32_t pj = ((pos2[j / 2] >> ((j & 1) * 16)) & 0xffffu) + s_lbase[dj] + wcnt[dj];
                pos2[j / 2] = (j & 1) ? ((pos2[j / 2] & 0xffffu) | (pj << 16)) : ((pos2[j / 2] & 0xffff0000u) | pj);
                xk[pj] = key[j];
            }
        }
    }
    __syncthreads();
    uint32_t gidx[OPT];
#pragma unroll
    for (int j = 0; j < OPT; ++j) {
        const uint32_t i = (uint32_t)j * THREADS + threadIdx.x;
        gidx[j] = 0;
        if (i < cnt) {
            const KeyT k = xk[i];
            gidx[j] = s_goff[rs_digit<KeyT>(k, shift, dmask)] + i;
            ((KeyT *)a.kout)[gidx[j]] = k;
        }
    }
    __syncthreads();
    ValT *xv = reinterpret_cast<ValT *>(s_x);
    if (is_key) {
#pragma unroll
        for (int j = 0; j < KPT; ++j)
            if (e0 + (uint32_t)j * 64u < cnt) xv[(pos2[j / 2] >> ((j & 1) * 16)) & 0xffffu] = val[j];
    }
    __syncthreads();
#pragma unroll
    for (int j = 0; j < OPT; ++j) {
        const uint32_t i = (uint32_t)j * THREADS + threadIdx.x;
        if (i < cnt) ((ValT *)a.vout)[gidx[j]] = xv[i];
    }
}

struct rs_plan {
    uint32_t n = 0, seg_len = 0, nseg = 0, tps = 0, ntiles = 0, hbps = 0;
    int npass = 0, shift[RS_MAX_PASS], width[RS_MAX_PASS];
    size_t off_ticket = 0, off_status[RS_MAX_PASS], zero_bytes = 0, off_base = 0, off_data = 0, ctl_bytes = 0;
};

static void rs_split_bits(unsigned bits, int *npass, int *shift, int *width) {
    int P = (int)((bits + RS_RB - 1) / RS_RB);
    if (P < 1) P = 1;
    const int lo = (int)bits / P, rem = (int)bits % P;
    int s = 0;
    for (int p = 0; p < P; ++p) {
        width[p] = lo + (p < rem ? 1 : 0);
        if (width[p] < 1) width[p] = 1;
        shift[p] = s;
        s += width[p];
    }
    *npass = P;
}

static void rs_make_plan(rs_plan &pl, size_t n, size_t seg_len, unsigned bits, unsigned tile) {
    pl.n = (uint32_t)n;
    pl.seg_len = (uint32_t)(seg_len && seg_len < n ? seg_len : n);
    pl.nseg = (uint32_t)((n + pl.seg_len - 1) / pl.seg_len);
    pl.tps = (pl.seg_len + tile - 1) / tile;
    pl.ntiles = pl.nseg * pl.tps;
    pl.hbps = (pl.seg_len + RS_HIST_KEYS - 1) / RS_HIST_KEYS;
    rs_split_bits(bits, &pl.npass, pl.shift, pl.width);
    size_t o = (size_t)pl.nseg * pl.npass * RS_RADIX * 4;
    pl.off_ticket = o;
    o += 512;
    for (int p = 0; p < pl.npass; ++p) {
        pl.off_status[p] = o;
        o += (size_t)pl.ntiles * ((size_t)1 << pl.width[p]) * 4;
    }
    pl.zero_bytes = o;
    o = (o + 255) & ~(size_t)255;
    pl.off_base = o;
    o += (size_t)pl.nseg * pl.npass * RS_RADIX * 4;
    pl.off_data = (o + 255) & ~(size_t)255;
    pl.ctl_bytes = pl.off_data;
}

#ifndef RS_BIG_THREADS
#define RS_BIG_THREADS 512
#endif
#ifndef RS_BIG_KPT
#define RS_BIG_KPT 16
#endif

template <class KeyT, class ValT, int LOADER>
struct rs_kernels {
    static void launch(int cfg, bool single, unsigned grid, hipStream_t s, const rs_args &a) {
        if (single)
            hipLaunchKernelGGL((k_rs_scatter<KeyT, ValT, 256, 16, RS_LOAD_PLAIN, true>), dim3(1), dim3(256), 0, s, a);
        else if (cfg == 1)
            hipLaunchKernelGGL((k_rs_scatter<KeyT, ValT, RS_BIG_THREADS, RS_BIG_KPT, LOADER, false>), dim3(grid), dim3(RS_BIG_THREADS), 0, s, a);
        else
            hipLaunchKernelGGL((k_rs_scatter<KeyT, ValT, 256, 16, LOADER, false>), dim3(grid), dim3(256), 0, s, a);
    }
};

static inline unsigned rs_tile_of(int cfg) { return cfg == 1 ? (unsigned)(RS_BIG_THREADS * RS_BIG_KPT) : 4096u; }

template <class KeyT, class ValT, int LOADER>
static int rs_sort(slk_ctx *ctx, slk_buf &scratch, rs_args a, size_t n, size_t seg_len, unsigned bits, void *kalt, void *valt,
                   hipStream_t s) {
    if (n == 0) return SLK_OK;
    if (n >= ((size_t)1 << 31)) return slk_fail(ctx, SLK_EINVAL, "sort of %zu pairs: at most 2^31 - 1", n);
    if (bits > 8 * sizeof(KeyT)) bits = 8 * sizeof(KeyT);
    if (bits < 1) bits = 1;
    const bool single = LOADER == RS_LOAD_PLAIN && n <= 4096 && (seg_len == 0 || seg_len >= n);
    const int cfg = (!single && n >= (size_t)ctx->opt_sort_big_min) ? 1 : 0;
    const unsigned tile = rs_tile_of(cfg);
    rs_plan pl;
    rs_make_plan(pl, n, single ? 0 : seg_len, bits, tile);
    if (pl.seg_len >= (1u << 30)) return slk_fail(ctx, SLK_EINVAL, "sort segment of %u pairs: at most 2^30 - 1", pl.seg_len);
    const bool inplace0 = kalt && kalt == a.kin && (pl.npass & 1) == 0;
    const bool need_tmp = pl.npass > 1 && (!kalt || inplace0);
    const size_t koff = pl.off_data, voff = (koff + n * sizeof(KeyT) + 255) & ~(size_t)255;
    int rc = slk_ensure(ctx, scratch, need_tmp ? voff + n * sizeof(ValT) : pl.ctl_bytes);
    if (rc) return rc;
    char *base = (char *)scratch.p;
    void *k0dst = nullptr, *v0dst = nullptr;
    if (need_tmp && !kalt) {
        kalt = base + koff;
        valt = base + voff;
    } else if (inplace0) {
        k0dst = base + koff;
        v0dst = base + voff;
    }
    a.n = pl.n;
    a.seg_len = pl.seg_len;
    a.tps = pl.tps;
    a.ntiles = pl.ntiles;
    a.hbps = pl.hbps;
    a.npass = pl.npass;
    for (int p = 0; p < pl.npass; ++p) {
        a.shift[p] = pl.shift[p];
        a.width[p] = pl.width[p];
    }
    a.hist = (uint32_t *)base;
    a.base = (uint32_t *)(base + pl.off_base);
    a.ticket = (uint32_t *)(base + pl.off_ticket);
    a.abort_flag = &ctx->d_rng->sort_abort;
    a.debug = ctx->opt_sort_debug;
    a.nseg = pl.nseg;
    a.xcd = pl.nseg >= 2 ? 1 : 0;
    void *kfinal = a.kout, *vfinal = a.vout;
    if (!single) {
        SLK_HIP(ctx, hipMemsetAsync(base, 0, pl.zero_bytes, s));
        a.pass = 0;
        hipLaunchKernelGGL((k_rs_hist<KeyT, LOADER>), dim3(pl.nseg * pl.hbps), dim3(256), 0, s, a);
        SLK_LAUNCH_CHECK(ctx, "k_rs_hist");
        hipLaunchKernelGGL(k_rs_scan, dim3(pl.nseg * (unsigned)pl.npass), dim3(256), 0, s, a);
        SLK_LAUNCH_CHECK(ctx, "k_rs_scan");
    }
    for (int p = 0; p < pl.npass; ++p) {
        const bool to_final = ((pl.npass - 1 - p) & 1) == 0;
        a.pass = p;
        a.kout = to_final ? kfinal : kalt;
        a.vout = to_final ? vfinal : valt;
        if (p == 0 && k0dst) {
            a.kout = k0dst;
            a.vout = v0dst;
        }
        a.status = (uint32_t *)(base + pl.off_status[p]);
        if (p == 0)
            rs_kernels<KeyT, ValT, LOADER>::launch(cfg, single, pl.ntiles, s, a);
        else
            rs_kernels<KeyT, ValT, RS_LOAD_PLAIN>::launch(cfg, single, pl.ntiles, s, a);
        SLK_LAUNCH_CHECK(ctx, "k_rs_scatter");
        a.kin = a.kout;
        a.vin = a.vout;
    }
    return SLK_OK;
}

}

int slk_sort_pairs_u32_u32_in(slk_ctx *ctx, slk_buf &scratch, const uint32_t *kin, uint32_t *kout, const uint32_t *vin,
                              uint32_t *vout, size_t n, unsigned end_bit, hipStream_t s, bool clobber) {
    rs_args a;
    memset(&a, 0, sizeof(a));
    a.kin = kin;
    a.vin = vin;
    a.kout = kout;
    a.vout = vout;
    return rs_sort<uint32_t, uint32_t, RS_LOAD_PLAIN>(ctx, scratch, a, n, 0, end_bit, clobber ? (void *)kin : nullptr,
                                                      clobber ? (void *)vin : nullptr, s);
}

int slk_sort_pairs_u64_u32_in(slk_ctx *ctx, slk_buf &scratch, const uint64_t *kin, uint64_t *kout, const uint32_t *vin,
                              uint32_t *vout, size_t n, unsigned end_bit, hipStream_t s, bool clobber) {
    rs_args a;
    memset(&a, 0, sizeof(a));
    a.kin = kin;
    a.vin = vin;
    a.kout = kout;
    a.vout = vout;
    return rs_sort<uint64_t, uint32_t, RS_LOAD_PLAIN>(ctx, scratch, a, n, 0, end_bit, clobber ? (void *)kin : nullptr,
                                                      clobber ? (void *)vin : nullptr, s);
}

int slk_sort_pairs_u32_u32(slk_ctx *ctx, const uint32_t *kin, uint32_t *kout, const uint32_t *vin, uint32_t *vout, size_t n,
                           unsigned end_bit, hipStream_t s, bool clobber) {
    return slk_sort_pairs_u32_u32_in(ctx, ctx->sort_tmp, kin, kout, vin, vout, n, end_bit, s, clobber);
}

int slk_sort_pairs_u32_u64(slk_ctx *ctx, const uint32_t *kin, uint32_t *kout, const uint64_t *vin, uint64_t *vout, size_t n,
                           unsigned end_bit, hipStream_t s, bool clobber) {
    rs_args a;
    memset(&a, 0, sizeof(a));
    a.kin = kin;
    a.vin = vin;
    a.kout = kout;
    a.vout = vout;
    return rs_sort<uint32_t, uint64_t, RS_LOAD_PLAIN>(ctx, ctx->sort_tmp, a, n, 0, end_bit, clobber ? (void *)kin : nullptr,
                                                      clobber ? (void *)vin : nullptr, s);
}

int slk_sort_fy_steps(slk_ctx *ctx, slk_buf &scratch, const uint32_t *J, uint32_t n, uint32_t *const key[2], uint32_t *const val[2],
                      hipStream_t s) {
    rs_args a;
    memset(&a, 0, sizeof(a));
    a.uit = J;
    a.fy_n = n;
    a.kout = key[1];
    a.vout = val[1];
    return rs_sort<uint32_t, uint32_t, RS_LOAD_FY_STEPS>(ctx, scratch, a, (size_t)n - 1, 0, slk_bits_for((uint64_t)n), key[0], val[0], s);
}

int slk_sort_pairs_any(slk_ctx *ctx, int kind, const void *kin, void *kout, const void *vin, void *vout, size_t n, size_t seg_len,
                       unsigned bits, hipStream_t s, bool clobber) {
    rs_args a;
    memset(&a, 0, sizeof(a));
    a.kin = kin;
    a.vin = vin;
    a.kout = kout;
    a.vout = vout;
    void *ka = clobber ? (void *)kin : nullptr, *va = clobber ? (void *)vin : nullptr;
    if (kind == 0) return rs_sort<uint32_t, uint32_t, RS_LOAD_PLAIN>(ctx, ctx->sort_tmp, a, n, seg_len, bits, ka, va, s);
    if (kind == 1) return rs_sort<uint32_t, uint64_t, RS_LOAD_PLAIN>(ctx, ctx->sort_tmp, a, n, seg_len, bits, ka, va, s);
    if (kind == 2) return rs_sort<uint64_t, uint32_t, RS_LOAD_PLAIN>(ctx, ctx->sort_tmp, a, n, seg_len, bits, ka, va, s);
    return slk_fail(ctx, SLK_EINVAL, "slk_sort_pairs_any: kind %d", kind);
}

static bool rs_segmented(size_t n, size_t seg_len) { return seg_len < n && seg_len >= 32768; }

template <class KeyT, class ValT, int LOADER>
static int rs_sort_fused(slk_ctx *ctx, rs_args a, size_t n, size_t seg_len, unsigned idbits, unsigned mbbits, void *const key[2],
                         void *const val[2], hipStream_t s) {
    a.idbits = idbits;
    a.kout = key[1];
    a.vout = val[1];
    const bool seg = rs_segmented(n, seg_len), one = seg_len >= n;
    a.kseg = seg ? 0u : (uint32_t)seg_len;
    return rs_sort<KeyT, ValT, LOADER>(ctx, ctx->sort_tmp, a, n, seg ? seg_len : 0, (seg || one) ? idbits : idbits + mbbits, key[0],
                                       val[0], s);
}

int slk_sort_user_fat(slk_ctx *ctx, const int64_t *users, const int64_t *items, const uint32_t *neg32, size_t nc, size_t bsz,
                      unsigned ubits, unsigned mbbits, uint32_t *const key[2], uint64_t *const val[2], hipStream_t s) {
    rs_args a;
    memset(&a, 0, sizeof(a));
    a.users = users;
    a.items = items;
    a.neg32 = neg32;
    return rs_sort_fused<uint32_t, uint64_t, RS_LOAD_USER_FAT>(ctx, a, nc, bsz, ubits, mbbits, (void *const *)key, (void *const *)val, s);
}

int slk_sort_user_idx(slk_ctx *ctx, const int64_t *users, size_t nc, size_t bsz, unsigned ubits, unsigned mbbits,
                      uint32_t *const key[2], uint32_t *const val[2], hipStream_t s) {
    rs_args a;
    memset(&a, 0, sizeof(a));
    a.users = users;
    return rs_sort_fused<uint32_t, uint32_t, RS_LOAD_USER_IDX>(ctx, a, nc, bsz, ubits, mbbits, (void *const *)key, (void *const *)val, s);
}

int slk_sort_item_occ(slk_ctx *ctx, const uint32_t *uit, size_t nocc, size_t bsz, int NP, unsigned ibits, unsigned mbbits,
                      uint32_t *const key[2], uint32_t *const val[2], hipStream_t s) {
    rs_args a;
    memset(&a, 0, sizeof(a));
    a.uit = uit;
    return rs_sort_fused<uint32_t, uint32_t, RS_LOAD_ITEM_OCC>(ctx, a, nocc, bsz * (size_t)NP, ibits, mbbits, (void *const *)key,
                                                               (void *const *)val, s);
}

int slk_sort_reserve(slk_ctx *ctx, size_t n) {
    if (n == 0) return SLK_OK;
    rs_plan pl;
    rs_make_plan(pl, n, 0, 32, 4096);
    size_t need = pl.ctl_bytes;
    need += (size_t)pl.ntiles * RS_RADIX * 4 * 4;
    return slk_ensure(ctx, ctx->sort_tmp, need);
}
```

Measured before the change: 1.636 billion.

## Add MSD top-digit scatter plus in-LDS bucket finish for large radix sorts

```diff
diff --git a/spotlight_amd/csrc/slk_api.hip b/spotlight_amd/csrc/slk_api.hip
--- a/spotlight_amd/csrc/slk_api.hip
+++ b/spotlight_amd/csrc/slk_api.hip
@@ -285,6 +285,15 @@
     else if (!strcmp(name, "lds_per_block")) *value = (int64_t)ctx->lds_per_block;
     else if (!strcmp(name, "lds_per_cu")) *value = (int64_t)ctx->lds_per_cu;
     else if (!strcmp(name, "prefetch_pending")) *value = !ctx->pf.valid ? 0 : (ctx->pf.all ? 2 : 1);
+    else if (!strcmp(name, "sort_finish_cap")) *value = slk_sort_finish_cap();
+    else if (!strcmp(name, "sort_finish_sorts")) *value = ctx->stat_sort_finish_sorts;
+    else if (!strcmp(name, "sort_finish_fallbacks")) {
+        uint32_t h = 0;
+        SLK_HIP(ctx, hipSetDevice(ctx->device));
+        SLK_HIP(ctx, hipDeviceSynchronize());
+        SLK_HIP(ctx, hipMemcpy(&h, &ctx->d_rng->sort_fallbacks, sizeof(h), hipMemcpyDeviceToHost));
+        *value = (int64_t)h;
+    }
     else return slk_fail(ctx, SLK_EINVAL, "slk_ctx_get_stat: unknown statistic %s", name);
     return SLK_OK;
 }
diff --git a/spotlight_amd/csrc/slk_bilinear.hip b/spotlight_amd/csrc/slk_bilinear.hip
--- a/spotlight_amd/csrc/slk_bilinear.hip
+++ b/spotlight_amd/csrc/slk_bilinear.hip
@@ -1259,11 +1259,13 @@
     uint32_t *const ukeys[2] = {u32p(pb.ukey[0]), ukey};
     if (!p.pre) {
         uint64_t *const uvals[2] = {(uint64_t *)pb.uval[0].p, (uint64_t *)pb.uval[1].p};
-        if ((rc = slk_sort_user_fat(ctx, cu, ci, neg32, nc, (size_t)bsz, p.ubits, mbbits, ukeys, uvals, s))) return rc;
+        if ((rc = slk_sort_user_fat(ctx, cu, ci, neg32, nc, (size_t)bsz, p.ubits, mbbits, (size_t)c.tables->num_users, ukeys, uvals,
+                                    s)))
+            return rc;
         uit = u32p(pb.uval[1]);
     } else {
         uint32_t *const uvals[2] = {u32p(pb.uval[0]), u32p(pb.uval[1])};
-        if ((rc = slk_sort_user_idx(ctx, cu, nc, (size_t)bsz, p.ubits, mbbits, ukeys, uvals, s))) return rc;
+        if ((rc = slk_sort_user_idx(ctx, cu, nc, (size_t)bsz, p.ubits, mbbits, (size_t)c.tables->num_users, ukeys, uvals, s))) return rc;
         uk = u32p(pb.uval[1]);
         hipLaunchKernelGGL(k_pack_items, dim3(slk_grid_for(ctx, nc, 256)), dim3(256), 0, s, uk, ci, neg32, nc, p.nn, u32p(pb.uit));
         SLK_LAUNCH_CHECK(ctx, "k_pack_items");
@@ -1275,7 +1277,8 @@
     } else {
         uint32_t *const ikeys[2] = {u32p(pb.ikey[0]), u32p(pb.ikey[1])};
         uint32_t *const ivals[2] = {u32p(pb.ipay[0]), u32p(pb.ipay[1])};
-        if ((rc = slk_sort_item_occ(ctx, uit, nocc, (size_t)bsz, p.NP, p.ibits, mbbits, ikeys, ivals, s))) return rc;
+        if ((rc = slk_sort_item_occ(ctx, uit, nocc, (size_t)bsz, p.NP, p.ibits, mbbits, (size_t)c.tables->num_items, ikeys, ivals, s)))
+            return rc;
         if (p.sgl_on && (rc = prep_single_flags(ctx, p, c, pb, ck, s))) return rc;
     }
     if (!run.epoch_route) {
diff --git a/spotlight_amd/csrc/slk_common.h b/spotlight_amd/csrc/slk_common.h
--- a/spotlight_amd/csrc/slk_common.h
+++ b/spotlight_amd/csrc/slk_common.h
@@ -61,6 +61,8 @@
     unsigned long long accepted;
     int32_t epoch_abort;
     int32_t sort_abort;
+    uint32_t sort_fallbacks;
+    uint32_t pad_;
 };
 
 #define SLK_EXTRA_BUFS 56
@@ -201,6 +203,7 @@
     int64_t stat_shadowed = 0;
     int64_t stat_pingpong = 0;
     int64_t stat_single = 0;
+    int64_t stat_sort_finish_sorts = 0;
     int last_pipe_set = -1;
     uint32_t ipart_gen = 0;
     uint32_t upart_gen = 0;
@@ -284,11 +287,11 @@
 int slk_sort_pairs_any(slk_ctx *ctx, int kind, const void *kin, void *kout, const void *vin, void *vout, size_t n, size_t seg_len,
                        unsigned bits, hipStream_t s, bool clobber);
 int slk_sort_user_fat(slk_ctx *ctx, const int64_t *users, const int64_t *items, const uint32_t *neg32, size_t nc, size_t bsz,
-                      unsigned ubits, unsigned mbbits, uint32_t *const key[2], uint64_t *const val[2], hipStream_t s);
-int slk_sort_user_idx(slk_ctx *ctx, const int64_t *users, size_t nc, size_t bsz, unsigned ubits, unsigned mbbits,
+                      unsigned ubits, unsigned mbbits, size_t num_users, uint32_t *const key[2], uint64_t *const val[2], hipStream_t s);
+int slk_sort_user_idx(slk_ctx *ctx, const int64_t *users, size_t nc, size_t bsz, unsigned ubits, unsigned mbbits, size_t num_users,
                       uint32_t *const key[2], uint32_t *const val[2], hipStream_t s);
 int slk_sort_item_occ(slk_ctx *ctx, const uint32_t *uit, size_t nocc, size_t bsz, int NP, unsigned ibits, unsigned mbbits,
-                      uint32_t *const key[2], uint32_t *const val[2], hipStream_t s);
+                      size_t num_items, uint32_t *const key[2], uint32_t *const val[2], hipStream_t s);
 
 int slk_eval_predict_all(slk_ctx *ctx, const slk_tables *tables, const float *rep, const float *rbias, const int64_t *gmap,
                          float *d_out, hipStream_t s);
@@ -300,6 +303,7 @@
 int slk_launch_i64_to_u32(slk_ctx *ctx, const int64_t *in, uint32_t *out, size_t n, hipStream_t s);
 
 int slk_sort_reserve(slk_ctx *ctx, size_t n);
+int64_t slk_sort_finish_cap(void);
 int slk_compact_heads(slk_ctx *ctx, const uint32_t *d_sorted, uint32_t n, uint32_t *d_heads, uint32_t *d_segid,
                       uint32_t *nseg_out, hipStream_t s);
 bool slk_epoch_eligible(const slk_ctx *ctx, const slk_tables *tables, const slk_optim *optim, int64_t bsz, int loss, bool bloom);
diff --git a/spotlight_amd/csrc/slk_sort.hip b/spotlight_amd/csrc/slk_sort.hip
--- a/spotlight_amd/csrc/slk_sort.hip
+++ b/spotlight_amd/csrc/slk_sort.hip
@@ -1,3 +1,5 @@
+#include <math.h>
+
 #include "slk_common.h"
 
 namespace {
@@ -31,6 +33,12 @@
     int xcd;
     uint32_t nseg;
     int debug;
+    int topw, topshift;
+    uint32_t *tpre;
+    uint32_t *btot, *bbase;
+    uint32_t *nofit;
+    uint32_t *fallbacks;
+    int gate;
 };
 
 template <class KeyT>
@@ -77,6 +85,7 @@
 template <class KeyT, int LOADER>
 __global__ __launch_bounds__(256) void k_rs_hist(rs_args a) {
     __shared__ uint32_t sh[RS_MAX_PASS * RS_RADIX];
+    if (a.gate && !*a.nofit) return;
     const uint32_t seg = blockIdx.x / a.hbps, hb = blockIdx.x - seg * a.hbps;
     const uint32_t s0 = seg * a.seg_len;
     const uint32_t s1 = (a.n - s0 < a.seg_len) ? a.n : s0 + a.seg_len;
@@ -126,6 +135,7 @@
 
 __global__ __launch_bounds__(256) void k_rs_scan(rs_args a) {
     __shared__ uint32_t s_wsum[4];
+    if (a.gate && !*a.nofit) return;
     const uint32_t seg = blockIdx.x / (uint32_t)a.npass;
     const size_t o = (size_t)blockIdx.x * RS_RADIX + threadIdx.x;
     const uint32_t c = a.hist[o];
@@ -182,7 +192,7 @@
     return true;
 }
 
-template <class KeyT, class ValT, int THREADS, int KPT, int LOADER, bool SINGLE>
+template <class KeyT, class ValT, int THREADS, int KPT, int LOADER, bool SINGLE, bool TOP = false>
 __global__ __launch_bounds__(THREADS) SLK_WAVES_PER_EU_RANGE(4, 6) void k_rs_scatter(rs_args a) {
     constexpr int WAVES = THREADS / 64, KW = WAVES, TILE = KW * 64 * KPT;
     constexpr int OPT = (TILE + THREADS - 1) / THREADS;
@@ -196,9 +206,14 @@
 
     const int lane = threadIdx.x & 63, wave = threadIdx.x >> 6;
     constexpr bool is_key = true;
-    const int shift = a.shift[a.pass], nbits = a.width[a.pass];
+    if (TOP) {
+        if (*a.nofit) return;
+    } else if (!SINGLE && a.gate && !*a.nofit) {
+        return;
+    }
+    const int shift = TOP ? a.topshift : a.shift[a.pass], nbits = TOP ? a.topw : a.width[a.pass];
     const uint32_t radix = 1u << nbits, dmask = radix - 1u;
-    if (!SINGLE && threadIdx.x == 0) {
+    if (!SINGLE && !TOP && threadIdx.x == 0) {
         if (a.xcd) {
             const uint32_t x0 = rs_xcc_id();
             uint32_t t = 0xffffffffu;
@@ -217,7 +232,7 @@
     for (int i = threadIdx.x; i < KW * RS_RADIX; i += THREADS) s_cnt[i] = 0u;
     if (threadIdx.x < RS_RADIX) s_lbase[threadIdx.x] = 0u;
     __syncthreads();
-    const uint32_t tile = SINGLE ? 0u : s_tile;
+    const uint32_t tile = SINGLE ? 0u : (TOP ? blockIdx.x : s_tile);
     if (tile == 0xffffffffu) return;
     const uint32_t seg = tile / a.tps, tis = tile - seg * a.tps;
     const uint32_t s0 = seg * a.seg_len;
@@ -250,7 +265,7 @@
                 if (e < cnt) rs_load<KeyT, ValT, LOADER>(a, t0 + e, seg, key[j], val[j]);
             }
         }
-        if (!SINGLE) {
+        if (!SINGLE && !TOP) {
 #pragma unroll
             for (int j = 0; j < KPT; ++j)
                 if (e0 + (uint32_t)j * 64u < cnt) atomicAdd(&s_lbase[rs_digit<KeyT>(key[j], shift, dmask)], 1u);
@@ -262,7 +277,7 @@
             val[j] = 0;
         }
     }
-    if (!SINGLE) __syncthreads();
+    if (!SINGLE && !TOP) __syncthreads();
 
     uint32_t tcount = 0, before = 0;
     uint32_t *wcnt = s_cnt + (is_key ? wave : 0) * RS_RADIX;
@@ -289,7 +304,8 @@
     };
     {
         const uint32_t d = threadIdx.x;
-        if (!SINGLE && d < radix) {
+        if (TOP && d < radix) before = a.tpre[(size_t)tile * radix + d];
+        if (!SINGLE && !TOP && d < radix) {
             tcount = s_lbase[d];
             __hip_atomic_store(a.status + (size_t)tile * radix + d, ((tis == 0 ? RS_INC : RS_AGG) << 30) | tcount, __ATOMIC_RELAXED,
                                __HIP_MEMORY_SCOPE_AGENT);
@@ -308,12 +324,13 @@
                 s_cnt[w * RS_RADIX + d] = run;
                 run += c;
             }
-            if (SINGLE) tcount = run;
+            if (SINGLE || TOP) tcount = run;
         }
         const uint32_t lb = rs_block_excl_scan<THREADS>(tcount, s_wsum);
         if (d < radix) {
             uint32_t gbase = lb;
-            if (!SINGLE) gbase = a.base[((size_t)seg * a.npass + a.pass) * RS_RADIX + d];
+            if (TOP) gbase = a.bbase[(size_t)seg * RS_RADIX + d];
+            else if (!SINGLE) gbase = a.base[((size_t)seg * a.npass + a.pass) * RS_RADIX + d];
             s_lbase[d] = lb;
             s_goff[d] = gbase + before - lb;
         }
@@ -358,10 +375,203 @@
     }
 }
 
+
+#ifndef RS_FIN_THREADS
+#define RS_FIN_THREADS 512
+#endif
+#ifndef RS_FIN_KPT
+#define RS_FIN_KPT 18
+#endif
+#ifndef RS_FIN_MIN_SEG
+#define RS_FIN_MIN_SEG (1 << 20)
+#endif
+constexpr uint32_t RS_FIN_CAP = (uint32_t)RS_FIN_THREADS * RS_FIN_KPT;
+static_assert(RS_FIN_KPT % 2 == 0 && RS_FIN_THREADS % 64 == 0 && RS_FIN_THREADS >= RS_RADIX && RS_FIN_CAP <= 65536u, "finish tile shape");
+
+template <class KeyT, int LOADER, int THREADS, int KPT>
+__global__ __launch_bounds__(THREADS) void k_rs_tile_hist(rs_args a) {
+    constexpr uint32_t TILE = (uint32_t)THREADS * KPT;
+    __shared__ uint32_t sh[RS_RADIX];
+    const uint32_t tile = blockIdx.x, seg = tile / a.tps, tis = tile - seg * a.tps;
+    const uint32_t s0 = seg * a.seg_len;
+    const uint32_t s1 = (a.n - s0 < a.seg_len) ? a.n : s0 + a.seg_len;
+    const uint32_t t0 = s0 + tis * TILE;
+    const uint32_t cnt = t0 >= s1 ? 0u : ((s1 - t0 < TILE) ? s1 - t0 : TILE);
+    const uint32_t radix = 1u << a.topw, dmask = radix - 1u;
+    for (uint32_t i = threadIdx.x; i < radix; i += THREADS) sh[i] = 0u;
+    __syncthreads();
+    KeyT k[KPT];
+#pragma unroll
+    for (int j = 0; j < KPT; ++j) {
+        const uint32_t e = (uint32_t)j * THREADS + threadIdx.x;
+        k[j] = e < cnt ? rs_load_key<KeyT, LOADER>(a, t0 + e, seg) : (KeyT)0;
+    }
+#pragma unroll
+    for (int j = 0; j < KPT; ++j)
+        if ((uint32_t)j * THREADS + threadIdx.x < cnt) atomicAdd(&sh[rs_digit<KeyT>(k[j], a.topshift, dmask)], 1u);
+    __syncthreads();
+    for (uint32_t i = threadIdx.x; i < radix; i += THREADS) a.tpre[(size_t)tile * radix + i] = sh[i];
+}
+
+__global__ __launch_bounds__(256) void k_rs_tile_scan(rs_args a) {
+    __shared__ uint32_t s_part[256];
+    const uint32_t radix = 1u << a.topw;
+    const uint32_t dg = radix < 32u ? radix : 32u, ngr = radix / dg, parts = 256u / dg;
+    const uint32_t seg = blockIdx.x / ngr, dl = threadIdx.x % dg, part = threadIdx.x / dg;
+    const uint32_t d = (blockIdx.x - seg * ngr) * dg + dl;
+    const uint32_t tpp = (a.tps + parts - 1u) / parts;
+    const uint32_t ta = part * tpp < a.tps ? part * tpp : a.tps, tb = ta + tpp < a.tps ? ta + tpp : a.tps;
+    uint32_t *col = a.tpre + (size_t)seg * a.tps * radix + d;
+    uint32_t sum = 0;
+#pragma unroll 8
+    for (uint32_t t = ta; t < tb; ++t) sum += col[(size_t)t * radix];
+    s_part[threadIdx.x] = sum;
+    __syncthreads();
+    uint32_t run = 0, tot = 0;
+    for (uint32_t p = 0; p < parts; ++p) {
+        const uint32_t v = s_part[p * dg + dl];
+        if (p < part) run += v;
+        tot += v;
+    }
+    for (uint32_t t = ta; t < tb; t += 8u) {
+        uint32_t c[8];
+#pragma unroll
+        for (uint32_t u = 0; u < 8u; ++u) c[u] = t + u < tb ? col[(size_t)(t + u) * radix] : 0u;
+#pragma unroll
+        for (uint32_t u = 0; u < 8u; ++u) {
+            if (t + u < tb) col[(size_t)(t + u) * radix] = run;
+            run += c[u];
+        }
+    }
+    if (part == 0) a.btot[(size_t)seg * RS_RADIX + d] = tot;
+}
+
+__global__ __launch_bounds__(256) void k_rs_bucket_base(rs_args a) {
+    __shared__ uint32_t s_wsum[4];
+    __shared__ uint32_t s_over;
+    const uint32_t seg = blockIdx.x, d = threadIdx.x, radix = 1u << a.topw;
+    if (d == 0) s_over = 0u;
+    const uint32_t c = d < radix ? a.btot[(size_t)seg * RS_RADIX + d] : 0u;
+    const uint32_t ex = rs_block_excl_scan<256>(c, s_wsum);
+    if (d < radix) a.bbase[(size_t)seg * RS_RADIX + d] = seg * a.seg_len + ex;
+    if (c > RS_FIN_CAP) atomicOr(&s_over, 1u);
+    __syncthreads();
+    if (d == 0 && s_over && atomicExch(a.nofit, 1u) == 0u) atomicAdd(a.fallbacks, 1u);
+}
+
+template <class ValT>
+__global__ __launch_bounds__(RS_FIN_THREADS) SLK_WAVES_PER_EU_RANGE(4, 8) void k_rs_finish(rs_args a) {
+    constexpr int THREADS = RS_FIN_THREADS, KPT = RS_FIN_KPT, WAVES = THREADS / 64;
+    __shared__ uint32_t s_cnt[WAVES * RS_RADIX];
+    __shared__ uint32_t s_lbase[RS_RADIX];
+    __shared__ uint32_t s_wsum[WAVES];
+    __shared__ uint32_t s_x[RS_FIN_CAP];
+    if (*a.nofit) return;
+    const uint32_t seg = blockIdx.x >> a.topw, b = blockIdx.x & ((1u << a.topw) - 1u);
+    const uint32_t cnt = a.btot[(size_t)seg * RS_RADIX + b];
+    if (cnt == 0u) return;
+    const uint32_t b0 = a.bbase[(size_t)seg * RS_RADIX + b];
+    const uint32_t *kin = (const uint32_t *)a.kin + b0;
+    const ValT *vin = (const ValT *)a.vin + b0;
+    const int lane = threadIdx.x & 63, wave = threadIdx.x >> 6;
+    const uint32_t e0 = (uint32_t)wave * 64u * KPT + (uint32_t)lane;
+    uint32_t key[KPT];
+    ValT val[KPT];
+    uint32_t pos2[KPT / 2];
+#pragma unroll
+    for (int j = 0; j < KPT; ++j) {
+        const uint32_t e = e0 + (uint32_t)j * 64u;
+        key[j] = e < cnt ? kin[e] : 0u;
+    }
+#pragma unroll
+    for (int j = 0; j < KPT; ++j) {
+        const uint32_t e = e0 + (uint32_t)j * 64u;
+        val[j] = e < cnt ? vin[e] : (ValT)0;
+    }
+    const int rem = a.topshift, R = (rem + RS_RB - 1) / RS_RB, lo = rem / R, extra = rem % R;
+    uint32_t *wcnt = s_cnt + wave * RS_RADIX;
+    int shift = 0;
+    for (int r = 0; r < R; ++r) {
+        const int nbits = lo + (r < extra ? 1 : 0);
+        const uint32_t radix = 1u << nbits, dmask = radix - 1u;
+        for (int i = threadIdx.x; i < WAVES * RS_RADIX; i += THREADS) s_cnt[i] = 0u;
+        __syncthreads();
+#pragma unroll
+        for (int j = 0; j < KPT; ++j) {
+            if ((j & 1) == 0) pos2[j / 2] = 0u;
+            if ((uint32_t)wave * 64u * KPT + (uint32_t)j * 64u >= cnt) continue;
+            const bool valid = e0 + (uint32_t)j * 64u < cnt;
+            const uint32_t dj = rs_digit<uint32_t>(key[j], shift, dmask);
+            const unsigned long long m = rs_match(dj, nbits, valid);
+            const int leader = m ? __ffsll((long long)m) - 1 : lane;
+            uint32_t first = 0;
+            if (m && lane == leader) first = atomicAdd(&wcnt[dj], (uint32_t)__popcll(m));
+            first = __shfl(first, leader);
+            const uint32_t rk = first + (uint32_t)__popcll(m & ((1ull << lane) - 1ull));
+            pos2[j / 2] = (j & 1) ? (pos2[j / 2] | (rk << 16)) : rk;
+        }
+        __syncthreads();
+        uint32_t tcount = 0;
+        if (threadIdx.x < radix) {
+            uint32_t run = 0;
+            for (int w = 0; w < WAVES; ++w) {
+                const uint32_t c = s_cnt[w * RS_RADIX + threadIdx.x];
+                s_cnt[w * RS_RADIX + threadIdx.x] = run;
+                run += c;
+            }
+            tcount = run;
+        }
+        const uint32_t lb = rs_block_excl_scan<THREADS>(tcount, s_wsum);
+        if (threadIdx.x < radix) s_lbase[threadIdx.x] = lb;
+        __syncthreads();
+#pragma unroll
+        for (int j = 0; j < KPT; ++j) {
+            if (e0 + (uint32_t)j * 64u < cnt) {
+                const uint32_t dj = rs_digit<uint32_t>(key[j], shift, dmask);
+                const uint32_t pj = ((pos2[j / 2] >> ((j & 1) * 16)) & 0xffffu) + s_lbase[dj] + wcnt[dj];
+                pos2[j / 2] = (j & 1) ? ((pos2[j / 2] & 0xffffu) | (pj << 16)) : ((pos2[j / 2] & 0xffff0000u) | pj);
+                s_x[pj] = key[j];
+            }
+        }
+        __syncthreads();
+#pragma unroll
+        for (int j = 0; j < KPT; ++j)
+            if (e0 + (uint32_t)j * 64u < cnt) key[j] = s_x[e0 + (uint32_t)j * 64u];
+        __syncthreads();
+#pragma unroll
+        for (int h = 0; h < (int)(sizeof(ValT) / 4); ++h) {
+#pragma unroll
+            for (int j = 0; j < KPT; ++j)
+                if (e0 + (uint32_t)j * 64u < cnt)
+                    s_x[(pos2[j / 2] >> ((j & 1) * 16)) & 0xffffu] = (uint32_t)((uint64_t)val[j] >> (32 * h));
+            __syncthreads();
+#pragma unroll
+            for (int j = 0; j < KPT; ++j)
+                if (e0 + (uint32_t)j * 64u < cnt) {
+                    const uint64_t w32 = s_x[e0 + (uint32_t)j * 64u];
+                    if (sizeof(ValT) == 4) val[j] = (ValT)w32;
+                    else val[j] = (ValT)(h == 0 ? (((uint64_t)val[j] & 0xffffffff00000000ull) | w32)
+                                                : (((uint64_t)val[j] & 0xffffffffull) | (w32 << 32)));
+                }
+            __syncthreads();
+        }
+        shift += nbits;
+    }
+    uint32_t *kout = (uint32_t *)a.kout + b0;
+    ValT *vout = (ValT *)a.vout + b0;
+#pragma unroll
+    for (int j = 0; j < KPT; ++j)
+        if (e0 + (uint32_t)j * 64u < cnt) kout[e0 + (uint32_t)j * 64u] = key[j];
+#pragma unroll
+    for (int j = 0; j < KPT; ++j)
+        if (e0 + (uint32_t)j * 64u < cnt) vout[e0 + (uint32_t)j * 64u] = val[j];
+}
+
 struct rs_plan {
     uint32_t n = 0, seg_len = 0, nseg = 0, tps = 0, ntiles = 0, hbps = 0;
     int npass = 0, shift[RS_MAX_PASS], width[RS_MAX_PASS];
     size_t off_ticket = 0, off_status[RS_MAX_PASS], zero_bytes = 0, off_base = 0, off_data = 0, ctl_bytes = 0;
+    size_t off_tpre = 0, off_btot = 0, off_bbase = 0;
 };
 
 static void rs_split_bits(unsigned bits, int *npass, int *shift, int *width) {
@@ -378,7 +588,19 @@
     *npass = P;
 }
 
-static void rs_make_plan(rs_plan &pl, size_t n, size_t seg_len, unsigned bits, unsigned tile) {
+static int rs_pick_topw(size_t seg_len, unsigned bits, size_t krange) {
+    const double full = ldexp(1.0, (int)bits);
+    double fill[2] = {0.5, 1.0};
+    if (krange) fill[0] = fill[1] = (double)krange < full ? (double)krange / full : 1.0;
+    for (int f = 0; f < 2; ++f)
+        for (int w = 1; w <= RS_RB; ++w) {
+            const double mean = (double)seg_len / (ldexp(1.0, w) * fill[f]);
+            if (mean + 6.0 * sqrt(mean) <= (double)RS_FIN_CAP) return w;
+        }
+    return 0;
+}
+
+static void rs_make_plan(rs_plan &pl, size_t n, size_t seg_len, unsigned bits, unsigned tile, int topw = 0) {
     pl.n = (uint32_t)n;
     pl.seg_len = (uint32_t)(seg_len && seg_len < n ? seg_len : n);
     pl.nseg = (uint32_t)((n + pl.seg_len - 1) / pl.seg_len);
@@ -397,6 +619,14 @@
     o = (o + 255) & ~(size_t)255;
     pl.off_base = o;
     o += (size_t)pl.nseg * pl.npass * RS_RADIX * 4;
+    if (topw > 0) {
+        pl.off_tpre = o = (o + 255) & ~(size_t)255;
+        o += (size_t)pl.ntiles * ((size_t)1 << topw) * 4;
+        pl.off_btot = o = (o + 255) & ~(size_t)255;
+        o += (size_t)pl.nseg * RS_RADIX * 4;
+        pl.off_bbase = o;
+        o += (size_t)pl.nseg * RS_RADIX * 4;
+    }
     pl.off_data = (o + 255) & ~(size_t)255;
     pl.ctl_bytes = pl.off_data;
 }
@@ -424,7 +654,7 @@
 
 template <class KeyT, class ValT, int LOADER>
 static int rs_sort(slk_ctx *ctx, slk_buf &scratch, rs_args a, size_t n, size_t seg_len, unsigned bits, void *kalt, void *valt,
-                   hipStream_t s) {
+                   hipStream_t s, size_t krange = 0) {
     if (n == 0) return SLK_OK;
     if (n >= ((size_t)1 << 31)) return slk_fail(ctx, SLK_EINVAL, "sort of %zu pairs: at most 2^31 - 1", n);
     if (bits > 8 * sizeof(KeyT)) bits = 8 * sizeof(KeyT);
@@ -432,15 +662,21 @@
     const bool single = LOADER == RS_LOAD_PLAIN && n <= 4096 && (seg_len == 0 || seg_len >= n);
     const int cfg = (!single && n >= (size_t)ctx->opt_sort_big_min) ? 1 : 0;
     const unsigned tile = rs_tile_of(cfg);
+    int topw = 0;
+    if (sizeof(KeyT) == 4 && LOADER != RS_LOAD_FY_STEPS && cfg == 1 && seg_len > 0 && bits > (unsigned)RS_RB &&
+        (seg_len < n ? seg_len : n) >= ((size_t)ctx->opt_sort_big_min < (size_t)RS_FIN_MIN_SEG ? (size_t)ctx->opt_sort_big_min : (size_t)RS_FIN_MIN_SEG))
+        topw = rs_pick_topw(seg_len < n ? seg_len : n, bits, krange);
     rs_plan pl;
-    rs_make_plan(pl, n, single ? 0 : seg_len, bits, tile);
+    rs_make_plan(pl, n, single ? 0 : seg_len, bits, tile, topw);
     if (pl.seg_len >= (1u << 30)) return slk_fail(ctx, SLK_EINVAL, "sort segment of %u pairs: at most 2^30 - 1", pl.seg_len);
     const bool inplace0 = kalt && kalt == a.kin && (pl.npass & 1) == 0;
-    const bool need_tmp = pl.npass > 1 && (!kalt || inplace0);
+    const bool need_tmp = (pl.npass > 1 && (!kalt || inplace0)) || (topw && kalt && kalt == a.kin);
     const size_t koff = pl.off_data, voff = (koff + n * sizeof(KeyT) + 255) & ~(size_t)255;
     int rc = slk_ensure(ctx, scratch, need_tmp ? voff + n * sizeof(ValT) : pl.ctl_bytes);
     if (rc) return rc;
     char *base = (char *)scratch.p;
+    void *const kmid = (kalt && kalt != a.kin) ? kalt : (void *)(base + koff);
+    void *const vmid = (kalt && kalt != a.kin) ? valt : (void *)(base + voff);
     void *k0dst = nullptr, *v0dst = nullptr;
     if (need_tmp && !kalt) {
         kalt = base + koff;
@@ -467,8 +703,40 @@
     a.nseg = pl.nseg;
     a.xcd = pl.nseg >= 2 ? 1 : 0;
     void *kfinal = a.kout, *vfinal = a.vout;
+    if (!single) SLK_HIP(ctx, hipMemsetAsync(base, 0, pl.zero_bytes, s));
+    if constexpr (sizeof(KeyT) == 4 && LOADER != RS_LOAD_FY_STEPS) {
+        if (topw) {
+            a.topw = topw;
+            a.topshift = (int)bits - topw;
+            a.tpre = (uint32_t *)(base + pl.off_tpre);
+            a.btot = (uint32_t *)(base + pl.off_btot);
+            a.bbase = (uint32_t *)(base + pl.off_bbase);
+            a.nofit = a.ticket + 120;
+            a.fallbacks = &ctx->d_rng->sort_fallbacks;
+            const unsigned ngr = (1u << topw) < 32u ? 1u : (1u << topw) / 32u;
+            hipLaunchKernelGGL((k_rs_tile_hist<KeyT, LOADER, RS_BIG_THREADS, RS_BIG_KPT>), dim3(pl.ntiles), dim3(RS_BIG_THREADS), 0, s, a);
+            SLK_LAUNCH_CHECK(ctx, "k_rs_tile_hist");
+            hipLaunchKernelGGL(k_rs_tile_scan, dim3(pl.nseg * ngr), dim3(256), 0, s, a);
+            SLK_LAUNCH_CHECK(ctx, "k_rs_tile_scan");
+            hipLaunchKernelGGL(k_rs_bucket_base, dim3(pl.nseg), dim3(256), 0, s, a);
+            SLK_LAUNCH_CHECK(ctx, "k_rs_bucket_base");
+            rs_args t = a;
+            t.kout = kmid;
+            t.vout = vmid;
+            hipLaunchKernelGGL((k_rs_scatter<KeyT, ValT, RS_BIG_THREADS, RS_BIG_KPT, LOADER, false, true>), dim3(pl.ntiles), dim3(RS_BIG_THREADS),
+                               0, s, t);
+            SLK_LAUNCH_CHECK(ctx, "k_rs_scatter (top digit)");
+            t.kin = kmid;
+            t.vin = vmid;
+            t.kout = kfinal;
+            t.vout = vfinal;
+            hipLaunchKernelGGL((k_rs_finish<ValT>), dim3(pl.nseg << topw), dim3(RS_FIN_THREADS), 0, s, t);
+            SLK_LAUNCH_CHECK(ctx, "k_rs_finish");
+            a.gate = 1;
+            ++ctx->stat_sort_finish_sorts;
+        }
+    }
     if (!single) {
-        SLK_HIP(ctx, hipMemsetAsync(base, 0, pl.zero_bytes, s));
         a.pass = 0;
         hipLaunchKernelGGL((k_rs_hist<KeyT, LOADER>), dim3(pl.nseg * pl.hbps), dim3(256), 0, s, a);
         SLK_LAUNCH_CHECK(ctx, "k_rs_hist");
@@ -568,43 +836,45 @@
 static bool rs_segmented(size_t n, size_t seg_len) { return seg_len < n && seg_len >= 32768; }
 
 template <class KeyT, class ValT, int LOADER>
-static int rs_sort_fused(slk_ctx *ctx, rs_args a, size_t n, size_t seg_len, unsigned idbits, unsigned mbbits, void *const key[2],
-                         void *const val[2], hipStream_t s) {
+static int rs_sort_fused(slk_ctx *ctx, rs_args a, size_t n, size_t seg_len, unsigned idbits, unsigned mbbits, size_t nids,
+                         void *const key[2], void *const val[2], hipStream_t s) {
     a.idbits = idbits;
     a.kout = key[1];
     a.vout = val[1];
     const bool seg = rs_segmented(n, seg_len), one = seg_len >= n;
     a.kseg = seg ? 0u : (uint32_t)seg_len;
     return rs_sort<KeyT, ValT, LOADER>(ctx, ctx->sort_tmp, a, n, seg ? seg_len : 0, (seg || one) ? idbits : idbits + mbbits, key[0],
-                                       val[0], s);
+                                       val[0], s, nids);
 }
 
 int slk_sort_user_fat(slk_ctx *ctx, const int64_t *users, const int64_t *items, const uint32_t *neg32, size_t nc, size_t bsz,
-                      unsigned ubits, unsigned mbbits, uint32_t *const key[2], uint64_t *const val[2], hipStream_t s) {
+                      unsigned ubits, unsigned mbbits, size_t num_users, uint32_t *const key[2], uint64_t *const val[2], hipStream_t s) {
     rs_args a;
     memset(&a, 0, sizeof(a));
     a.users = users;
     a.items = items;
     a.neg32 = neg32;
-    return rs_sort_fused<uint32_t, uint64_t, RS_LOAD_USER_FAT>(ctx, a, nc, bsz, ubits, mbbits, (void *const *)key, (void *const *)val, s);
-}
-
-int slk_sort_user_idx(slk_ctx *ctx, const int64_t *users, size_t nc, size_t bsz, unsigned ubits, unsigned mbbits,
+    return rs_sort_fused<uint32_t, uint64_t, RS_LOAD_USER_FAT>(ctx, a, nc, bsz, ubits, mbbits, num_users, (void *const *)key, (void *const *)val, s);
+}
+
+int slk_sort_user_idx(slk_ctx *ctx, const int64_t *users, size_t nc, size_t bsz, unsigned ubits, unsigned mbbits, size_t num_users,
                       uint32_t *const key[2], uint32_t *const val[2], hipStream_t s) {
     rs_args a;
     memset(&a, 0, sizeof(a));
     a.users = users;
-    return rs_sort_fused<uint32_t, uint32_t, RS_LOAD_USER_IDX>(ctx, a, nc, bsz, ubits, mbbits, (void *const *)key, (void *const *)val, s);
+    return rs_sort_fused<uint32_t, uint32_t, RS_LOAD_USER_IDX>(ctx, a, nc, bsz, ubits, mbbits, num_users, (void *const *)key, (void *const *)val, s);
 }
 
 int slk_sort_item_occ(slk_ctx *ctx, const uint32_t *uit, size_t nocc, size_t bsz, int NP, unsigned ibits, unsigned mbbits,
-                      uint32_t *const key[2], uint32_t *const val[2], hipStream_t s) {
+                      size_t num_items, uint32_t *const key[2], uint32_t *const val[2], hipStream_t s) {
     rs_args a;
     memset(&a, 0, sizeof(a));
     a.uit = uit;
-    return rs_sort_fused<uint32_t, uint32_t, RS_LOAD_ITEM_OCC>(ctx, a, nocc, bsz * (size_t)NP, ibits, mbbits, (void *const *)key,
+    return rs_sort_fused<uint32_t, uint32_t, RS_LOAD_ITEM_OCC>(ctx, a, nocc, bsz * (size_t)NP, ibits, mbbits, num_items, (void *const *)key,
                                                                (void *const *)val, s);
 }
+
+int64_t slk_sort_finish_cap(void) { return (int64_t)RS_FIN_CAP; }
 
 int slk_sort_reserve(slk_ctx *ctx, size_t n) {
     if (n == 0) return SLK_OK;
@@ -612,5 +882,6 @@
     rs_make_plan(pl, n, 0, 32, 4096);
     size_t need = pl.ctl_bytes;
     need += (size_t)pl.ntiles * RS_RADIX * 4 * 4;
+    need += ((n / rs_tile_of(1)) + n / 32768 + 2) * RS_RADIX * 4 + (n / 32768 + 2) * RS_RADIX * 8 + 1024;
     return slk_ensure(ctx, ctx->sort_tmp, need);
 }
```

Measured after the change: 1.685 billion (median of 6 runs). 3.0% higher.
